# keisuke-777/HandyRL

Measured on AMD Instinct MI355X. Metric: learner env-steps/sec at B=4096 T=32 (TicTacToe net, UPGO/VTRACE), higher is better.
Workload: dtype f32; 1 GPU; TicTacToe SimpleConv2dModel learner step: forward + IS ratios + fused HIP V-trace/UPGO scans + losses + backward + grad all-reduce + clip + Adam; global_batch=4096, per_gpu_batch=4096, seq_len=32, players=2, parallelism=dp1, hip_graph=True

## Files before the change

### handyrl_amd/_native.py

```python

import ctypes
import os

import torch

LIB_PATH = os.path.join(os.path.dirname(os.path.abspath(__file__)), '_lib', 'libhrl.so')
LIB_PATH = os.environ.get('HRL_LIB_PATH', LIB_PATH)

HRL_OK = 0
HRL_EINVAL = -22

ALG = {'MC': 0, 'TD': 1, 'UPGO': 2, 'VTRACE': 3}

_f32p = ctypes.c_void_p
_i64 = ctypes.c_int64
_dbl = ctypes.c_double

SIGNATURES = {
    'hrl_abi_version': (ctypes.c_int, []),
    'hrl_targets_set_short_form': (ctypes.c_int, [ctypes.c_int]),
    'hrl_strerror': (ctypes.c_char_p, [ctypes.c_int]),
    'hrl_compute_target': (ctypes.c_int, [
        ctypes.c_int, _f32p, _f32p, _f32p, _f32p, _f32p,
        _i64, _i64, _i64, _i64, _i64, _i64, _dbl, _dbl, _f32p, _f32p, ctypes.c_void_p]),
    'hrl_compute_targets_fused': (ctypes.c_int, [
        ctypes.c_int, ctypes.c_int, _f32p, _f32p, _f32p, _f32p, _f32p,
        _i64, _i64, _i64, _i64, _i64, _i64, _dbl, _dbl, _f32p, _f32p, ctypes.c_void_p]),
    'hrl_bn_workspace_bytes': (ctypes.c_int64, [_i64, _i64, _i64]),
    'hrl_bn_forward_train': (ctypes.c_int, [
        _f32p, _i64, _i64, _i64, _f32p, _f32p, _f32p, _f32p, _dbl, _dbl, ctypes.c_int, _f32p, _f32p, _f32p,
        ctypes.c_void_p, _i64, ctypes.c_void_p]),
    'hrl_bn_backward': (ctypes.c_int, [
        _f32p, _f32p, _i64, _i64, _i64, _f32p, _f32p, _f32p, _f32p, ctypes.c_int, _f32p, _f32p, _f32p,
        ctypes.c_void_p, _i64, ctypes.c_void_p]),
    'hrl_bn_workspace_bytes_grouped': (ctypes.c_int64, [_i64, _i64, _i64, _i64]),
    'hrl_bn_forward_train_grouped': (ctypes.c_int, [
        _f32p, _i64, _i64, _i64, _i64, _f32p, _f32p, _f32p, _f32p, _dbl, _dbl, ctypes.c_int, _f32p, _f32p, _f32p,
        ctypes.c_void_p, _i64, ctypes.c_void_p]),
    'hrl_bn_backward_grouped': (ctypes.c_int, [
        _f32p, _f32p, _i64, _i64, _i64, _i64, _f32p, _f32p, _f32p, _f32p, ctypes.c_int, _f32p, _f32p, _f32p,
        ctypes.c_void_p, _i64, ctypes.c_void_p]),
    'hrl_loss_workspace_bytes': (ctypes.c_int64, [_i64, _i64, _i64, _i64]),
    'hrl_loss_forward': (ctypes.c_int, [
        _f32p, _f32p, ctypes.c_void_p, _i64, _i64, _i64, _i64, _i64,
        _f32p, _f32p, _f32p, _f32p, _f32p, _f32p, _f32p, _f32p, _f32p,
        ctypes.c_int, ctypes.c_int, ctypes.c_int, _dbl, _dbl, _dbl, _dbl,
        ctypes.c_void_p, _i64, _f32p, ctypes.c_void_p]),
    'hrl_loss_backward': (ctypes.c_int, [
        _f32p, ctypes.c_void_p, _i64, _i64, _i64, _i64, _i64,
        _f32p, _f32p, _f32p, _f32p, _f32p, _f32p, _dbl, _dbl,
        ctypes.c_void_p, _i64, _f32p, _f32p, _f32p, _f32p, ctypes.c_void_p]),
    'hrl_output_mask_forward': (ctypes.c_int, [_f32p, _f32p, _f32p, _f32p, _f32p, _i64, _i64, _i64, _i64, _f32p,
                                               _f32p, ctypes.c_void_p]),
    'hrl_output_mask_backward': (ctypes.c_int, [_f32p, _f32p, _f32p, _f32p, _i64, _i64, _i64, _i64, _f32p, _f32p,
                                                ctypes.c_void_p]),
    'hrl_board_weight': (ctypes.c_int, [_f32p, _i64, _i64, _i64, _i64, _i64, _i64, _f32p, ctypes.c_void_p]),
    'hrl_board_fold': (ctypes.c_int, [_f32p, _i64, _i64, _i64, _i64, _i64, _i64, _f32p, ctypes.c_void_p]),
    'hrl_board_bias': (ctypes.c_int, [_f32p, _i64, _i64, _f32p, ctypes.c_void_p]),
    'hrl_board_bias_fold': (ctypes.c_int, [_f32p, _i64, _i64, _f32p, ctypes.c_void_p]),
    'hrl_conv3x3_workspace_bytes': (ctypes.c_int64, [_i64]),
    'hrl_conv3x3_forward': (ctypes.c_int, [_f32p, _i64, _i64, _i64, _f32p, _f32p, ctypes.c_int, _f32p,
                                           ctypes.c_void_p, _i64, ctypes.c_void_p]),
    'hrl_conv3x3_wgrad': (ctypes.c_int, [_f32p, _f32p, _i64, _i64, _i64, _f32p, ctypes.c_void_p, _i64,
                                         ctypes.c_void_p]),
    'hrl_colsum_workspace_bytes': (ctypes.c_int64, [_i64, _i64]),
    'hrl_colsum': (ctypes.c_int, [_f32p, _i64, _i64, _f32p, ctypes.c_void_p, _i64, ctypes.c_void_p]),
    'hrl_bn_finalize_stats': (ctypes.c_int, [ctypes.c_void_p, _i64, _i64, _i64, _f32p, _f32p, _f32p, _f32p,
                                             ctypes.c_double, ctypes.c_double, _f32p, _f32p, _f32p, _f32p,
                                             ctypes.c_void_p]),
    'hrl_bn_forward_eval': (ctypes.c_int, [_f32p, _i64, _i64, _i64, _f32p, _f32p, _f32p, _f32p, ctypes.c_double,
                                           ctypes.c_int, _f32p, _f32p, ctypes.c_void_p]),
    'hrl_bn_apply': (ctypes.c_int, [_f32p, _i64, _i64, _i64, _f32p, _f32p, ctypes.c_int, _f32p, ctypes.c_void_p]),
    'hrl_conv3x3_stats_blocks': (ctypes.c_int64, [_i64]),
    'hrl_conv3x3_block_sum_blocks': (ctypes.c_int64, [_i64]),
    'hrl_conv3x3_set_split': (ctypes.c_int, [ctypes.c_int]),
    'hrl_conv3x3_set_block_form': (ctypes.c_int, [ctypes.c_int]),
    'hrl_conv3x3_set_fwd_form': (ctypes.c_int, [ctypes.c_int]),
    'hrl_torus_set_split': (ctypes.c_int, [ctypes.c_int]),
    'hrl_torus_set_form': (ctypes.c_int, [ctypes.c_int]),
    'hrl_conv3x3_pack_n': (ctypes.c_int, [ctypes.c_void_p, ctypes.c_int, _f32p, ctypes.c_void_p]),
    'hrl_conv3x3_forward_ex': (ctypes.c_int, [_f32p, _i64, _f32p, _f32p, _f32p, _f32p, ctypes.c_int, _f32p,
                                              ctypes.c_int, _f32p, _f32p, _f32p, _f32p, ctypes.c_void_p,
                                              ctypes.c_void_p, _i64, ctypes.c_void_p]),
    'hrl_bn_finalize_backward': (ctypes.c_int, [ctypes.c_void_p, _i64, _i64, _i64, _f32p, _f32p, _f32p, _f32p,
                                                _f32p, _f32p, ctypes.c_void_p]),
    'hrl_bn_backward_apply': (ctypes.c_int, [_f32p, _f32p, _i64, _i64, _i64, _f32p, _f32p, _f32p, _f32p,
                                             ctypes.c_int, _f32p, _f32p, _f32p, ctypes.c_void_p]),
    'hrl_conv3x3_block_backward': (ctypes.c_int, [_f32p, _f32p, _i64, _f32p, _f32p, _f32p, _f32p, _f32p, _f32p,
                                                  _f32p, _f32p, _f32p, _f32p, _f32p, _f32p, ctypes.c_int, _f32p,
                                                  _f32p, _f32p, ctypes.c_void_p, ctypes.c_void_p, _i64,
                                                  ctypes.c_void_p]),
    'hrl_conv3x3_wgrad_ex': (ctypes.c_int, [_f32p, _f32p, _f32p, _f32p, _i64, _f32p, ctypes.c_void_p, _i64,
                                            ctypes.c_void_p]),
    'hrl_hidden_gather': (ctypes.c_int, [ctypes.c_void_p, _f32p, _i64, _i64, ctypes.c_int, ctypes.c_void_p,
                                         ctypes.c_int, ctypes.c_void_p, ctypes.c_void_p]),
    'hrl_hidden_gather_backward': (ctypes.c_int, [ctypes.c_void_p, _f32p, _i64, _i64, ctypes.c_int, ctypes.c_void_p,
                                                  ctypes.c_int, ctypes.c_void_p, ctypes.c_void_p]),
    'hrl_hidden_gather_backward_add': (ctypes.c_int, [ctypes.c_void_p, _f32p, _i64, _i64, ctypes.c_int,
                                                      ctypes.c_void_p, ctypes.c_int, ctypes.c_void_p, ctypes.c_void_p,
                                                      ctypes.c_void_p, ctypes.c_void_p]),
    'hrl_hidden_update_gather': (ctypes.c_int, [ctypes.c_void_p, ctypes.c_void_p, _i64, _f32p, _f32p, _i64, _i64,
                                                ctypes.c_int, ctypes.c_void_p, ctypes.c_int, ctypes.c_void_p,
                                                ctypes.c_void_p, ctypes.c_void_p]),
    'hrl_hidden_update_gather_backward': (ctypes.c_int, [ctypes.c_void_p, _f32p, _f32p, _i64, _i64, _i64,
                                                         ctypes.c_int, ctypes.c_void_p, ctypes.c_int, ctypes.c_void_p,
                                                         ctypes.c_void_p, ctypes.c_void_p, ctypes.c_void_p,
                                                         ctypes.c_void_p, ctypes.c_void_p, ctypes.c_void_p]),
    'hrl_hidden_update_backward_add': (ctypes.c_int, [ctypes.c_void_p, _f32p, _i64, _i64, _i64, ctypes.c_int,
                                                      ctypes.c_void_p, ctypes.c_void_p, ctypes.c_void_p,
                                                      ctypes.c_void_p, ctypes.c_void_p, ctypes.c_void_p]),
    'hrl_hidden_update': (ctypes.c_int, [ctypes.c_void_p, ctypes.c_void_p, _i64, _f32p, _i64, _i64, ctypes.c_int,
                                         ctypes.c_void_p, ctypes.c_void_p, ctypes.c_void_p]),
    'hrl_hidden_update_backward': (ctypes.c_int, [ctypes.c_void_p, _f32p, _i64, _i64, _i64, ctypes.c_int,
                                                  ctypes.c_void_p, ctypes.c_void_p, ctypes.c_void_p, ctypes.c_void_p]),
    'hrl_lstm_gates_forward': (ctypes.c_int, [_f32p, _i64, _f32p, _f32p, _i64, _i64, _i64, _f32p, _i64, _f32p,
                                              _f32p, _f32p, ctypes.c_void_p]),
    'hrl_lstm_gates_backward': (ctypes.c_int, [_f32p, _f32p, _f32p, _f32p, _f32p, _i64, _i64, _i64, _f32p, _f32p,
                                               ctypes.c_void_p]),
    'hrl_torus_workspace_bytes': (ctypes.c_int64, [_i64]),
    'hrl_torus_stats_blocks': (ctypes.c_int64, [_i64]),
    'hrl_torus_conv_forward': (ctypes.c_int, [_f32p, _i64, _i64, _i64, _i64, _i64, _f32p, _f32p, ctypes.c_int,
                                              _f32p, ctypes.c_void_p, _f32p, _f32p, ctypes.c_void_p, _i64,
                                              ctypes.c_void_p]),
    'hrl_stem_workspace_bytes': (ctypes.c_int64, [_i64]),
    'hrl_stem_forward': (ctypes.c_int, [_f32p, _i64, _i64, _f32p, _f32p, _f32p, ctypes.c_void_p]),
    'hrl_stem_wgrad': (ctypes.c_int, [_f32p, _f32p, _i64, _i64, _f32p, _f32p, ctypes.c_void_p, _i64,
                                      ctypes.c_void_p]),
    'hrl_stem_set_wgrad_form': (ctypes.c_int, [ctypes.c_int]),
    'hrl_stem_set_fwd_form': (ctypes.c_int, [ctypes.c_int]),
    'hrl_clip_grad_norm': (ctypes.c_int, [_f32p, _i64, _dbl, _f32p, ctypes.c_void_p]),
    'hrl_clip_workspace_bytes': (ctypes.c_int64, [_i64]),
    'hrl_grad_fold_norm_blocks': (ctypes.c_int64, [_i64]),
    'hrl_grad_fold_norm': (ctypes.c_int, [_f32p, _i64, ctypes.c_void_p, ctypes.c_void_p, ctypes.c_void_p,
                                          ctypes.c_void_p, ctypes.c_void_p, ctypes.c_void_p, ctypes.c_void_p,
                                          ctypes.c_int, _f32p, ctypes.c_void_p, ctypes.c_void_p, ctypes.c_int,
                                          ctypes.c_void_p, _i64, ctypes.c_void_p]),
    'hrl_adam_clip': (ctypes.c_int, [_f32p, _i64, ctypes.c_void_p, _dbl, _f32p, ctypes.c_void_p, ctypes.c_void_p,
                                     ctypes.c_void_p, ctypes.c_int, _f32p, _f32p, _f32p, _f32p, _dbl, _dbl, _dbl,
                                     _dbl, ctypes.c_void_p, ctypes.c_int, _f32p, ctypes.c_void_p]),
    'hrl_conv3x3_wgrad_partials': (ctypes.c_int64, [_i64, ctypes.c_void_p]),
    'hrl_stem_wgrad_partials': (ctypes.c_int64, [_i64, ctypes.c_void_p]),
    'hrl_clip_grad_norm_ws': (ctypes.c_int, [_f32p, _i64, _dbl, _f32p, ctypes.c_void_p, _i64, ctypes.c_void_p]),
    'hrl_heads_workspace_bytes': (ctypes.c_int64, [_i64]),
    'hrl_heads_bn_parts': (ctypes.c_int64, [_i64]),
    'hrl_heads_set_bwd_form': (ctypes.c_int, [ctypes.c_int]),
    'hrl_heads_forward': (ctypes.c_int, [_f32p, _i64, _f32p, _f32p, _f32p, _f32p, _f32p, _f32p, _f32p, _f32p,
                                         _f32p, _f32p, _f32p, _f32p, ctypes.c_int, ctypes.c_void_p]),
    'hrl_heads_backward': (ctypes.c_int, [_f32p, _i64, _f32p, _f32p, _f32p, _f32p, _f32p, _f32p, _f32p,
                                          ctypes.c_void_p, _f32p, _f32p, _f32p, _f32p, _f32p, _f32p, _f32p, _f32p,
                                          _f32p, _f32p, _f32p, _f32p, ctypes.c_void_p, _i64, ctypes.c_void_p]),
    'hrl_bn_apply_residual': (ctypes.c_int, [_f32p, _f32p, _i64, _i64, _i64, _f32p, _f32p, _f32p, ctypes.c_void_p]),
    'hrl_bn_backward_masked': (ctypes.c_int, [_f32p, _f32p, _f32p, _i64, _i64, _i64, _f32p, _f32p, _f32p, _f32p,
                                              _f32p, _f32p, ctypes.c_void_p, _i64, ctypes.c_void_p]),
    'hrl_torus_conv_wgrad': (ctypes.c_int, [_f32p, _f32p, _i64, _i64, _i64, _i64, _i64, _f32p, _f32p,
                                            ctypes.c_void_p, _i64, ctypes.c_void_p]),
    'hrl_torus_conv_wgrad_bn': (ctypes.c_int, [_f32p, _i64, _i64, _i64, _i64, _f32p, _f32p, _f32p, _f32p,
                                               ctypes.c_int, _f32p, _f32p, _f32p, _f32p, _f32p, _f32p, _f32p, _f32p,
                                               ctypes.c_void_p, _i64, ctypes.c_void_p]),
    'hrl_bn_backward_masked_coefs': (ctypes.c_int, [_f32p, _f32p, _f32p, _i64, _i64, _i64, _f32p, _f32p, _f32p,
                                                    _f32p, _f32p, _f32p, _f32p, ctypes.c_void_p, _i64,
                                                    ctypes.c_void_p]),
    'hrl_torus_unit_forward': (ctypes.c_int, [_f32p, _f32p, _f32p, _f32p, _f32p, _i64, _i64, _i64, _f32p, _f32p,
                                              _f32p, ctypes.c_void_p, ctypes.c_void_p, _i64, ctypes.c_void_p]),
    'hrl_torus_unit_input_grad': (ctypes.c_int, [_f32p, _i64, _i64, _i64, _f32p, _f32p, _f32p, _f32p, _f32p,
                                                 _f32p, _f32p, ctypes.c_void_p, ctypes.c_void_p, _i64,
                                                 ctypes.c_void_p]),
    'hrl_board_conv_workspace_bytes': (ctypes.c_int64, [_i64]),
    'hrl_board_conv_forward': (ctypes.c_int, [_f32p, _i64, _i64, _i64, _i64, _f32p, _i64, _i64, _i64, _f32p, _f32p,
                                              ctypes.c_void_p, _i64, ctypes.c_void_p]),
    'hrl_board_conv_pack': (ctypes.c_int, [_f32p, _i64, _i64, _i64, ctypes.c_void_p, _i64, ctypes.c_void_p]),
    'hrl_board_conv_forward_packed': (ctypes.c_int, [_f32p, _i64, _i64, _i64, _i64, ctypes.c_void_p, _i64, _f32p,
                                                     _f32p, ctypes.c_void_p]),
    'hrl_gboard_pack_bytes': (ctypes.c_int64, [_i64, _i64]),
    'hrl_gboard_pack': (ctypes.c_int, [_f32p, _i64, _i64, _i64, _i64, ctypes.c_void_p, _i64, ctypes.c_void_p]),
    'hrl_gboard_pack_adjoint': (ctypes.c_int, [_f32p, _i64, _i64, _i64, _i64, ctypes.c_void_p, _i64,
                                               ctypes.c_void_p]),
    'hrl_gboard_wgrad_workspace_bytes': (ctypes.c_int64, [_i64, _i64, _i64]),
    'hrl_gboard_wgrad': (ctypes.c_int, [ctypes.c_void_p, ctypes.c_void_p, ctypes.c_void_p, ctypes.c_void_p,
                                        ctypes.c_void_p, ctypes.c_int, _i64, _i64, _f32p, _i64, _i64, _f32p,
                                        ctypes.c_void_p, _i64, ctypes.c_void_p]),
    'hrl_gboard_set_whole_ring': (ctypes.c_int, [ctypes.c_int]),
    'hrl_gboard_set_nctw': (ctypes.c_int, [ctypes.c_int]),
    'hrl_gboard_launch_stats': (ctypes.c_int, [ctypes.c_void_p, ctypes.c_int, ctypes.c_int]),
    'hrl_gboard_pointwise_wgrad_workspace_bytes': (_i64, [_i64, _i64, _i64]),
    'hrl_gboard_pointwise_wgrad': (ctypes.c_int, [_f32p, _i64, _f32p, _i64, _i64, _i64, _i64, _f32p, ctypes.c_void_p,
                                                  _i64, ctypes.c_void_p]),
    'hrl_gboard_forward_groups': (ctypes.c_int, [ctypes.c_void_p, ctypes.c_void_p, _i64, _i64, _i64, ctypes.c_void_p,
                                                 _i64, _i64, _f32p, _i64, ctypes.c_void_p]),
    'hrl_lstm_gates_backward_ex': (ctypes.c_int, [_f32p, _f32p, _f32p, _f32p, _i64, ctypes.c_int, _i64, _f32p, _i64,
                                                  _i64, _i64, _f32p, _f32p, _f32p, ctypes.c_int, ctypes.c_void_p]),
    'hrl_lstm_gates_forward_grouped': (ctypes.c_int, [ctypes.c_int, _f32p, _i64, ctypes.c_void_p, ctypes.c_void_p,
                                                      ctypes.c_void_p, _i64, _i64, _i64, ctypes.c_void_p,
                                                      ctypes.c_void_p, ctypes.c_void_p, ctypes.c_void_p]),
    'hrl_gboard_forward': (ctypes.c_int, [_f32p, _i64, _f32p, _i64, _i64, _i64, _i64, ctypes.c_void_p, _i64, _i64,
                                          _f32p, _f32p, _f32p, ctypes.c_int, _f32p, _i64, ctypes.c_void_p]),
    'hrl_gboard_pointwise': (ctypes.c_int, [_f32p, _i64, _i64, _f32p, _i64, _i64, _i64, _f32p, _i64, _f32p, _f32p,
                                            ctypes.c_int, _f32p, _i64, ctypes.c_void_p]),
    'hrl_torus_head_pool': (ctypes.c_int, [_f32p, _f32p, _i64, _i64, _i64, _i64, _f32p, _f32p, ctypes.c_void_p]),
    'hrl_torus_head_unpool': (ctypes.c_int, [_f32p, _f32p, _f32p, _i64, _i64, _i64, _i64, _f32p,
                                             ctypes.c_void_p]),
    'hrl_bn_backward_apply_masked': (ctypes.c_int, [_f32p, _f32p, _f32p, _i64, _i64, _i64, _f32p, _f32p, _f32p,
                                                    _f32p, _f32p, _f32p, ctypes.c_void_p]),
    'hrl_geister_legal': (ctypes.c_int, [ctypes.c_void_p, ctypes.c_void_p, ctypes.c_void_p, _i64, ctypes.c_void_p,
                                         ctypes.c_void_p]),
    'hrl_geister_observation': (ctypes.c_int, [ctypes.c_void_p, ctypes.c_void_p, ctypes.c_void_p, ctypes.c_void_p,
                                               _i64, ctypes.c_int, _f32p, _f32p, ctypes.c_void_p]),
    'hrl_geister_step': (ctypes.c_int, [ctypes.c_void_p, ctypes.c_void_p, ctypes.c_void_p, ctypes.c_void_p,
                                        ctypes.c_void_p, ctypes.c_void_p, ctypes.c_void_p, ctypes.c_void_p,
                                        ctypes.c_void_p, _i64, ctypes.c_void_p, ctypes.c_void_p]),
    'hrl_selfplay_sample_record': (ctypes.c_int, [_f32p, _i64, ctypes.c_void_p, _f32p, ctypes.c_void_p, _f32p,
                                                  ctypes.c_void_p, ctypes.c_void_p, ctypes.c_void_p, _i64, _i64,
                                                  _i64, _i64, ctypes.c_void_p, _f32p, _f32p, ctypes.c_void_p, _f32p,
                                                  ctypes.c_void_p, ctypes.c_void_p, ctypes.c_void_p]),
    'hrl_masked_rows_copy': (ctypes.c_int, [ctypes.c_int, ctypes.c_void_p, ctypes.c_void_p, ctypes.c_void_p,
                                            ctypes.c_void_p, ctypes.c_void_p, ctypes.c_void_p, _i64,
                                            ctypes.c_void_p]),
    'hrl_geister_observation_record': (ctypes.c_int, [ctypes.c_void_p, ctypes.c_void_p, ctypes.c_void_p,
                                                      ctypes.c_void_p, _i64, ctypes.c_int, _f32p, _f32p,
                                                      ctypes.c_void_p, ctypes.c_void_p, _i64, _f32p, _f32p,
                                                      ctypes.c_void_p]),
}

ABI_VERSION = 27

_lib = None


def load():
    global _lib
    if _lib is not None:
        return _lib
    if not os.path.exists(LIB_PATH):
        raise RuntimeError('HIP library %s is missing: run `python -m handyrl_amd.build` '
                           '(there is no CPU fallback for the learner kernels)' % LIB_PATH)
    lib = ctypes.CDLL(LIB_PATH)
    for name, (res, args) in SIGNATURES.items():
        fn = getattr(lib, name)
        fn.restype = res
        fn.argtypes = args
    if lib.hrl_abi_version() != ABI_VERSION:
        raise RuntimeError('libhrl.so ABI %d != expected %d' % (lib.hrl_abi_version(), ABI_VERSION))
    _lib = lib
    return lib


def check(code, what):
    if code != HRL_OK:
        msg = load().hrl_strerror(code).decode()
        if code == HRL_EINVAL:
            raise ValueError('%s: %s' % (what, msg))
        raise RuntimeError('%s failed (%d): %s' % (what, code, msg))


def ptr(t):
    return None if t is None else ctypes.c_void_p(t.data_ptr())


def ptr_array(tensors):
    arr = (ctypes.c_void_p * len(tensors))(*[None if t is None else t.data_ptr() for t in tensors])
    return arr


def i64_array(values):
    return (ctypes.c_int64 * len(values))(*values)


def stream_of(device):
    return ctypes.c_void_p(torch.cuda.current_stream(device).cuda_stream)
```

### handyrl_amd/csrc/hrl_conv.hip

```cpp

#include <hip/hip_runtime.h>
#include <stdint.h>
#include <stdlib.h>

#include <type_traits>

#include "../../include/hrl_nn.h"
#include "../../include/hrl_targets.h"
#include "hrl_split.h"
#include "hrl_stamps.h"

namespace {

HRL_STAMP_DECL

typedef float f32x4 __attribute__((ext_vector_type(4)));

constexpr int kBoard = 3;
constexpr int kCells = kBoard * kBoard;
constexpr int kTaps = 9;
constexpr int kC = 32;
constexpr int kRow = kC * kCells;
constexpr int kStride = kRow + 2;
constexpr int kTile = 16;
// ... 385 lines not shown
                    acc[tap][1][1] = mfma(a1, b1, acc[tap][1][1]);
                }
            }
        }
        __builtin_amdgcn_wave_barrier();
    }
    __syncthreads();
    float *red = lds;
    constexpr int kW = kTaps * kC * kC;
#pragma unroll
    for (int t = 0; t < kTaps; ++t)
#pragma unroll
        for (int it = 0; it < 2; ++it)
#pragma unroll
            for (int jt = 0; jt < 2; ++jt)
#pragma unroll
                for (int r = 0; r < 4; ++r) {
                    const int ci = it * 16 + (lane >> 4) * 4 + r;
                    const int co = jt * 16 + (lane & 15);
                    red[wave * kW + (t * kC + ci) * kC + co] = acc[t][it][jt][r];
                }
    __syncthreads();
    float *out = partial + (int64_t)blockIdx.x * kW;
    for (int i = threadIdx.x; i < kW; i += kThreads)
        out[i] = ((red[i] + red[kW + i]) + red[2 * kW + i]) + red[3 * kW + i];
}

constexpr int kStrideW = kRow + 4;
typedef float f32x16 __attribute__((ext_vector_type(16)));
typedef __bf16 bf16x8_t __attribute__((ext_vector_type(8)));

__device__ __forceinline__ f32x16 mfma32(const uint4 &a, const uint4 &b, f32x16 c) {
    return __builtin_amdgcn_mfma_f32_32x32x16_bf16(__builtin_bit_cast(bf16x8_t, a), __builtin_bit_cast(bf16x8_t, b),
                                                   c, 0, 0, 0);
}

template <bool PRO>
__global__ __launch_bounds__(kThreads) void conv3x3_wgrad_split_kernel(const float *__restrict__ x,
                                                                       const float *__restrict__ in_alpha,
                                                                       const float *__restrict__ in_beta,
                                                                       const float *__restrict__ dy, int64_t M,
                                                                       float *__restrict__ partial) {
    __shared__ __attribute__((aligned(16))) float lds[2 * kWaves * kTile * kStrideW];
    static_assert(2 * kWaves * kTile * kStrideW >= kWaves * kTaps * kC * kC, "fold buffer");
    const int lane = threadIdx.x & 63;
    const int wave = threadIdx.x >> 6;
    float *xs = lds + wave * kTile * kStrideW;
    float *gs = lds + (kWaves + wave) * kTile * kStrideW;
    const int r = lane & 31, h = lane >> 5;
    float pa = 1.f, pb = 0.f;
    if constexpr (PRO) {
        pa = in_alpha[r];
        pb = in_beta[r];
    }
    const int64_t ntiles = (M + kTile - 1) / kTile;
    const int64_t stride = (int64_t)gridDim.x * kWaves;
    const int64_t lim = M * kRow;

    f32x16 acc[kTaps];
#pragma unroll
    for (int t = 0; t < kTaps; ++t)
#pragma unroll
        for (int i = 0; i < 16; ++i) acc[t][i] = 0.f;

    for (int64_t tile = (int64_t)blockIdx.x * kWaves + wave; tile < ntiles; tile += stride) {
        {
            const int64_t base = tile * kTile * kRow;
            float4 sx[kVec], sg[kVec];
#pragma unroll
            for (int k = 0; k < kVec; ++k) {
                const int64_t e = base + (int64_t)(k * 64 + lane) * 4;
                const int64_t ec = e < lim ? e : lim - 4;
                sx[k] = *reinterpret_cast<const float4 *>(x + ec);
                sg[k] = *reinterpret_cast<const float4 *>(dy + ec);
            }
#pragma unroll
            for (int k = 0; k < kVec; ++k) {
                const int e = (k * 64 + lane) * 4;
                const int row = e / kRow, c = e - row * kRow;
                const bool ok = base + e < lim;
                *reinterpret_cast<float4 *>(xs + row * kStrideW + c) = sx[k];
                *reinterpret_cast<float4 *>(gs + row * kStrideW + c) = ok ? sg[k] : make_float4(0.f, 0.f, 0.f, 0.f);
            }
        }
        __builtin_amdgcn_s_waitcnt(0xc07f);
        __builtin_amdgcn_wave_barrier();

        uint4 Bh[kCells], Bm[kCells], Bl[kCells];
        const float *gcol = gs + (8 * h) * kStrideW + r * kCells;
#pragma unroll
        for (int q = 0; q < kCells; ++q) {
            float v[8];
#pragma unroll
            for (int j = 0; j < 8; ++j) v[j] = gcol[j * kStrideW + q];
            hrl_split::split8(v, Bh[q], Bm[q], Bl[q]);
        }
        const float *xcol = xs + (8 * h) * kStrideW + r * kCells;
#pragma unroll
        for (int p = 0; p < kCells; ++p) {
            float v[8];
#pragma unroll
            for (int j = 0; j < 8; ++j) {
                float a = xcol[j * kStrideW + p];
                if constexpr (PRO) {
                    const float t = a * pa + pb;
                    a = t < 0.f ? 0.f : t;
                }
                v[j] = a;
            }
            uint4 Ah, Am, Al;
            hrl_split::split8(v, Ah, Am, Al);
#pragma unroll
            for (int q = 0; q < kCells; ++q) {
                const int tap = tap_of(p, q);
                if (tap < 0) continue;
                f32x16 c = acc[tap];
                c = mfma32(Al, Bh[q], c);
                c = mfma32(Am, Bm[q], c);
                c = mfma32(Ah, Bl[q], c);
                c = mfma32(Am, Bh[q], c);
                c = mfma32(Ah, Bm[q], c);
                c = mfma32(Ah, Bh[q], c);
                acc[tap] = c;
            }
        }
        __builtin_amdgcn_wave_barrier();
    }
    __syncthreads();
    float *red = lds;
    constexpr int kW = kTaps * kC * kC;
#pragma unroll
    for (int t = 0; t < kTaps; ++t)
#pragma unroll
        for (int i = 0; i < 16; ++i) {
            const int ci = (i & 3) + 8 * (i >> 2) + 4 * h;
            red[wave * kW + (t * kC + ci) * kC + r] = acc[t][i];
        }
    __syncthreads();
    float *out = partial + (int64_t)blockIdx.x * kW;
    for (int i = threadIdx.x; i < kW; i += kThreads)
        out[i] = ((red[i] + red[kW + i]) + red[2 * kW + i]) + red[3 * kW + i];
}

struct BlockBwdArgs {
    const float *g, *y;
    const float *bn_w, *bn_b, *bn_mean, *bn_invstd, *bn_k, *bn_gm;
    const float *x, *in_alpha, *in_beta;
    const float *wpk;
    const float *ep_mean, *ep_alpha, *ep_beta;
    float *gin;
    double *part;
    float *wpart;
    int64_t M;
};

typedef unsigned int u32x3 __attribute__((ext_vector_type(3)));
typedef unsigned int u32x2 __attribute__((ext_vector_type(2)));
typedef unsigned int u32x4 __attribute__((ext_vector_type(4)));

__device__ __forceinline__ __amdgpu_buffer_rsrc_t wave_rsrc(const void *base, uint32_t bytes) {
    const uint64_t p = reinterpret_cast<uint64_t>(base);
    const uint32_t lo = __builtin_amdgcn_readfirstlane((uint32_t)p);
    const uint32_t hi = __builtin_amdgcn_readfirstlane((uint32_t)(p >> 32));
    const uint32_t n = __builtin_amdgcn_readfirstlane(bytes);
    return __builtin_amdgcn_make_buffer_rsrc(reinterpret_cast<void *>(((uint64_t)hi << 32) | lo), (short)0, (int)n,
                                             0x00020000);
}

__device__ __forceinline__ void load_cells(__amdgpu_buffer_rsrc_t rs, int off, float (&d)[kCells]) {
#pragma unroll
    for (int m = 0; m < 3; ++m) {
        const u32x3 v = __builtin_amdgcn_raw_buffer_load_b96(rs, off + 12 * m, 0, 0);
        d[3 * m + 0] = __uint_as_float(v.x);
        d[3 * m + 1] = __uint_as_float(v.y);
        d[3 * m + 2] = __uint_as_float(v.z);
    }
}

__device__ __forceinline__ void store_cells(__amdgpu_buffer_rsrc_t rs, int off, const float (&d)[kCells]) {
#pragma unroll
    for (int m = 0; m < 3; ++m) {
        u32x3 v;
        v.x = __float_as_uint(d[3 * m + 0]);
        v.y = __float_as_uint(d[3 * m + 1]);
        v.z = __float_as_uint(d[3 * m + 2]);
        __builtin_amdgcn_raw_buffer_store_b96(v, rs, off + 12 * m, 0, 0);
    }
}

template <bool PRO, int EPI, bool DG>
__global__ __launch_bounds__(kThreads) void conv3x3_block_bwd_kernel(BlockBwdArgs a) {
    constexpr int kWWords = kTaps * 2 * 3 * 64 * 4;
    constexpr int kTileF = kTile * kStride;
    constexpr int kW = kTaps * kC * kC;
    constexpr int kFoldF = (kWaves - 1) * kW;
    constexpr int kUseF = DG ? kWWords + kWaves * kTileF : 0;
    constexpr int kSmemF = kUseF > kFoldF ? kUseF : kFoldF;
    __shared__ __attribute__((aligned(16))) float smem[kSmemF];
    uint32_t *w_lds_u = reinterpret_cast<uint32_t *>(smem);
    const int lane = threadIdx.x & 63;
    const int wave = threadIdx.x >> 6;
    float *as = smem + kWWords + wave * kTileF;
    if constexpr (DG) {
        for (int i = threadIdx.x; i < kWWords; i += kThreads) {
            const int d = i & 3, l = (i >> 2) & 63, f = i >> 8;
            const int part = f % 3, tc = f / 3;
            const int ci = 8 * (l >> 4) + 2 * d, j = l & 15;
            const float w0 = a.wpk[(tc * kC + ci) * 16 + j];
            const float w1 = a.wpk[(tc * kC + ci + 1) * 16 + j];
            w_lds_u[i] = split_part(w0, part) | (split_part(w1, part) << 16);
        }
    }
    const int r = lane & 31, h = lane >> 5;
    const float mu = a.bn_mean[r], kk = a.bn_k[r], gmn = a.bn_gm[r], is = a.bn_invstd[r];
    const float ww = a.bn_w ? a.bn_w[r] : 1.0f;
    const float al = is * ww;
    const float be = (a.bn_b ? a.bn_b[r] : 0.0f) - mu * al;
    float pa = 1.f, pb = 0.f;
    if constexpr (PRO) {
        pa = a.in_alpha[r];
        pb = a.in_beta[r];
    }
    float em = 0.f, ea = 1.f, eb = 0.f;
    if constexpr (DG && EPI == 2) {
        em = a.ep_mean[r];
        ea = a.ep_alpha[r];
        eb = a.ep_beta[r];
    }
    double s1 = 0.0, s2 = 0.0;
    f32x16 wacc[kTaps];
#pragma unroll
    for (int t = 0; t < kTaps; ++t)
#pragma unroll
        for (int i = 0; i < 16; ++i) wacc[t][i] = 0.f;
    if constexpr (DG) __syncthreads();

    const int64_t ntiles = (a.M + kTile - 1) / kTile;
    const int64_t stride = (int64_t)gridDim.x * kWaves;
    const int off0 = ((8 * h) * kRow + r * kCells) * 4;
    HRL_STAMP_WALL(14);
    int st_it = 0;
    for (int64_t tile = (int64_t)blockIdx.x * kWaves + wave; tile < ntiles; tile += stride, ++st_it) {
        if (st_it < 2) HRL_STAMP(6 * st_it + 0);
        const int64_t row0 = tile * kTile;
        const int rows = (int)min<int64_t>(kTile, a.M - row0);
        const uint32_t bytes = (uint32_t)rows * kRow * 4;
        const int64_t eofs = row0 * kRow;
        const __amdgpu_buffer_rsrc_t rg = wave_rsrc(a.g + eofs, bytes);
        const __amdgpu_buffer_rsrc_t ry = wave_rsrc(a.y + eofs, bytes);
        const __amdgpu_buffer_rsrc_t rx = wave_rsrc(a.x + eofs, bytes);
        float G[8][kCells], X[8][kCells];
        {
            float Y[8][kCells];
            auto bn_apply = [&]() __attribute__((always_inline)) {
#pragma unroll
                for (int j = 0; j < 8; ++j) {
                    const bool valid = 8 * h + j < rows;
#pragma unroll
                    for (int c = 0; c < kCells; ++c) {
                        const float yv = Y[j][c];
                        float gv = G[j][c];
                        if (!(yv * al + be > 0.f)) gv = 0.f;
                        const float t = (yv - mu) * kk;
                        const float d = (((gv - gmn) - t) * is) * ww;
                        G[j][c] = valid ? d : 0.f;
                    }
                }
            };
#pragma unroll
            for (int j = 0; j < 8; ++j) {
                load_cells(rg, off0 + j * kRow * 4, G[j]);
                load_cells(ry, off0 + j * kRow * 4, Y[j]);
                load_cells(rx, off0 + j * kRow * 4, X[j]);
            }
            bn_apply();
        }
        if (st_it < 2) HRL_STAMP(6 * st_it + 1);
        if constexpr (DG) {
#pragma unroll
            for (int j = 0; j < 8; ++j)
#pragma unroll
                for (int c = 0; c < kCells; ++c) as[(8 * h + j) * kStride + r * kCells + c] = G[j][c];
        }
        {
            uint4 Bh[kCells], Bm[kCells], Bl[kCells];
#pragma unroll
            for (int q = 0; q < kCells; ++q) {
                float v[8];
#pragma unroll
                for (int j = 0; j < 8; ++j) v[j] = G[j][q];
                hrl_split::split8(v, Bh[q], Bm[q], Bl[q]);
            }
#pragma unroll
            for (int p = 0; p < kCells; ++p) {
                float v[8];
#pragma unroll
                for (int j = 0; j < 8; ++j) {
                    float xv = X[j][p];
                    if constexpr (PRO) {
                        const float t = xv * pa + pb;
                        xv = t < 0.f ? 0.f : t;
                    }
                    v[j] = xv;
                }
                uint4 Ah, Am, Al;
                hrl_split::split8(v, Ah, Am, Al);
#pragma unroll
                for (int q = 0; q < kCells; ++q) {
                    const int tap = tap_of(p, q);
                    if (tap < 0) continue;
                    f32x16 c = wacc[tap];
                    c = mfma32(Al, Bh[q], c);
                    c = mfma32(Am, Bm[q], c);
                    c = mfma32(Ah, Bl[q], c);
                    c = mfma32(Am, Bh[q], c);
                    c = mfma32(Ah, Bm[q], c);
                    c = mfma32(Ah, Bh[q], c);
                    wacc[tap] = c;
                }
            }
        }
        if (st_it < 2) HRL_STAMP(6 * st_it + 2);
        if constexpr (DG) {
            float R[8][kCells];
            if constexpr (EPI == 2 || EPI == 3) {
#pragma unroll
                for (int j = 0; j < 8; ++j) load_cells(rx, off0 + j * kRow * 4, R[j]);
            }
            __builtin_amdgcn_s_waitcnt(0xc07f);
            __builtin_amdgcn_wave_barrier();
            f32x4 acc[kCells][2];
#pragma unroll
            for (int q = 0; q < kCells; ++q) acc[q][0] = acc[q][1] = (f32x4){0.f, 0.f, 0.f, 0.f};
            split_tile_mfma<false, true>(as, w_lds_u, lane, nullptr, nullptr, acc);
            __builtin_amdgcn_s_waitcnt(0xc07f);
            __builtin_amdgcn_wave_barrier();
            if (st_it < 2) HRL_STAMP(6 * st_it + 3);
#pragma unroll
            for (int q = 0; q < kCells; ++q)
#pragma unroll
                for (int ct = 0; ct < 2; ++ct)
#pragma unroll
                    for (int rr = 0; rr < 4; ++rr) {
                        const int row = (lane >> 4) * 4 + rr;
                        const int co = ct * 16 + (lane & 15);
                        as[row * kStride + co * kCells + q] = acc[q][ct][rr];
                    }
            __builtin_amdgcn_s_waitcnt(0xc07f);
            __builtin_amdgcn_wave_barrier();
            const __amdgpu_buffer_rsrc_t ro = wave_rsrc(a.gin + eofs, bytes);
            float t1 = 0.f, t2 = 0.f;
#pragma unroll
            for (int j = 0; j < 8; ++j) {
                const bool valid = 8 * h + j < rows;
                float o[kCells];
#pragma unroll
                for (int c = 0; c < kCells; ++c) {
                    float v = as[(8 * h + j) * kStride + r * kCells + c];
                    const float rv = (EPI == 2 || EPI == 3) ? R[j][c] : 0.f;
                    if constexpr (EPI == 3) {
                        if (!(rv > 0.f)) v = 0.f;
                    } else if constexpr (EPI == 2) {
                        const float gm = (rv * ea + eb > 0.f && valid) ? v : 0.f;
                        t1 += gm;
                        t2 += gm * (rv - em);
                    }
                    o[c] = v;
                }
                store_cells(ro, off0 + j * kRow * 4, o);
            }
            if constexpr (EPI == 2) {
                s1 += (double)t1;
                s2 += (double)t2;
            }
            __builtin_amdgcn_s_waitcnt(0xc07f);
            __builtin_amdgcn_wave_barrier();
        }
        if (st_it < 2) HRL_STAMP(6 * st_it + 4);
    }
    HRL_STAMP(12);
    __syncthreads();
    float *red = smem;
    if (wave > 0) {
#pragma unroll
        for (int t = 0; t < kTaps; ++t)
#pragma unroll
            for (int i = 0; i < 16; ++i) {
                const int ci = (i & 3) + 8 * (i >> 2) + 4 * h;
                red[(wave - 1) * kW + (t * kC + ci) * kC + r] = wacc[t][i];
            }
    }
    __syncthreads();
    if (wave == 0) {
        float *out = a.wpart + (int64_t)blockIdx.x * kW;
#pragma unroll
        for (int t = 0; t < kTaps; ++t)
#pragma unroll
            for (int i = 0; i < 16; ++i) {
                const int idx = (t * kC + (i & 3) + 8 * (i >> 2) + 4 * h) * kC + r;
                out[idx] = ((wacc[t][i] + red[idx]) + red[kW + idx]) + red[2 * kW + idx];
            }
    }
    if constexpr (DG && EPI == 2) {
        __syncthreads();
        double *dred = reinterpret_cast<double *>(smem);
        dred[((wave * 2 + h) * kC + r) * 2 + 0] = s1;
        dred[((wave * 2 + h) * kC + r) * 2 + 1] = s2;
        __syncthreads();
        if (threadIdx.x < 2 * kC) {
            const int c = threadIdx.x >> 1, k = threadIdx.x & 1;
            double t = 0.0;
            for (int i = 0; i < 2 * kWaves; ++i) t += dred[(i * kC + c) * 2 + k];
            a.part[((int64_t)blockIdx.x * kC + c) * 2 + k] = t;
        }
    }
    HRL_STAMP(13);
    HRL_STAMP_WALL(15);
}

namespace bb2 {

constexpr int kWaves = 8;
constexpr int kThreads = 64 * kWaves;
constexpr int kPartBytes = kCells * kC * kTile * 2;
constexpr int kImgBytes = 3 * kPartBytes;
constexpr int kDy0 = 0;
constexpr int kX0 = 2 * kImgBytes;
constexpr int kXrStride = kRow + 4;
constexpr int kXrBytes = kTile * kXrStride * 4;
constexpr int kXr0 = 4 * kImgBytes;
constexpr int kLdsBytes = kXr0 + 2 * kXrBytes;
static_assert(kLdsBytes <= 160 * 1024, "LDS");

typedef short v4s __attribute__((ext_vector_type(4)));
typedef __attribute__((address_space(3))) v4s lds_v4s;

__device__ __forceinline__ int img_off(int c, int ch, int half) {
    const int R = ch >> 3, j = ch & 7;
    return c * 1024 + R * 256 + 16 * ((2 * j + half) ^ (9 * (R & 1)));
}

__device__ __forceinline__ void bar_lds() {
    asm volatile("s_waitcnt lgkmcnt(0)" ::: "memory");
    __builtin_amdgcn_s_barrier();
    asm volatile("" ::: "memory");
}

template <int W> struct Role;
template <> struct Role<0> { static constexpr bool kIg = true, kCFirst = true; static constexpr int kCt = 0, kNq = 5, kNt = 0;
                             static constexpr int kQ[5] = {4, 5, 6, 7, 8}; static constexpr int kTap[1] = {0}; };
template <> struct Role<1> { static constexpr bool kIg = true, kCFirst = true; static constexpr int kCt = 1, kNq = 5, kNt = 0;
                             static constexpr int kQ[5] = {4, 5, 6, 7, 8}; static constexpr int kTap[1] = {0}; };
template <> struct Role<2> { static constexpr bool kIg = true, kCFirst = false; static constexpr int kCt = 0, kNq = 4, kNt = 0;
                             static constexpr int kQ[4] = {0, 1, 2, 3}; static constexpr int kTap[1] = {0}; };
template <> struct Role<3> { static constexpr bool kIg = true, kCFirst = false; static constexpr int kCt = 1, kNq = 4, kNt = 0;
                             static constexpr int kQ[4] = {0, 1, 2, 3}; static constexpr int kTap[1] = {0}; };
template <> struct Role<4> { static constexpr bool kIg = false, kCFirst = false; static constexpr int kCt = 0, kNq = 0, kNt = 2;
                             static constexpr int kQ[1] = {0}; static constexpr int kTap[2] = {0, 1}; };
template <> struct Role<5> { static constexpr bool kIg = false, kCFirst = false; static constexpr int kCt = 0, kNq = 0, kNt = 2;
                             static constexpr int kQ[1] = {0}; static constexpr int kTap[2] = {2, 5}; };
template <> struct Role<6> { static constexpr bool kIg = false, kCFirst = true; static constexpr int kCt = 0, kNq = 0, kNt = 2;
                             static constexpr int kQ[1] = {0}; static constexpr int kTap[2] = {3, 4}; };
template <> struct Role<7> { static constexpr bool kIg = false, kCFirst = true; static constexpr int kCt = 0, kNq = 0, kNt = 3;
                             static constexpr int kQ[1] = {0}; static constexpr int kTap[3] = {6, 7, 8}; };

template <int W> __device__ constexpr bool uses_p(int p) {
    using R = Role<W>;
    if constexpr (R::kIg) {
        for (int s = 0; s < R::kNq; ++s)
            if (tap_of(p, R::kQ[s]) >= 0) return true;
    } else {
        for (int s = 0; s < R::kNt; ++s) {
            const int dy = R::kTap[s] / 3, dx = R::kTap[s] % 3;
            const int qy = p / 3 - dy + 1, qx = p % 3 - dx + 1;
            if (qy >= 0 && qy < 3 && qx >= 0 && qx < 3) return true;
        }
    }
    return false;
}
template <int W> __device__ constexpr bool uses_tap(int t) {
    using R = Role<W>;
    for (int s = 0; s < R::kNq; ++s)
        for (int p = 0; p < kCells; ++p)
            if (tap_of(p, R::kQ[s]) == t) return true;
    return false;
}

#ifdef HRL_STAMPS
#define BB2_STAMP(it, k)                                                                                        \
    do {                                                                                                       \
        if ((it) == 2 || (it) == 3) {                                                                          \
            const unsigned long long t_ = __builtin_amdgcn_s_memtime();                                        \
            if (lane == 0 && g_hrl_stamps)                                                                     \
                g_hrl_stamps[(((size_t)blockIdx.x * 8 + W) * 2 + (it) - 2) * 8 + (k)] = t_;                    \
        }                                                                                                      \
    } while (0)
#else
#define BB2_STAMP(it, k) do { } while (0)
#endif

template <bool PRO, int EPI, int W>
__device__ __forceinline__ void run(const BlockBwdArgs &a, unsigned char *smem, int lane) {
    using R = Role<W>;
    constexpr bool kIg = R::kIg;
    constexpr int kNq = R::kNq > 0 ? R::kNq : 1;
    constexpr int kNt = R::kNt > 0 ? R::kNt : 1;
    constexpr int kCt = R::kCt;
    const int ch = lane & 31, hh = lane >> 5;
    constexpr bool kFwd = EPI == 1;
    float mu = 0.f, kk = 0.f, gmn = 0.f, is = 1.f, ww = 1.f, al = 1.f, be = 0.f;
    if constexpr (!kFwd) {
        kk = a.bn_k[ch]; gmn = a.bn_gm[ch];
        mu = a.bn_mean[ch]; is = a.bn_invstd[ch];
        ww = a.bn_w ? a.bn_w[ch] : 1.0f;
        al = is * ww;
        be = (a.bn_b ? a.bn_b[ch] : 0.0f) - mu * al;
    }
    float pa = 1.f, pb = 0.f;
    if constexpr (PRO) {
        pa = a.in_alpha[ch];
        pb = a.in_beta[ch];
    }
    uint4 wh[kTaps], wm[kTaps], wl[kTaps];
    if constexpr (kIg) {
        const int ci0 = 8 * (lane >> 4), j = lane & 15;
#pragma unroll
        for (int t = 0; t < kTaps; ++t) {
            if (!uses_tap<W>(t)) continue;
            uint32_t hv[4], mv[4], lv[4];
#pragma unroll
            for (int d = 0; d < 4; ++d) {
                const int tc = t * 2 + kCt;
                const float w0 = a.wpk[(tc * kC + ci0 + 2 * d) * 16 + j];
                const float w1 = a.wpk[(tc * kC + ci0 + 2 * d + 1) * 16 + j];
                uint32_t h0, m0, l0, h1, m1, l1;
                hrl_split::split3(w0, h0, m0, l0);
                hrl_split::split3(w1, h1, m1, l1);
                hv[d] = h0 | (h1 << 16);
                mv[d] = m0 | (m1 << 16);
                lv[d] = l0 | (l1 << 16);
            }
            wh[t] = make_uint4(hv[0], hv[1], hv[2], hv[3]);
            wm[t] = make_uint4(mv[0], mv[1], mv[2], mv[3]);
            wl[t] = make_uint4(lv[0], lv[1], lv[2], lv[3]);
        }
    }
    float em = 0.f, ea = 1.f, eb = 0.f;
    if constexpr (EPI == 2 && kIg) {
        em = a.ep_mean[kCt * 16 + (lane & 15)];
        ea = a.ep_alpha[kCt * 16 + (lane & 15)];
        eb = a.ep_beta[kCt * 16 + (lane & 15)];
    }
    double s1 = 0.0, s2 = 0.0;
    f32x16 wacc[kNt];
#pragma unroll
    for (int t = 0; t < kNt; ++t)
#pragma unroll
        for (int i = 0; i < 16; ++i) wacc[t][i] = 0.f;

    const int64_t ntiles = (a.M + kTile - 1) / kTile;
    const int64_t t0 = blockIdx.x;
    const int64_t step = gridDim.x;
    const int n_iter = t0 < ntiles ? (int)((ntiles - 1 - t0) / step + 1) : 0;
    const int rho0 = 2 * ((W + (ch >> 2)) & 7);
    const int c0 = hh ? 4 : 0;
    const int ldoff = (rho0 * kRow + ch * kCells + c0) * 4;
    float G[2][5], Y[2][5], X[2][5];
    auto rsrc_of = [&](const float *base, int it, int &rows) __attribute__((always_inline)) {
        const int64_t t = t0 + (int64_t)it * step;
        const bool ok = it < n_iter;
        rows = ok ? (int)min<int64_t>(kTile, a.M - t * kTile) : 0;
        return wave_rsrc(base + (ok ? t * kTile * kRow : 0), (uint32_t)rows * kRow * 4);
    };
    auto issue = [&](int it) __attribute__((always_inline)) {
        int rows;
        const __amdgpu_buffer_rsrc_t rg = rsrc_of(a.g, it, rows), ry = rsrc_of(a.y, it, rows),
                                     rx = rsrc_of(a.x, it, rows);
#pragma unroll
        for (int r = 0; r < 2; ++r) {
            const int off = ldoff + r * kRow * 4;
#pragma unroll
            for (int k = kFwd ? 2 : 0; k < 3; ++k) {
                const __amdgpu_buffer_rsrc_t rs = k == 0 ? rg : (k == 1 ? ry : rx);
                float(&d)[5] = k == 0 ? G[r] : (k == 1 ? Y[r] : X[r]);
                const u32x3 v = __builtin_amdgcn_raw_buffer_load_b96(rs, off, 0, 0);
                const u32x2 u = __builtin_amdgcn_raw_buffer_load_b64(rs, off + 12, 0, 0);
                d[0] = __uint_as_float(v.x);
                d[1] = __uint_as_float(v.y);
                d[2] = __uint_as_float(v.z);
                d[3] = __uint_as_float(u.x);
                d[4] = __uint_as_float(u.y);
            }
        }
    };
    auto stage = [&](int it) __attribute__((always_inline)) {
        const int64_t t = t0 + (int64_t)it * step;
        const int rows = (int)max<int64_t>(0, min<int64_t>(kTile, a.M - t * kTile));
        unsigned char *dyi = smem + kDy0 + (it & 1) * kImgBytes;
        unsigned char *xi = smem + kX0 + (it & 1) * kImgBytes;
        uint32_t dp[3][5], xp[3][5];
#pragma unroll
        for (int i = 0; i < 5; ++i) {
            float dv[2], xv2[2];
#pragma unroll
            for (int r = 0; r < 2; ++r) {
                const bool valid = rho0 + r < rows;
                const float yv = Y[r][i];
                float gv = G[r][i];
                if (!(yv * al + be > 0.f)) gv = 0.f;
                const float tt = (yv - mu) * kk;
                float d = (((gv - gmn) - tt) * is) * ww;
                d = valid ? d : 0.f;
                float xv = X[r][i];
                if constexpr (PRO) {
                    const float u = xv * pa + pb;
                    xv = u < 0.f ? 0.f : u;
                }
                if constexpr (kFwd) d = xv;
                dv[r] = d;
                xv2[r] = xv;
            }
            hrl_split::split_pair(dv[0], dv[1], dp[0][i], dp[1][i], dp[2][i]);
            if constexpr (!kFwd) hrl_split::split_pair(xv2[0], xv2[1], xp[0][i], xp[1][i], xp[2][i]);
        }
        const int half = rho0 >> 3, sub = 2 * (rho0 & 7);
#pragma unroll
        for (int i = 0; i < 5; ++i) {
            const int o = img_off(c0 + i, ch, half) + sub;
#pragma unroll
            for (int part = 0; part < 3; ++part) {
                *reinterpret_cast<uint32_t *>(dyi + part * kPartBytes + o) = dp[part][i];
                if constexpr (!kFwd) *reinterpret_cast<uint32_t *>(xi + part * kPartBytes + o) = xp[part][i];
            }
        }
        if constexpr (EPI == 2 || EPI == 3) {
            float *xr = reinterpret_cast<float *>(smem + kXr0 + (it & 1) * kXrBytes);
#pragma unroll
            for (int r = 0; r < 2; ++r)
#pragma unroll
                for (int i = 0; i < 5; ++i) xr[(rho0 + r) * kXrStride + ch * kCells + c0 + i] = X[r][i];
        }
    };
    f32x4 acc[kNq];
    auto compute = [&](int it) __attribute__((always_inline)) {
        const unsigned char *dyi = smem + kDy0 + (it & 1) * kImgBytes;
        if constexpr (!kIg && kFwd) {
        } else if constexpr (!kIg) {
            const unsigned char *xi = smem + kX0 + (it & 1) * kImgBytes;
            const int kg = lane >> 5;
#pragma unroll
            for (int p = 0; p < kCells; ++p) {
                if (!uses_p<W>(p)) continue;
                const int o = img_off(p, ch, kg);
                const uint4 Ah = *reinterpret_cast<const uint4 *>(xi + o);
                const uint4 Am = *reinterpret_cast<const uint4 *>(xi + kPartBytes + o);
                const uint4 Al = *reinterpret_cast<const uint4 *>(xi + 2 * kPartBytes + o);
#pragma unroll
                for (int s = 0; s < R::kNt; ++s) {
                    const int dy = R::kTap[s] / 3, dx = R::kTap[s] % 3;
                    const int qy = p / 3 - dy + 1, qx = p % 3 - dx + 1;
                    if (qy < 0 || qy > 2 || qx < 0 || qx > 2) continue;
                    const int ob = img_off(qy * 3 + qx, ch, kg);
                    const uint4 Bh = *reinterpret_cast<const uint4 *>(dyi + ob);
                    const uint4 Bm = *reinterpret_cast<const uint4 *>(dyi + kPartBytes + ob);
                    const uint4 Bl = *reinterpret_cast<const uint4 *>(dyi + 2 * kPartBytes + ob);
                    f32x16 c = wacc[s];
                    c = mfma32(Al, Bh, c);
                    c = mfma32(Am, Bm, c);
                    c = mfma32(Ah, Bl, c);
                    c = mfma32(Am, Bh, c);
                    c = mfma32(Ah, Bm, c);
                    c = mfma32(Ah, Bh, c);
                    wacc[s] = c;
                }
            }
        } else {
#pragma unroll
            for (int s = 0; s < kNq; ++s) acc[s] = (f32x4){0.f, 0.f, 0.f, 0.f};
            const int g = lane >> 4, i = lane & 15, qq = i >> 2, pp = i & 3;
            const int tr_sub = 8 * (pp & 1);
#pragma unroll
            for (int p = 0; p < kCells; ++p) {
                if (!uses_p<W>(p)) continue;
                uint32_t A[3][4];
#pragma unroll
                for (int part = 0; part < 3; ++part) {
#pragma unroll
                    for (int hlf = 0; hlf < 2; ++hlf) {
                        const int o = part * kPartBytes + img_off(p, 8 * g + 4 * hlf + qq, pp >> 1) + tr_sub;
                        const v4s r = __builtin_amdgcn_ds_read_tr16_b64_v4i16(
                            (lds_v4s *)((__attribute__((address_space(3))) unsigned char *)(dyi + o)));
                        const uint2 u = __builtin_bit_cast(uint2, r);
                        A[part][2 * hlf] = u.x;
                        A[part][2 * hlf + 1] = u.y;
                    }
                }
                const uint4 Ah = make_uint4(A[0][0], A[0][1], A[0][2], A[0][3]);
                const uint4 Am = make_uint4(A[1][0], A[1][1], A[1][2], A[1][3]);
                const uint4 Al = make_uint4(A[2][0], A[2][1], A[2][2], A[2][3]);
#pragma unroll
                for (int s = 0; s < R::kNq; ++s) {
                    const int tap = tap_of(p, R::kQ[s]);
                    if (tap < 0) continue;
                    const uint4 Bl = wl[tap];
                    f32x4 c = acc[s];
                    c = mfma_bf16(Al, wh[tap], c);
                    c = mfma_bf16(Am, wm[tap], c);
                    c = mfma_bf16(Ah, Bl, c);
                    c = mfma_bf16(Am, wh[tap], c);
                    c = mfma_bf16(Ah, wm[tap], c);
                    c = mfma_bf16(Ah, wh[tap], c);
                    acc[s] = c;
                }
            }
        }
    };
    auto epilogue = [&](int it) __attribute__((always_inline)) {
        if constexpr (kIg) {
            int rows;
            const __amdgpu_buffer_rsrc_t ro = rsrc_of(a.gin, it, rows);
            const int co = kCt * 16 + (lane & 15);
            float rv[kNq < 4 ? 4 : kNq][4];
            if constexpr (EPI == 2 || EPI == 3) {
                const float *xr = reinterpret_cast<const float *>(smem + kXr0 + (it & 1) * kXrBytes);
#pragma unroll
                for (int rr = 0; rr < 4; ++rr) {
                    const int row = (lane >> 4) * 4 + rr;
#pragma unroll
                    for (int s = 0; s < R::kNq; ++s) rv[s][rr] = xr[row * kXrStride + co * kCells + R::kQ[s]];
                }
            }
            if constexpr (EPI == 1) {
                float t1 = 0.f, t2 = 0.f;
#pragma unroll
                for (int s = 0; s < R::kNq; ++s) {
#pragma unroll
                    for (int rr = 0; rr < 4; ++rr) {
                        const int row = (lane >> 4) * 4 + rr;
                        const float u = row < rows ? acc[s][rr] : 0.f;
                        t1 += u;
                        t2 += u * u;
                    }
                }
                s1 += (double)t1;
                s2 += (double)t2;
            }
            if constexpr (EPI == 2) {
                float t1 = 0.f, t2 = 0.f;
#pragma unroll
                for (int s = 0; s < R::kNq; ++s) {
#pragma unroll
                    for (int rr = 0; rr < 4; ++rr) {
                        const int row = (lane >> 4) * 4 + rr;
                        const float x0 = rv[s][rr];
                        const float gm = (x0 * ea + eb > 0.f && row < rows) ? acc[s][rr] : 0.f;
                        t1 += gm;
                        t2 += gm * (x0 - em);
                    }
                }
                s1 += (double)t1;
                s2 += (double)t2;
            }
#pragma unroll
            for (int rr = 0; rr < 4; ++rr) {
                const int row = (lane >> 4) * 4 + rr;
                const int off = (row * kRow + co * kCells + R::kQ[0]) * 4;
                float v[kNq];
#pragma unroll
                for (int s = 0; s < R::kNq; ++s) {
                    v[s] = acc[s][rr];
                    if constexpr (EPI == 3)
                        if (!(rv[s][rr] > 0.f)) v[s] = 0.f;
                }
                u32x4 w;
                w.x = __float_as_uint(v[0]);
                w.y = __float_as_uint(v[1]);
                w.z = __float_as_uint(v[2]);
                w.w = __float_as_uint(v[3]);
                __builtin_amdgcn_raw_buffer_store_b128(w, ro, off, 0, 0);
                if constexpr (R::kNq > 4)
                    __builtin_amdgcn_raw_buffer_store_b32(__float_as_uint(v[4 % kNq]), ro, off + 16, 0, 0);
            }
        }
    };

    if (n_iter > 0) {
        issue(0);
        stage(0);
        issue(1);
    }
    bar_lds();
    for (int it = 0; it < n_iter; ++it) {
        BB2_STAMP(it, 0);
        if constexpr (R::kCFirst) {
            compute(it);
            epilogue(it);
            BB2_STAMP(it, 1);
            stage(it + 1);
            issue(it + 2);
            BB2_STAMP(it, 2);
        } else {
            stage(it + 1);
            issue(it + 2);
            BB2_STAMP(it, 1);
            compute(it);
            epilogue(it);
            BB2_STAMP(it, 2);
        }
        bar_lds();
        BB2_STAMP(it, 3);
    }
    if constexpr (!kIg && !kFwd) {
        constexpr int kW = kTaps * kC * kC;
        float *outp = a.wpart + (int64_t)blockIdx.x * kW;
        const int h = lane >> 5;
#pragma unroll
        for (int s = 0; s < R::kNt; ++s)
#pragma unroll
            for (int i = 0; i < 16; ++i) {
                const int ci = (i & 3) + 8 * (i >> 2) + 4 * h;
                outp[(R::kTap[s] * kC + ci) * kC + ch] = wacc[s][i];
            }
    }
    if constexpr (EPI == 1 || EPI == 2) {
        __syncthreads();
        double *dred = reinterpret_cast<double *>(smem);
        if (kIg) {
            dred[(W * 64 + lane) * 2 + 0] = s1;
            dred[(W * 64 + lane) * 2 + 1] = s2;
        }
        __syncthreads();
        if (W == 0) {
            const int c = lane >> 1, k = lane & 1, ct = c >> 4, l16 = c & 15;
            double tot = 0.0;
            for (int w = ct; w < 4; w += 2)
                for (int lg = 0; lg < 4; ++lg) tot += dred[(w * 64 + lg * 16 + l16) * 2 + k];
            a.part[((int64_t)blockIdx.x * kC + c) * 2 + k] = tot;
        }
    }
}

}

namespace fw3 {

constexpr int kSlots = 5;
constexpr int kRawBytes = kTile * kRow * 4;
constexpr int kPieces = kRawBytes / 1024;
constexpr int kImg0 = 0;
constexpr int kRaw0 = 2 * bb2::kImgBytes;
constexpr int kLdsBytes = kRaw0 + kSlots * kRawBytes;
static_assert(kLdsBytes <= 160 * 1024, "LDS");
static_assert(kRawBytes % 1024 == 0, "whole LDS-DMA pieces per tile");

template <int N> __device__ __forceinline__ void vm_wait() { asm volatile("s_waitcnt vmcnt(%0)" ::"n"(N) : "memory"); }

__device__ __forceinline__ void dma16(u32x4 desc, uint32_t voff, uint32_t lds_byte) {
    uint32_t keep;
    asm volatile("s_mov_b32 %0, m0\n\ts_mov_b32 m0, %3\n\ts_nop 0\n\tbuffer_load_dwordx4 %1, %2, 0 offen lds\n\t"
                 "s_mov_b32 m0, %0"
                 : "=&s"(keep)
                 : "v"(voff), "s"(desc), "s"(lds_byte)
                 : "memory");
}

__device__ __forceinline__ u32x4 wave_desc(const void *base, uint32_t bytes) {
    const uint64_t p = reinterpret_cast<uint64_t>(base);
    u32x4 d;
    d.x = __builtin_amdgcn_readfirstlane((uint32_t)p);
    d.y = __builtin_amdgcn_readfirstlane((uint32_t)(p >> 32)) & 0xffffu;
    d.z = __builtin_amdgcn_readfirstlane(bytes);
    d.w = 0x00020000u;
    return d;
}

template <int G> struct Cells;
template <> struct Cells<0> { static constexpr int kN = 3; static constexpr int kQ[3] = {0, 1, 2}; };
template <> struct Cells<1> { static constexpr int kN = 2; static constexpr int kQ[2] = {3, 4}; };
template <> struct Cells<2> { static constexpr int kN = 2; static constexpr int kQ[2] = {5, 6}; };
template <> struct Cells<3> { static constexpr int kN = 2; static constexpr int kQ[2] = {7, 8}; };

template <int G> __device__ constexpr bool g_uses_p(int p) {
    for (int s = 0; s < Cells<G>::kN; ++s)
        if (tap_of(p, Cells<G>::kQ[s]) >= 0) return true;
    return false;
}
template <int G> __device__ constexpr bool g_uses_tap(int t) {
    for (int s = 0; s < Cells<G>::kN; ++s)
        for (int p = 0; p < kCells; ++p)
            if (tap_of(p, Cells<G>::kQ[s]) == t) return true;
    return false;
}

template <int W> __device__ constexpr int pieces_of() {
    int n = 0;
    for (int p = W; p < kPieces; p += 8) ++n;
    return n;
}

template <int NP, int NS>
__device__ __forceinline__ void wait_tile_after(int it) {
    static_assert((kSlots - 2) * (NP + NS) + NS <= 63, "vmcnt");
    if (it == 0) vm_wait<(kSlots - 2) * NP + NS>();
    else if (it == 1) vm_wait<(kSlots - 2) * NP + 2 * NS>();
    else if (it == 2) vm_wait<(kSlots - 2) * NP + 3 * NS>();
    else vm_wait<(kSlots - 2) * (NP + NS) + NS>();
    static_assert(kSlots == 5, "the early-iteration counts above are written for kSlots = 5");
}

template <bool PRO, int W>
__device__ __forceinline__ void run(const BlockBwdArgs &a, unsigned char *smem, int lane) {
    constexpr int kCt = W & 1, G = W >> 1;
    using C = Cells<G>;
    constexpr int kNq = C::kN;
    constexpr int NP = pieces_of<W>();
    constexpr int NS = 4;
    const int64_t ntiles = (a.M + kTile - 1) / kTile;
    const int64_t t0 = blockIdx.x;
    const int64_t step = gridDim.x;
    const int n_iter = t0 < ntiles ? (int)((ntiles - 1 - t0) / step + 1) : 0;
    const int ch = lane & 31, hh = lane >> 5;
    uint4 wh[kTaps], wm[kTaps], wl[kTaps];
    {
        const int ci0 = 8 * (lane >> 4), j = lane & 15;
#pragma unroll
        for (int t = 0; t < kTaps; ++t) {
            if (!g_uses_tap<G>(t)) continue;
            uint32_t hv[4], mv[4], lv[4];
#pragma unroll
            for (int d = 0; d < 4; ++d) {
                const int tc = t * 2 + kCt;
                const float w0 = a.wpk[(tc * kC + ci0 + 2 * d) * 16 + j];
                const float w1 = a.wpk[(tc * kC + ci0 + 2 * d + 1) * 16 + j];
                uint32_t h0, m0, l0, h1, m1, l1;
                hrl_split::split3(w0, h0, m0, l0);
                hrl_split::split3(w1, h1, m1, l1);
                hv[d] = h0 | (h1 << 16);
                mv[d] = m0 | (m1 << 16);
                lv[d] = l0 | (l1 << 16);
            }
            wh[t] = make_uint4(hv[0], hv[1], hv[2], hv[3]);
            wm[t] = make_uint4(mv[0], mv[1], mv[2], mv[3]);
            wl[t] = make_uint4(lv[0], lv[1], lv[2], lv[3]);
        }
    }
    float pa = 1.f, pb = 0.f;
    if constexpr (PRO) {
        pa = a.in_alpha[ch];
        pb = a.in_beta[ch];
    }
    asm volatile("s_waitcnt vmcnt(0)" ::: "memory");
    const uint32_t smem_base = (uint32_t)(uintptr_t)smem;
    auto dma = [&](int it, int slot) __attribute__((always_inline)) {
        const int64_t t = t0 + (int64_t)it * step;
        const bool ok = it < n_iter;
// ... 15 lines not shown
        float xv[2][5];
#pragma unroll
        for (int r = 0; r < 2; ++r) {
            const float *src = raw + (rho0 + r) * kRow + ch * kCells + c0;
#pragma unroll
            for (int i = 0; i < 5; ++i) {
                float v = src[i];
                if constexpr (PRO) {
                    const float u = v * pa + pb;
                    v = u < 0.f ? 0.f : u;
                }
                xv[r][i] = v;
            }
        }
#pragma unroll
        for (int i = 0; i < 5; ++i) hrl_split::split_pair(xv[0][i], xv[1][i], xp[0][i], xp[1][i], xp[2][i]);
        const int half = rho0 >> 3, sub = 2 * (rho0 & 7);
#pragma unroll
        for (int i = 0; i < 5; ++i) {
            const int o = bb2::img_off(c0 + i, ch, half) + sub;
#pragma unroll
            for (int part = 0; part < 3; ++part)
                *reinterpret_cast<uint32_t *>(xi + part * bb2::kPartBytes + o) = xp[part][i];
        }
    };
    const int co = kCt * 16 + (lane & 15);
    const int g = lane >> 4, i16 = lane & 15, qq = i16 >> 2, pp = i16 & 3;
    const int tr_sub = 8 * (pp & 1);
    double s1 = 0.0, s2 = 0.0;
#pragma unroll
    for (int j = 0; j < kSlots; ++j) dma(j, j);
    vm_wait<(kSlots - 1) * NP>();
    bb2::bar_lds();
    stage(0, 0);
    vm_wait<(kSlots - 2) * NP>();
    bb2::bar_lds();
    int slot = 0;
    for (int it = 0; it < n_iter; ++it) {
        BB2_STAMP(it, 0);
        dma(it + kSlots, slot);
        const int next = slot + 1 == kSlots ? 0 : slot + 1;
        stage(it + 1, next);
        BB2_STAMP(it, 1);
        const unsigned char *img = smem + kImg0 + (it & 1) * bb2::kImgBytes;
        f32x4 acc[kNq];
#pragma unroll
        for (int s = 0; s < kNq; ++s) acc[s] = (f32x4){0.f, 0.f, 0.f, 0.f};
#pragma unroll
        for (int p = 0; p < kCells; ++p) {
            if (!g_uses_p<G>(p)) continue;
            uint32_t A[3][4];
#pragma unroll
            for (int part = 0; part < 3; ++part) {
#pragma unroll
                for (int hlf = 0; hlf < 2; ++hlf) {
                    const int o = part * bb2::kPartBytes + bb2::img_off(p, 8 * g + 4 * hlf + qq, pp >> 1) + tr_sub;
                    const bb2::v4s r = __builtin_amdgcn_ds_read_tr16_b64_v4i16(
                        (bb2::lds_v4s *)((__attribute__((address_space(3))) unsigned char *)(img + o)));
                    const uint2 u = __builtin_bit_cast(uint2, r);
                    A[part][2 * hlf] = u.x;
                    A[part][2 * hlf + 1] = u.y;
                }
            }
            const uint4 Ah = make_uint4(A[0][0], A[0][1], A[0][2], A[0][3]);
            const uint4 Am = make_uint4(A[1][0], A[1][1], A[1][2], A[1][3]);
            const uint4 Al = make_uint4(A[2][0], A[2][1], A[2][2], A[2][3]);
#pragma unroll
            for (int s = 0; s < kNq; ++s) {
                const int tap = tap_of(p, C::kQ[s]);
                if (tap < 0) continue;
                f32x4 c = acc[s];
                c = mfma_bf16(Al, wh[tap], c);
                c = mfma_bf16(Am, wm[tap], c);
                c = mfma_bf16(Ah, wl[tap], c);
                c = mfma_bf16(Am, wh[tap], c);
                c = mfma_bf16(Ah, wm[tap], c);
                c = mfma_bf16(Ah, wh[tap], c);
                acc[s] = c;
            }
        }
        BB2_STAMP(it, 2);
        const int64_t t = t0 + (int64_t)it * step;
        const int rows = (int)min<int64_t>(kTile, a.M - t * kTile);
        const __amdgpu_buffer_rsrc_t od = wave_rsrc(a.gin + t * kTile * kRow, (uint32_t)rows * kRow * 4);
        float t1 = 0.f, t2 = 0.f;
#pragma unroll
        for (int s = 0; s < kNq; ++s) {
#pragma unroll
            for (int rr = 0; rr < 4; ++rr) {
                const int row = (lane >> 4) * 4 + rr;
                const float u = row < rows ? acc[s][rr] : 0.f;
                t1 += u;
                t2 += u * u;
            }
        }
        s1 += (double)t1;
        s2 += (double)t2;
#pragma unroll
        for (int rr = 0; rr < 4; ++rr) {
            const int row = (lane >> 4) * 4 + rr;
            const int off = (row * kRow + co * kCells + C::kQ[0]) * 4;
            if constexpr (kNq == 3) {
                u32x3 v;
                v.x = __float_as_uint(acc[0][rr]);
                v.y = __float_as_uint(acc[1][rr]);
                v.z = __float_as_uint(acc[2 % kNq][rr]);
                __builtin_amdgcn_raw_buffer_store_b96(v, od, off, 0, 0);
            } else {
                u32x2 v;
                v.x = __float_as_uint(acc[0][rr]);
                v.y = __float_as_uint(acc[1][rr]);
                __builtin_amdgcn_raw_buffer_store_b64(v, od, off, 0, 0);
            }
        }
        wait_tile_after<NP, NS>(it);
        BB2_STAMP(it, 3);
        bb2::bar_lds();
        slot = next;
    }
    vm_wait<0>();
    __syncthreads();
    double *dred = reinterpret_cast<double *>(smem);
    dred[(W * 64 + lane) * 2 + 0] = s1;
    dred[(W * 64 + lane) * 2 + 1] = s2;
    __syncthreads();
    if (W == 0) {
        const int c = lane >> 1, k = lane & 1, ct = c >> 4, l16 = c & 15;
        double tot = 0.0;
        for (int w = ct; w < 8; w += 2)
            for (int lg = 0; lg < 4; ++lg) tot += dred[(w * 64 + lg * 16 + l16) * 2 + k];
        a.part[((int64_t)blockIdx.x * kC + c) * 2 + k] = tot;
    }
}

}

template <bool PRO>
__global__ __launch_bounds__(bb2::kThreads) void conv3x3_fwd_dma_kernel(BlockBwdArgs a) {
    __shared__ __attribute__((aligned(16))) unsigned char smem[fw3::kLdsBytes];
    const int lane = threadIdx.x & 63;
    const int wave = __builtin_amdgcn_readfirstlane(threadIdx.x >> 6);
    switch (wave) {
    case 0: fw3::run<PRO, 0>(a, smem, lane); break;
    case 1: fw3::run<PRO, 1>(a, smem, lane); break;
    case 2: fw3::run<PRO, 2>(a, smem, lane); break;
    case 3: fw3::run<PRO, 3>(a, smem, lane); break;
    case 4: fw3::run<PRO, 4>(a, smem, lane); break;
    case 5: fw3::run<PRO, 5>(a, smem, lane); break;
    case 6: fw3::run<PRO, 6>(a, smem, lane); break;
    default: fw3::run<PRO, 7>(a, smem, lane); break;
    }
}

template <bool PRO, int EPI>
__global__ __launch_bounds__(bb2::kThreads) void conv3x3_block_bwd2_kernel(BlockBwdArgs a) {
    __shared__ __attribute__((aligned(16))) unsigned char smem[bb2::kLdsBytes];
    const int lane = threadIdx.x & 63;
    const int wave = __builtin_amdgcn_readfirstlane(threadIdx.x >> 6);
    switch (wave) {
    case 0: bb2::run<PRO, EPI, 0>(a, smem, lane); break;
    case 1: bb2::run<PRO, EPI, 1>(a, smem, lane); break;
    case 2: bb2::run<PRO, EPI, 2>(a, smem, lane); break;
    case 3: bb2::run<PRO, EPI, 3>(a, smem, lane); break;
    case 4: bb2::run<PRO, EPI, 4>(a, smem, lane); break;
    case 5: bb2::run<PRO, EPI, 5>(a, smem, lane); break;
    case 6: bb2::run<PRO, EPI, 6>(a, smem, lane); break;
    default: bb2::run<PRO, EPI, 7>(a, smem, lane); break;
    }
}

__global__ __launch_bounds__(256) void conv3x3_wgrad_reduce_kernel(const float *__restrict__ partial, int nparts,
                                                                   float *__restrict__ dw) {
    __shared__ float red[4][64];
    constexpr int kW = kTaps * kC * kC;
    const int col = threadIdx.x & 63, sub = threadIdx.x >> 6;
    const int i = blockIdx.x * 64 + col;
    float s0 = 0.f, s1 = 0.f, s2 = 0.f, s3 = 0.f;
    int w = sub;
    for (; w + 12 < nparts; w += 16) {
        s0 += partial[(int64_t)w * kW + i];
        s1 += partial[(int64_t)(w + 4) * kW + i];
        s2 += partial[(int64_t)(w + 8) * kW + i];
        s3 += partial[(int64_t)(w + 12) * kW + i];
    }
    for (; w < nparts; w += 4) s0 += partial[(int64_t)w * kW + i];
    red[sub][col] = (s0 + s1) + (s2 + s3);
    __syncthreads();
    if (sub == 0) {
        const float s = ((red[0][col] + red[1][col]) + red[2][col]) + red[3][col];
        const int co = i % kC, ci = (i / kC) % kC, tap = i / (kC * kC);
        dw[(co * kC + ci) * kTaps + tap] = s;
    }
}

__global__ void conv3x3_pack_kernel(const float *__restrict__ w, int flip, float *__restrict__ wpk) {
    const int i = blockIdx.x * blockDim.x + threadIdx.x;
    if (i >= kTaps * 2 * kC * 16) return;
    const int j = i % 16, k = (i / 16) % kC, ct = (i / (16 * kC)) % 2, tap = i / (16 * kC * 2);
    const int out_c = ct * 16 + j;
    const int in_c = k;
    float v;
    if (!flip) v = w[(out_c * kC + in_c) * kTaps + tap];
    else v = w[(in_c * kC + out_c) * kTaps + (kTaps - 1 - tap)];
    wpk[i] = v;
}

constexpr int kPack = kTaps * 2 * kC * 16;
struct WeightList {
    const float *w[8];
};
__global__ void conv3x3_pack_n_kernel(WeightList wl, int n, float *__restrict__ packed) {
    const int i = blockIdx.x * blockDim.x + threadIdx.x;
    if (i >= n * 2 * kPack) return;
    const int l = i / (2 * kPack), flip = (i / kPack) & 1, e = i % kPack;
    const int j = e % 16, k = (e / 16) % kC, ct = (e / (16 * kC)) % 2, tap = e / (16 * kC * 2);
    const int out_c = ct * 16 + j, in_c = k;
    const float *w = wl.w[l];
    packed[i] = !flip ? w[(out_c * kC + in_c) * kTaps + tap] : w[(in_c * kC + out_c) * kTaps + (kTaps - 1 - tap)];
}

int g_split = 1;
int g_block_form = 1;
int g_fwd_form = 2;

constexpr int kGrid = 256;

int status() {
    const hipError_t e = hipGetLastError();
    return e == hipSuccess ? HRL_OK : HRL_ELAUNCH_BASE - (int)e;
}

bool aligned16(const void *p) { return (reinterpret_cast<uintptr_t>(p) & 15) == 0; }

int grid_for(int64_t M) {
    const int64_t tiles = (M + kTile - 1) / kTile;
    const int64_t blocks = (tiles + kWaves - 1) / kWaves;
    return (int)(blocks < kGrid ? blocks : kGrid);
}

}

extern "C" {

#ifdef HRL_STAMPS
int hrl_debug_set_stamps_conv(void *buf) { return (int)hipMemcpyToSymbol(HIP_SYMBOL(g_hrl_stamps), &buf, sizeof(buf)); }
#endif

int64_t hrl_conv3x3_workspace_bytes(int64_t M) {
    if (M < 1) return -1;
    return (int64_t)grid_for(M) * kTaps * kC * kC * 4 + (int64_t)kTaps * 2 * kC * 16 * 4 * 2;
}

int64_t hrl_conv3x3_stats_blocks(int64_t M) { return M < 1 ? -1 : grid_for(M); }

int64_t hrl_conv3x3_block_sum_blocks(int64_t M) { return M < 1 ? -1 : grid_for(M); }

int hrl_conv3x3_set_block_form(int form) {
    const int prev = g_block_form;
    g_block_form = form < 0 ? 0 : (form > 1 ? 1 : form);
    return prev;
}

int hrl_conv3x3_set_fwd_form(int form) {
    const int prev = g_fwd_form;
    g_fwd_form = form < 0 ? 0 : (form > 2 ? 2 : form);
    return prev;
}

int hrl_conv3x3_set_split(int on) {
    const int prev = g_split;
    g_split = on ? 1 : 0;
    return prev;
}

int hrl_conv3x3_forward_ex(const float *x, int64_t M, const float *in_alpha, const float *in_beta,
                           const float *weight, const float *bias, int flip, float *y, int epilogue,
                           const float *ref, const float *ep_mean, const float *ep_alpha, const float *ep_beta,
                           double *part, void *workspace, int64_t workspace_bytes, void *stream) {
    if (M < 1 || !x || !weight || !y || !workspace) return HRL_EINVAL;
    if (!aligned16(x) || !aligned16(y) || workspace_bytes < hrl_conv3x3_workspace_bytes(M)) return HRL_EINVAL;
    if ((in_alpha == nullptr) != (in_beta == nullptr)) return HRL_EINVAL;
    if (epilogue < 0 || epilogue > 3) return HRL_EINVAL;
    if ((epilogue == 1 || epilogue == 2) && !part) return HRL_EINVAL;
    if ((epilogue == 2 || epilogue == 3) && (!ref || !aligned16(ref))) return HRL_EINVAL;
    if (epilogue == 2 && (!ep_mean || !ep_alpha || !ep_beta)) return HRL_EINVAL;
    if (epilogue >= 2 && bias) return HRL_EINVAL;
    hipStream_t s = static_cast<hipStream_t>(stream);
    const float *wpk = weight;
    if (!(flip & 2)) {
        float *dst = static_cast<float *>(workspace);
        hipLaunchKernelGGL(conv3x3_pack_kernel, dim3((kPack + 255) / 256), dim3(256), 0, s, weight, flip & 1, dst);
        const int rc = status();
        if (rc) return rc;
        wpk = dst;
    }
    if (epilogue == 1 && (flip & 2) && !bias && g_split && g_fwd_form >= 1 && M * kRow * 4 <= 0xffffffffLL) {
        BlockBwdArgs a{};
        a.x = x; a.in_alpha = in_alpha; a.in_beta = in_beta; a.wpk = wpk; a.gin = y; a.part = part; a.M = M;
        const dim3 grid(grid_for(M)), block(bb2::kThreads);
        if (g_fwd_form == 2) {
            if (in_alpha) hipLaunchKernelGGL((conv3x3_fwd_dma_kernel<true>), grid, block, 0, s, a);
            else hipLaunchKernelGGL((conv3x3_fwd_dma_kernel<false>), grid, block, 0, s, a);
        } else if (in_alpha) {
            hipLaunchKernelGGL((conv3x3_block_bwd2_kernel<true, 1>), grid, block, 0, s, a);
        } else {
            hipLaunchKernelGGL((conv3x3_block_bwd2_kernel<false, 1>), grid, block, 0, s, a);
        }
        return status();
    }
    const dim3 grid(grid_for(M)), block(kThreads);
#define HRL_CONV_LAUNCH(PRO, EPI)                                                                             \
    do {                                                                                                      \
        if (g_split)                                                                                          \
            hipLaunchKernelGGL((conv3x3_kernel<PRO, EPI, true>), grid, block, 0, s, x, M, wpk, bias, in_alpha, \
                               in_beta, ref, ep_mean, ep_alpha, ep_beta, y, part);                            \
        else                                                                                                  \
            hipLaunchKernelGGL((conv3x3_kernel<PRO, EPI, false>), grid, block, 0, s, x, M, wpk, bias, in_alpha, \
                               in_beta, ref, ep_mean, ep_alpha, ep_beta, y, part);                            \
    } while (0)
    const bool pro = in_alpha != nullptr;
    switch (epilogue) {
    case 0: if (pro) HRL_CONV_LAUNCH(true, 0); else HRL_CONV_LAUNCH(false, 0); break;
    case 1: if (pro) HRL_CONV_LAUNCH(true, 1); else HRL_CONV_LAUNCH(false, 1); break;
    case 2: if (pro) HRL_CONV_LAUNCH(true, 2); else HRL_CONV_LAUNCH(false, 2); break;
    default: if (pro) HRL_CONV_LAUNCH(true, 3); else HRL_CONV_LAUNCH(false, 3); break;
    }
#undef HRL_CONV_LAUNCH
    return status();
}

int hrl_conv3x3_pack_n(const float *const *weights, int n, float *packed, void *stream) {
    if (n < 1 || n > 8 || !weights || !packed) return HRL_EINVAL;
    WeightList wl{};
    for (int i = 0; i < n; ++i) {
        if (!weights[i]) return HRL_EINVAL;
        wl.w[i] = weights[i];
    }
    hipLaunchKernelGGL(conv3x3_pack_n_kernel, dim3((n * 2 * kPack + 255) / 256), dim3(256), 0,
                       static_cast<hipStream_t>(stream), wl, n, packed);
    return status();
}

int hrl_conv3x3_forward(const float *x, int64_t M, int64_t C_in, int64_t C_out, const float *weight,
                        const float *bias, int flip, float *y, void *workspace, int64_t workspace_bytes,
                        void *stream) {
    if (C_in != kC || C_out != kC) return HRL_EINVAL;
    return hrl_conv3x3_forward_ex(x, M, nullptr, nullptr, weight, bias, flip, y, 0, nullptr, nullptr, nullptr,
                                  nullptr, nullptr, workspace, workspace_bytes, stream);
}

int hrl_conv3x3_wgrad_ex(const float *x, const float *in_alpha, const float *in_beta, const float *dy, int64_t M,
                         float *dweight, void *workspace, int64_t workspace_bytes, void *stream) {
    if (M < 1 || !x || !dy || !dweight || !workspace) return HRL_EINVAL;
    if ((in_alpha == nullptr) != (in_beta == nullptr)) return HRL_EINVAL;
    if (!aligned16(x) || !aligned16(dy) || workspace_bytes < hrl_conv3x3_workspace_bytes(M)) return HRL_EINVAL;
    hipStream_t s = static_cast<hipStream_t>(stream);
    const int grid = grid_for(M);
    float *partial = static_cast<float *>(workspace) + kTaps * 2 * kC * 16 * 2;
    if (g_split) {
        if (in_alpha)
            hipLaunchKernelGGL((conv3x3_wgrad_split_kernel<true>), dim3(grid), dim3(kThreads), 0, s, x, in_alpha,
                               in_beta, dy, M, partial);
        else
            hipLaunchKernelGGL((conv3x3_wgrad_split_kernel<false>), dim3(grid), dim3(kThreads), 0, s, x, in_alpha,
                               in_beta, dy, M, partial);
    } else if (in_alpha) {
        hipLaunchKernelGGL((conv3x3_wgrad_kernel<true>), dim3(grid), dim3(kThreads), 0, s, x, in_alpha, in_beta, dy,
                           M, partial);
    } else {
        hipLaunchKernelGGL((conv3x3_wgrad_kernel<false>), dim3(grid), dim3(kThreads), 0, s, x, in_alpha, in_beta,
                           dy, M, partial);
    }
    int rc = status();
    if (rc) return rc;
    hipLaunchKernelGGL(conv3x3_wgrad_reduce_kernel, dim3(kTaps * kC * kC / 64), dim3(256), 0, s, partial, grid,
                       dweight);
    return status();
}

int hrl_conv3x3_block_backward(const float *g, const float *y, int64_t M, const float *bn_weight,
                               const float *bn_bias, const float *save_mean, const float *save_invstd,
                               const float *kcoef, const float *gmean, const float *x, const float *in_alpha,
                               const float *in_beta, const float *packed_flip, float *dweight, float *gin,
                               int epilogue, const float *ep_mean, const float *ep_alpha, const float *ep_beta,
                               double *part, void *workspace, int64_t workspace_bytes, void *stream) {
    if (M < 1 || !g || !y || !save_mean || !save_invstd || !kcoef || !gmean || !x || !workspace)
        return HRL_EINVAL;
    if ((in_alpha == nullptr) != (in_beta == nullptr)) return HRL_EINVAL;
    if (workspace_bytes < hrl_conv3x3_workspace_bytes(M) || M * kRow * 4 > 0xffffffffLL) return HRL_EINVAL;
    if (gin && (!packed_flip || epilogue < 0 || epilogue == 1 || epilogue > 3)) return HRL_EINVAL;
    if (gin && epilogue == 2 && (!ep_mean || !ep_alpha || !ep_beta || !part)) return HRL_EINVAL;
    hipStream_t s = static_cast<hipStream_t>(stream);
    const int grid = grid_for(M);
    float *wpart = static_cast<float *>(workspace) + kTaps * 2 * kC * 16 * 2;
    BlockBwdArgs a{g, y, bn_weight, bn_bias, save_mean, save_invstd, kcoef, gmean, x, in_alpha, in_beta, packed_flip,
                   ep_mean, ep_alpha, ep_beta, gin, part, wpart, M};
    const bool pro = in_alpha != nullptr;
#define HRL_BLOCK_LAUNCH(PRO, EPI, DG) \
    hipLaunchKernelGGL((conv3x3_block_bwd_kernel<PRO, EPI, DG>), dim3(grid), dim3(kThreads), 0, s, a)
#define HRL_BLOCK2_LAUNCH(PRO, EPI) \
    hipLaunchKernelGGL((conv3x3_block_bwd2_kernel<PRO, EPI>), dim3(grid), dim3(bb2::kThreads), 0, s, a)
    if (!gin) {
        if (pro) HRL_BLOCK_LAUNCH(true, 0, false); else HRL_BLOCK_LAUNCH(false, 0, false);
    } else if (g_block_form == 0) {
        if (epilogue == 2) {
            if (pro) HRL_BLOCK_LAUNCH(true, 2, true); else HRL_BLOCK_LAUNCH(false, 2, true);
        } else if (epilogue == 3) {
            if (pro) HRL_BLOCK_LAUNCH(true, 3, true); else HRL_BLOCK_LAUNCH(false, 3, true);
        } else {
            if (pro) HRL_BLOCK_LAUNCH(true, 0, true); else HRL_BLOCK_LAUNCH(false, 0, true);
        }
    } else if (epilogue == 2) {
        if (pro) HRL_BLOCK2_LAUNCH(true, 2); else HRL_BLOCK2_LAUNCH(false, 2);
    } else if (epilogue == 3) {
        if (pro) HRL_BLOCK2_LAUNCH(true, 3); else HRL_BLOCK2_LAUNCH(false, 3);
    } else {
        if (pro) HRL_BLOCK2_LAUNCH(true, 0); else HRL_BLOCK2_LAUNCH(false, 0);
    }
#undef HRL_BLOCK_LAUNCH
#undef HRL_BLOCK2_LAUNCH
    int rc = status();
    if (rc || !dweight) return rc;
    hipLaunchKernelGGL(conv3x3_wgrad_reduce_kernel, dim3(kTaps * kC * kC / 64), dim3(256), 0, s, wpart, grid,
                       dweight);
    return status();
}

int64_t hrl_conv3x3_wgrad_partials(int64_t M, int64_t *offset_bytes) {
    if (M < 1) return -1;
    if (offset_bytes) *offset_bytes = (int64_t)kTaps * 2 * kC * 16 * 2 * 4;
    return grid_for(M);
}

int hrl_conv3x3_wgrad(const float *x, const float *dy, int64_t M, int64_t C_in, int64_t C_out, float *dweight,
                      void *workspace, int64_t workspace_bytes, void *stream) {
    if (C_in != kC || C_out != kC) return HRL_EINVAL;
    return hrl_conv3x3_wgrad_ex(x, nullptr, nullptr, dy, M, dweight, workspace, workspace_bytes, stream);
}

}
```

### handyrl_amd/csrc/hrl_heads.hip

```cpp

#include <hip/hip_runtime.h>
#include <stdint.h>

#include <algorithm>

#include "../../include/hrl_nn.h"
#include "../../include/hrl_targets.h"

namespace {

constexpr int kC = 32;
constexpr int kHW = 9;
constexpr int kRow = kC * kHW;
constexpr int kMP = 2, kMV = 1;
constexpr int kM = kMP + kMV;
constexpr int kZ = kM * kHW;
constexpr int kZP = kMP * kHW;
constexpr int kOP = 9;
constexpr int kSC = 4;
constexpr int kNS = kC / kSC;
constexpr int kSF = kSC * kHW;
constexpr int kSV = kSF / 4;
constexpr int kTS = kSF + 1;
constexpr float kSlope = 0.1f;
// ... 222 lines not shown
    __shared__ float tile[64 * kTS];
    __shared__ float sw1[kM * kC], swp[kOP * kZP], swv[kHW], sal[kC], sbe[kC], smu[kC];
    __shared__ float gw1[kM * kC * 64];
    __shared__ float gbn[kC * 2 * 64];
    const int lane = threadIdx.x;
    for (int i = lane; i < kM * kC; i += 64) sw1[i] = w1_at(w, i / kC, i % kC);
    for (int i = lane; i < kOP * kZP; i += 64) swp[i] = w.wp[i];
    if (lane < kHW) swv[lane] = w.wv[lane];
    for (int i = lane; i < kM * kC * 64; i += 64) gw1[i] = 0.f;
    if (bn.alpha && lane < kC) {
        sal[lane] = bn.alpha[lane];
        sbe[lane] = bn.beta[lane];
        smu[lane] = bn.part ? bn.mean[lane] : 0.f;
    }
    if (bn.part)
        for (int i = lane; i < kC * 2 * 64; i += 64) gbn[i] = 0.f;
    __syncthreads();

    float gb1[kM];
#pragma unroll
    for (int i = 0; i < kM; ++i) gb1[i] = 0.f;

    for (int64_t base = (int64_t)blockIdx.x * 64; base < N; base += (int64_t)gridDim.x * 64) {
        const int nrows = (int)min<int64_t>(64, N - base);
        const bool valid = lane < nrows;
        const int64_t n = base + (valid ? lane : 0);
        float4 st[kSV];
        load_slice(h, base, nrows, 0, lane, st);
        float a[kZ], g[kOP], gv;
#pragma unroll
        for (int j = 0; j < kZP; ++j) a[j] = a_p[n * kZP + j];
#pragma unroll
        for (int q = 0; q < kHW; ++q) a[kZP + q] = a_v[n * kHW + q];
#pragma unroll
        for (int k = 0; k < kOP; ++k) g[k] = valid ? dp[n * kOP + k] : 0.f;
        gv = valid ? dv[n] : 0.f;
        if (vt) {
            gv = gv * (1.f - vt[n] * vt[n]);
            if (valid) dv_raw[n] = gv;
        }
        float dz[kZ];
#pragma unroll
        for (int j = 0; j < kZP; ++j) {
            float t = 0.f;
#pragma unroll
            for (int k = 0; k < kOP; ++k) t += g[k] * swp[k * kZP + j];
            dz[j] = a[j] > 0.f ? t : t * kSlope;
        }
#pragma unroll
        for (int q = 0; q < kHW; ++q) {
            const float t = gv * swv[q];
            dz[kZP + q] = a[kZP + q] > 0.f ? t : t * kSlope;
        }
#pragma unroll
        for (int m = 0; m < kM; ++m) {
            float t = 0.f;
#pragma unroll
            for (int q = 0; q < kHW; ++q) t += dz[m * kHW + q];
            gb1[m] += t;
        }
#pragma unroll 1
        for (int s = 0; s < kNS; ++s) {
            slice_to_lds(st, tile, lane);
            lds_fence();
            if (s + 1 < kNS) load_slice(h, base, nrows, s + 1, lane, st);
            float x[kSF], yraw[kSF];
#pragma unroll
            for (int j = 0; j < kSF; ++j) x[j] = yraw[j] = tile[lane * kTS + j];
            if (bn.alpha) {
#pragma unroll
                for (int j = 0; j < kSF; ++j) x[j] = bn_relu(x[j], sal[s * kSC + j / kHW], sbe[s * kSC + j / kHW]);
            }
#pragma unroll
            for (int m = 0; m < kM; ++m)
#pragma unroll
                for (int cc = 0; cc < kSC; ++cc) {
                    float t = 0.f;
#pragma unroll
                    for (int q = 0; q < kHW; ++q) t += dz[m * kHW + q] * x[cc * kHW + q];
                    gw1[(m * kC + s * kSC + cc) * 64 + lane] += t;
                }
            lds_fence();
#pragma unroll
            for (int cc = 0; cc < kSC; ++cc) {
                const int c = s * kSC + cc;
                float t1 = 0.f, t2 = 0.f;
#pragma unroll
                for (int q = 0; q < kHW; ++q) {
                    float t = 0.f;
#pragma unroll
                    for (int m = 0; m < kM; ++m) t += sw1[m * kC + c] * dz[m * kHW + q];
                    tile[lane * kTS + cc * kHW + q] = t;
                    if (bn.part) {
                        const float y = yraw[cc * kHW + q];
                        const float gm = (y * sal[c] + sbe[c] > 0.f) ? t : 0.f;
                        t1 += gm;
                        t2 += gm * (y - smu[c]);
                    }
                }
                if (bn.part) {
                    gbn[(c * 2 + 0) * 64 + lane] += t1;
                    gbn[(c * 2 + 1) * 64 + lane] += t2;
                }
            }
            lds_fence();
#pragma unroll
            for (int k = 0; k < kSV; ++k) {
                const int i = k * 64 + lane;
                const int r = i / kSV, c4 = i - r * kSV;
                if (r < nrows) {
                    const float *sp = tile + r * kTS + c4 * 4;
                    *reinterpret_cast<float4 *>(dh + (base + r) * kRow + s * kSF + c4 * 4) =
                        make_float4(sp[0], sp[1], sp[2], sp[3]);
                }
            }
            lds_fence();
        }
    }
    float *out = part + (int64_t)blockIdx.x * kGN;
    lds_fence();
    for (int i = lane; i < kM * kC; i += 64) {
        float t = 0.f;
        for (int l = 0; l < 64; ++l) t += gw1[i * 64 + l];
        out[kGW1 + i] = t;
    }
#pragma unroll
    for (int i = 0; i < kM; ++i) {
        const float t = wave_sum(gb1[i]);
        if (lane == 0) out[kGB1 + i] = t;
    }
    if (bn.part) {
        const int c = lane >> 1, k = lane & 1;
        double t = 0.0;
        for (int l = 0; l < 64; ++l) t += (double)gbn[(c * 2 + k) * 64 + l];
        bn.part[((int64_t)blockIdx.x * kC + c) * 2 + k] = t;
    }
}

constexpr int kBR = 32;
constexpr int kDZS = 28;
constexpr int kSMS = 40;
constexpr int kSmG = 0, kSmGV = 9, kSmAP = 10, kSmAV = 28;
constexpr int kFcN = kOP * kZP + kHW;
constexpr int kWaves2 = 4;
constexpr int kGR = 8;
constexpr int kGV = kGR * kRow / 4 / 64;

__device__ __forceinline__ void load_group(__amdgpu_buffer_rsrc_t rh, int64_t row0, int lane, hu32x4 (&st)[kGV]) {
    const uint32_t ob = (uint32_t)(row0 * kRow * 4);
#pragma unroll
    for (int k = 0; k < kGV; ++k) st[k] = __builtin_amdgcn_raw_buffer_load_b128(rh, ob + (k * 64 + lane) * 16, 0, 0);
}

template <bool BN>
__global__ __launch_bounds__(256, 2) void heads_bwd2_kernel(const float *__restrict__ h, int64_t N, Weights w, BnIn bn,
                                                         const float *__restrict__ a_p, const float *__restrict__ a_v,
                                                         const float *__restrict__ dp, const float *__restrict__ dv,
                                                         const float *__restrict__ vt, float *__restrict__ dh,
                                                         float *__restrict__ part) {
    __shared__ __attribute__((aligned(16))) float sdz[kWaves2][kBR * kDZS];
    __shared__ __attribute__((aligned(16))) float ssm[kWaves2][kBR * kSMS];
    __shared__ float swp[kOP * kZP], swv[kHW];
    __shared__ __attribute__((aligned(16))) float sx[kWaves2][kGR * kRow];
    static_assert(sizeof(float) * kWaves2 * 64 * 8 <= sizeof(float) * kWaves2 * kBR * kSMS, "fold");
    static_assert(sizeof(double) * kWaves2 * 64 * 2 <= sizeof(float) * kWaves2 * kBR * kDZS, "foldd");
    float(*fold)[64 * 8] = reinterpret_cast<float(*)[64 * 8]>(&ssm[0][0]);
    double(*foldd)[64 * 2] = reinterpret_cast<double(*)[64 * 2]>(&sdz[0][0]);
    const int lane = threadIdx.x & 63;
    const int wave = __builtin_amdgcn_readfirstlane(threadIdx.x >> 6);
    const int c = lane & 31, r = lane >> 5;
    for (int i = threadIdx.x; i < kOP * kZP; i += 256) swp[i] = w.wp[i];
    if (threadIdx.x < kHW) swv[threadIdx.x] = w.wv[threadIdx.x];
    float w1[kM];
#pragma unroll
    for (int m = 0; m < kM; ++m) w1[m] = w1_at(w, m, c);
    float al = 1.f, be = 0.f, mu = 0.f;
    if constexpr (BN) {
        al = bn.alpha[c];
        be = bn.beta[c];
        mu = bn.part ? bn.mean[c] : 0.f;
    }
    __syncthreads();
    float *dzs = sdz[wave];
    float *sm = ssm[wave];
    float gw[kM] = {0.f, 0.f, 0.f}, gb[kM] = {0.f, 0.f, 0.f}, fc[3] = {0.f, 0.f, 0.f};
    double t1d = 0.0, t2d = 0.0;
    int fo_g[3], fo_a[3];
#pragma unroll
    for (int s = 0; s < 3; ++s) {
        const int i = lane + 64 * s;
        const bool pol = i < kOP * kZP;
        fo_g[s] = pol ? kSmG + i / kZP : kSmGV;
        fo_a[s] = pol ? kSmAP + i % kZP : kSmAV + (i - kOP * kZP < kHW ? i - kOP * kZP : 0);
    }
    const __amdgpu_buffer_rsrc_t rh = heads_rsrc(h, (uint32_t)(N * kRow * 4));
    const __amdgpu_buffer_rsrc_t rd = heads_rsrc(dh, (uint32_t)(N * kRow * 4));
    const int64_t nblocks = (N + kBR - 1) / kBR;
    const int64_t wstep = (int64_t)gridDim.x * kWaves2;
    float *sxw = sx[wave];
    hu32x4 st[kGV];
    if ((int64_t)blockIdx.x * kWaves2 + wave < nblocks)
        load_group(rh, ((int64_t)blockIdx.x * kWaves2 + wave) * kBR, lane, st);
    for (int64_t blk = (int64_t)blockIdx.x * kWaves2 + wave; blk < nblocks; blk += wstep) {
        const int64_t base = blk * kBR;
        asm volatile("" ::: "memory");
        {
            const int row = lane & (kBR - 1);
            const int64_t n = base + row;
            const bool valid = n < N;
            const int64_t nn = valid ? n : 0;
            const int j0 = r * kHW;
            float ap[kHW], g[kOP];
#pragma unroll
            for (int j = 0; j < kHW; ++j) ap[j] = a_p[nn * kZP + j0 + j];
#pragma unroll
            for (int k = 0; k < kOP; ++k) g[k] = valid ? dp[nn * kOP + k] : 0.f;
            float dzp[kHW];
#pragma unroll
            for (int j = 0; j < kHW; ++j) {
                asm volatile("" ::: "memory");
                float t = 0.f;
#pragma unroll
                for (int k = 0; k < kOP; ++k) t += g[k] * swp[k * kZP + j0 + j];
                dzp[j] = ap[j] > 0.f ? t : t * kSlope;
            }
            {
                float t = 0.f;
#pragma unroll
                for (int q = 0; q < kHW; ++q) t += dzp[q];
                gb[r] += t;
            }
            float *dzr = dzs + row * kDZS;
            float *smr = sm + row * kSMS;
#pragma unroll
            for (int j = 0; j < kHW; ++j) {
                dzr[j0 + j] = dzp[j];
                smr[kSmAP + j0 + j] = valid ? ap[j] : 0.f;
            }
            if (r == 0) {
                float av[kHW];
#pragma unroll
                for (int q = 0; q < kHW; ++q) av[q] = a_v[nn * kHW + q];
                float gv = valid ? dv[nn] : 0.f;
                if (vt) gv = gv * (1.f - vt[nn] * vt[nn]);
                float t2 = 0.f;
#pragma unroll
                for (int q = 0; q < kHW; ++q) {
                    const float t = gv * swv[q];
                    const float d = av[q] > 0.f ? t : t * kSlope;
                    dzr[kZP + q] = d;
                    t2 += d;
                    smr[kSmAV + q] = valid ? av[q] : 0.f;
                }
                gb[2] += t2;
                dzr[kZ] = 0.f;
#pragma unroll
                for (int k = 0; k < kOP; ++k) smr[kSmG + k] = g[k];
                smr[kSmGV] = gv;
            }
        }
        lds_fence();
#pragma unroll 4
        for (int row = 0; row < kBR; ++row) {
            const float *smr = sm + row * kSMS;
#pragma unroll
            for (int s = 0; s < 3; ++s) fc[s] += smr[fo_g[s]] * smr[fo_a[s]];
        }
#pragma unroll 1
        for (int g = 0; g < kBR / kGR; ++g) {
#pragma unroll
            for (int k = 0; k < kGV; ++k) *reinterpret_cast<hu32x4 *>(sxw + 4 * (k * 64 + lane)) = st[k];
            lds_fence();
            {
                const int64_t nb = g + 1 < kBR / kGR ? base + kGR * (g + 1) : base + wstep * kBR;
                if (nb < N) {
                    load_group(rh, nb, lane, st);
                } else {
#pragma unroll
                    for (int k = 0; k < kGV; ++k) st[k] = (hu32x4){0u, 0u, 0u, 0u};
                }
            }
#pragma unroll 1
            for (int jj = 0; jj < kGR / 2; ++jj) {
                const int lr = 2 * jj + r;
                float *xr = sxw + lr * kRow + c * kHW;
                float x[kHW];
#pragma unroll
                for (int q = 0; q < kHW; ++q) x[q] = xr[q];
                float dz[kZ + 1];
                const float4 *dzr = reinterpret_cast<const float4 *>(dzs + (kGR * g + lr) * kDZS);
#pragma unroll
                for (int t = 0; t < 7; ++t) {
                    const float4 v = dzr[t];
                    dz[4 * t] = v.x; dz[4 * t + 1] = v.y; dz[4 * t + 2] = v.z; dz[4 * t + 3] = v.w;
                }
                float hx[kHW];
#pragma unroll
                for (int q = 0; q < kHW; ++q) hx[q] = BN ? bn_relu(x[q], al, be) : x[q];
#pragma unroll
                for (int m = 0; m < kM; ++m) {
                    float t = 0.f;
#pragma unroll
                    for (int q = 0; q < kHW; ++q) t += dz[m * kHW + q] * hx[q];
                    gw[m] += t;
                }
                float t1 = 0.f, t2 = 0.f;
#pragma unroll
                for (int q = 0; q < kHW; ++q) {
                    float t = 0.f;
#pragma unroll
                    for (int m = 0; m < kM; ++m) t += w1[m] * dz[m * kHW + q];
                    if constexpr (BN) {
                        if (bn.part) {
                            const float gm = (x[q] * al + be > 0.f) ? t : 0.f;
                            t1 += gm;
                            t2 += gm * (x[q] - mu);
                        }
                    }
                    xr[q] = t;
                }
                t1d += (double)t1;
                t2d += (double)t2;
            }
            lds_fence();
            const uint32_t ob = (uint32_t)((base + kGR * g) * kRow * 4);
#pragma unroll
            for (int k = 0; k < kGV; ++k)
                __builtin_amdgcn_raw_buffer_store_b128(*reinterpret_cast<const hu32x4 *>(sxw + 4 * (k * 64 + lane)),
                                                       rd, ob + (k * 64 + lane) * 16, 0, 0);
            lds_fence();
        }
        lds_fence();
    }
    __syncthreads();
    float *fw = fold[wave];
#pragma unroll
    for (int m = 0; m < kM; ++m) fw[m * 64 + lane] = gw[m];
#pragma unroll
    for (int m = 0; m < kM; ++m) fw[(3 + m) * 64 + lane] = gb[m];
    fw[6 * 64 + lane] = 0.f;
    foldd[wave][lane * 2] = t1d;
    foldd[wave][lane * 2 + 1] = t2d;
    __syncthreads();
    float *out = part + (int64_t)blockIdx.x * kGN;
    if (wave == 0) {
        for (int i = lane; i < kM * kC; i += 64) {
            const int m = i / kC, cc = i % kC;
            float t = 0.f;
            for (int wv = 0; wv < kWaves2; ++wv) t += fold[wv][m * 64 + cc] + fold[wv][m * 64 + cc + 32];
            out[kGW1 + i] = t;
        }
        if (lane < kM) {
            const int l0 = lane == 1 ? kBR : 0;
            float t = 0.f;
            for (int wv = 0; wv < kWaves2; ++wv)
                for (int l = 0; l < kBR; ++l) t += fold[wv][(3 + lane) * 64 + l0 + l];
            out[kGB1 + lane] = t;
        }
        if (BN && bn.part) {
            const int cc = lane >> 1, k = lane & 1;
            double t = 0.0;
            for (int wv = 0; wv < kWaves2; ++wv) t += foldd[wv][cc * 2 + k] + foldd[wv][(cc + 32) * 2 + k];
            bn.part[((int64_t)blockIdx.x * kC + cc) * 2 + k] = t;
        }
    }
    __syncthreads();
#pragma unroll
    for (int s = 0; s < 3; ++s) fw[s * 64 + lane] = fc[s];
    __syncthreads();
    if (wave == 0) {
#pragma unroll
        for (int s = 0; s < 3; ++s) {
            const int i = lane + 64 * s;
            if (i < kFcN) {
                float t = 0.f;
                for (int wv = 0; wv < kWaves2; ++wv) t += fold[wv][s * 64 + lane];
                out[kGWP + i] = t;
            }
        }
    }
}

__global__ __launch_bounds__(256) void fc_grad_kernel(const float *__restrict__ a_p, const float *__restrict__ a_v,
                                                      const float *__restrict__ dp, const float *__restrict__ dv,
                                                      int64_t N, int64_t rows_per_block, float *__restrict__ part) {
    const int t = threadIdx.x;
    if (t >= kOP * kZP + kHW) return;
    const int64_t r0 = (int64_t)blockIdx.x * rows_per_block;
    const int64_t r1 = min(N, r0 + rows_per_block);
    const bool pol = t < kOP * kZP;
    const int k = pol ? t / kZP : 0, j = pol ? t % kZP : t - kOP * kZP;
    float acc = 0.f;
    int64_t n = r0;
    for (; n + 8 <= r1; n += 8) {
        float x[8], y[8];
#pragma unroll
        for (int u = 0; u < 8; ++u) {
            x[u] = pol ? dp[(n + u) * kOP + k] : dv[n + u];
            y[u] = pol ? a_p[(n + u) * kZP + j] : a_v[(n + u) * kHW + j];
        }
#pragma unroll
        for (int u = 0; u < 8; ++u) acc += x[u] * y[u];
    }
    for (; n < r1; ++n) acc += pol ? dp[n * kOP + k] * a_p[n * kZP + j] : dv[n] * a_v[n * kHW + j];
    part[(int64_t)blockIdx.x * kGN + kGWP + t] = acc;
}

__global__ __launch_bounds__(256) void heads_reduce_kernel(const float *__restrict__ part, int nparts,
                                                           float *__restrict__ dw1p, float *__restrict__ dw1v,
                                                           float *__restrict__ db1p, float *__restrict__ db1v,
                                                           float *__restrict__ dwp, float *__restrict__ dwv) {
    __shared__ double red[256];
    const int i = blockIdx.x;
    double s = 0.0;
    for (int b = threadIdx.x; b < nparts; b += 256) s += (double)part[(int64_t)b * kGN + i];
    red[threadIdx.x] = s;
    __syncthreads();
    for (int w = 128; w > 0; w >>= 1) {
        if ((int)threadIdx.x < w) red[threadIdx.x] += red[threadIdx.x + w];
        __syncthreads();
    }
    if (threadIdx.x != 0) return;
    const float v = (float)red[0];
    if (i < kGB1) {
        const int m = i / kC, c = i % kC;
        if (m < kMP) dw1p[m * kC + c] = v;
        else dw1v[(m - kMP) * kC + c] = v;
    } else if (i < kGWP) {
        const int m = i - kGB1;
        if (m < kMP) db1p[m] = v;
        else db1v[m - kMP] = v;
    } else if (i < kGWV) {
        dwp[i - kGWP] = v;
    } else {
        dwv[i - kGWV] = v;
    }
}

constexpr int kGridFwd = 4096;
constexpr int kGridBwd = 768;
constexpr int kGridBwd2 = 512;
int g_heads_bwd_form = 2;

int status() {
    const hipError_t e = hipGetLastError();
    return e == hipSuccess ? HRL_OK : HRL_ELAUNCH_BASE - (int)e;
}

bool aligned16(const void *p) { return (reinterpret_cast<uintptr_t>(p) & 15) == 0; }

int grid_for(int64_t N, int cap = kGridBwd) {
    const int64_t blocks = (N + 63) / 64;
    return (int)(blocks < cap ? blocks : cap);
}

int grid_bwd(int64_t N) {
    if (g_heads_bwd_form != 2) return grid_for(N);
    const int64_t wgs = ((N + kBR - 1) / kBR + kWaves2 - 1) / kWaves2;
    return (int)(wgs < kGridBwd2 ? wgs : kGridBwd2);
}

}

extern "C" {

int64_t hrl_heads_workspace_bytes(int64_t N) {
    return N < 1 ? -1 : ((int64_t)std::max(grid_for(N), grid_bwd(N)) * kGN + N) * 4;
}

int64_t hrl_heads_bn_parts(int64_t N) { return N < 1 ? -1 : grid_bwd(N); }

int hrl_heads_set_bwd_form(int form) {
    const int prev = g_heads_bwd_form;
    if (form == 1 || form == 2) g_heads_bwd_form = form;
    return prev;
}

int hrl_heads_forward(const float *h, int64_t N, const float *w1p, const float *b1p, const float *w1v,
                      const float *b1v, const float *wp, const float *wv, const float *bn_alpha, const float *bn_beta,
                      float *a_p, float *a_v, float *p_out, float *v_out, int tanh_v, void *stream) {
    if (N < 1 || !h || !w1p || !b1p || !w1v || !b1v || !wp || !wv || !p_out || !v_out) return HRL_EINVAL;
    if ((a_p == nullptr) != (a_v == nullptr) || (bn_alpha == nullptr) != (bn_beta == nullptr) || !aligned16(h))
        return HRL_EINVAL;
    const Weights w{w1p, w1v, b1p, b1v, wp, wv};
    const BnIn bn{bn_alpha, bn_beta, nullptr, nullptr};
    hipLaunchKernelGGL(heads_fwd_kernel, dim3(grid_for(N, kGridFwd)), dim3(64), 0, static_cast<hipStream_t>(stream), h, N, w,
                       bn, a_p, a_v, p_out, v_out, tanh_v != 0);
    return status();
}

int hrl_heads_backward(const float *h, int64_t N, const float *w1p, const float *w1v, const float *wp,
                       const float *wv, const float *bn_alpha, const float *bn_beta, const float *bn_mean,
                       double *bn_part, const float *a_p, const float *a_v, const float *dp, const float *dv,
                       const float *v_tanh, float *dh, float *dw1p, float *db1p, float *dw1v, float *db1v, float *dwp, float *dwv,
                       void *workspace, int64_t workspace_bytes, void *stream) {
    if (N < 1 || !h || !w1p || !w1v || !wp || !wv || !a_p || !a_v || !dp || !dv || !dh || !workspace)
        return HRL_EINVAL;
    const bool defer = !dw1p && !db1p && !dw1v && !db1v && !dwp && !dwv;
    if (!defer && (!dw1p || !db1p || !dw1v || !db1v || !dwp || !dwv)) return HRL_EINVAL;
    if (defer && g_heads_bwd_form != 2) return HRL_EINVAL;
    if ((bn_alpha == nullptr) != (bn_beta == nullptr) || (bn_part && (!bn_alpha || !bn_mean))) return HRL_EINVAL;
    if (!aligned16(h) || !aligned16(dh) || workspace_bytes < hrl_heads_workspace_bytes(N)) return HRL_EINVAL;
    hipStream_t s = static_cast<hipStream_t>(stream);
    const Weights w{w1p, w1v, nullptr, nullptr, wp, wv};
    const BnIn bn{bn_alpha, bn_beta, bn_mean, bn_part};
    float *part = static_cast<float *>(workspace);
    if (g_heads_bwd_form == 2) {
        if ((N + kBR) * kRow * 4 >= (int64_t)1 << 32) return HRL_EINVAL;
        const int grid = grid_bwd(N);
        if (bn_alpha)
            hipLaunchKernelGGL(heads_bwd2_kernel<true>, dim3(grid), dim3(256), 0, s, h, N, w, bn, a_p, a_v, dp, dv,
                               v_tanh, dh, part);
        else
            hipLaunchKernelGGL(heads_bwd2_kernel<false>, dim3(grid), dim3(256), 0, s, h, N, w, bn, a_p, a_v, dp, dv,
                               v_tanh, dh, part);
        const int rc = status();
        if (rc || defer) return rc;
        hipLaunchKernelGGL(heads_reduce_kernel, dim3(kGN), dim3(256), 0, s, part, grid, dw1p, dw1v, db1p, db1v, dwp,
                           dwv);
        return status();
    }
    const int grid = grid_for(N);
    float *dv_raw = part + (int64_t)grid * kGN;
    hipLaunchKernelGGL(heads_bwd_kernel, dim3(grid), dim3(64), 0, s, h, N, w, bn, a_p, a_v, dp, dv, v_tanh, dv_raw, dh,
                       part);
    int rc = status();
    if (rc) return rc;
    const int64_t rows = (N + grid - 1) / grid;
    hipLaunchKernelGGL(fc_grad_kernel, dim3(grid), dim3(256), 0, s, a_p, a_v, dp, v_tanh ? dv_raw : dv, N, rows, part);
    rc = status();
    if (rc) return rc;
    hipLaunchKernelGGL(heads_reduce_kernel, dim3(kGN), dim3(256), 0, s, part, grid, dw1p, dw1v, db1p, db1v, dwp,
                       dwv);
    return status();
}

}
```

### handyrl_amd/csrc/hrl_targets.hip

```cpp

#include <hip/hip_runtime.h>
#include <stdint.h>

#include <type_traits>

#include "../../include/hrl_targets.h"
#include "hrl_scan.h"

namespace {

using namespace hrl_scan;

HRL_STAMP_DECL

constexpr int kMaxTile = kTChunk * kWave;
constexpr int kMaxVec = kMaxTile / 4 / kWave;
constexpr int kMaxScalar = kMaxTile / kWave;

struct Chunk {
    const float *base;
    int R;
    int L;
    int Lp;
    int n;
// ... 252 lines not shown
    if (g >= G || b >= a.B) return;
    const int64_t row = b * (int64_t)T;
    const float *pv = a.values + row * C + c;
    const float *pr = REW ? a.rewards + row * C + c : nullptr;
    const float *pret = kRet ? a.returns + row * C + c : nullptr;
    const int rc = c / a.rhoDiv;
    const float *prho = kRho ? a.rhos + row * a.rhoC + rc : nullptr;
    const float *pcs = kRho ? a.cs + row * a.rhoC + rc : nullptr;
    float xv[kTChunk], xr[kTChunk], xrho[kTChunk], xc[kTChunk], xret[kTChunk];
    const float boot = a.returns[b * (int64_t)a.retT * C + (int64_t)(a.retT - 1) * C + c];
#pragma unroll
    for (int tt = 0; tt < kTChunk; ++tt) {
        if (tt < T) {
            xv[tt] = pv[tt * C];
            xr[tt] = REW ? pr[tt * C] : 0.f;
            xret[tt] = kRet ? pret[tt * C] : boot;
            xrho[tt] = kRho ? prho[tt * a.rhoC] : 0.f;
            xc[tt] = kRho ? pcs[tt * a.rhoC] : 0.f;
        }
    }
    float *ptg = TGT != kNone ? a.targets + row * C + c : nullptr;
    float *pad = a.advantages + row * C + c;
    Carry s{0.f, 0.f, 0.f, 0.f, 0.f};
#pragma unroll
    for (int tt = kTChunk - 1; tt >= 0; --tt) {
        if (tt < T) {
            float tg, ad;
            fused_step<TGT, ADV, false>(s, tt == T - 1, xv[tt], xr[tt], xrho[tt], xc[tt], xret[tt], boot, a.k, tg,
                                        ad);
            if constexpr (TGT != kNone) ptg[tt * C] = tg;
            pad[tt * C] = ad;
        }
    }
}

int g_short_form = 1;

template <int TGT, int ADV, bool REW, bool RETT, bool VEC>
int launch_one(const Args &a, hipStream_t stream) {
    constexpr bool kRho = (TGT == HRL_ALG_VTRACE) || (ADV == HRL_ALG_VTRACE);
    constexpr bool kRet = RETT && (ADV == HRL_ALG_MC);
    const int G = a.G;
    const int tmax = a.T < kTChunk ? a.T : kTChunk;
    const int vtiles = 1 + (REW ? 1 : 0) + (kRet ? 1 : 0) + 1;
    const size_t vt = (size_t)G * odd_row(tmax, a.C);
    const size_t rt = (size_t)G * odd_row(tmax, a.rhoC);
    const size_t lds = sizeof(float) * (vtiles * vt + (kRho ? 2 : 0) * rt);
    const int64_t blocks = (a.B + G - 1) / G;
    if (blocks > 0x7fffffff) return HRL_EINVAL;
    if (a.T <= kTChunk && (g_short_form == 2 || (g_short_form == 1 && a.B * a.C <= 32768))) {
        Args b = a;
        b.G = kWave / a.C;
        const int64_t waves = (a.B + b.G - 1) / b.G;
        const int64_t wgs = (waves + 3) / 4;
        if (wgs > 0x7fffffff) return HRL_EINVAL;
        hipLaunchKernelGGL((targets_lane_kernel<TGT, ADV, REW, RETT>), dim3((unsigned)wgs), dim3(4 * kWave), 0,
                           stream, b);
    } else {
        if (a.T <= kTChunk)
            hipLaunchKernelGGL((targets_kernel<TGT, ADV, REW, RETT, VEC, true>), dim3((unsigned)blocks), dim3(kWave),
                               lds, stream, a);
        else
            hipLaunchKernelGGL((targets_kernel<TGT, ADV, REW, RETT, VEC, false>), dim3((unsigned)blocks), dim3(kWave),
                               lds, stream, a);
    }
    const hipError_t err = hipGetLastError();
    return err == hipSuccess ? HRL_OK : HRL_ELAUNCH_BASE - (int)err;
}

bool vector_ok(const Args &a) {
    auto aligned = [](const void *p) { return p == nullptr || (reinterpret_cast<uintptr_t>(p) & 15) == 0; };
    if (!aligned(a.values) || !aligned(a.returns) || !aligned(a.rewards) || !aligned(a.rhos) || !aligned(a.cs) ||
        !aligned(a.targets) || !aligned(a.advantages))
        return false;
    if (a.T <= kTChunk) return true;
    return ((a.T * a.C) & 3) == 0 && ((a.T * a.rhoC) & 3) == 0;
}

template <int TGT, int ADV, bool REW>
int launch_vec(const Args &a, hipStream_t s) {
    const bool rett = (ADV == HRL_ALG_MC) && a.retT == a.T && a.T > 1;
    if (vector_ok(a)) return rett ? launch_one<TGT, ADV, REW, true, true>(a, s) : launch_one<TGT, ADV, REW, false, true>(a, s);
    return rett ? launch_one<TGT, ADV, REW, true, false>(a, s) : launch_one<TGT, ADV, REW, false, false>(a, s);
}

template <int TGT, int ADV>
int launch_flags(const Args &a, hipStream_t s) {
    return a.rewards != nullptr ? launch_vec<TGT, ADV, true>(a, s) : launch_vec<TGT, ADV, false>(a, s);
}

template <int TGT>
int launch_adv(int adv, const Args &a, hipStream_t s) {
    switch (adv) {
        case HRL_ALG_MC: return launch_flags<TGT, HRL_ALG_MC>(a, s);
        case HRL_ALG_TD: return launch_flags<TGT, HRL_ALG_TD>(a, s);
        case HRL_ALG_UPGO: return launch_flags<TGT, HRL_ALG_UPGO>(a, s);
        case HRL_ALG_VTRACE: return launch_flags<TGT, HRL_ALG_VTRACE>(a, s);
        default: return HRL_EINVAL;
    }
}

int dispatch(int tgt, int adv, const Args &a, hipStream_t s) {
    switch (tgt) {
        case kNone: return launch_adv<kNone>(adv, a, s);
        case HRL_ALG_TD: return launch_adv<HRL_ALG_TD>(adv, a, s);
        case HRL_ALG_UPGO: return launch_adv<HRL_ALG_UPGO>(adv, a, s);
        case HRL_ALG_VTRACE: return launch_adv<HRL_ALG_VTRACE>(adv, a, s);
        default: return HRL_EINVAL;
    }
}

bool valid_alg(int alg) { return alg >= HRL_ALG_MC && alg <= HRL_ALG_VTRACE; }

int prepare(int target_alg, int adv_alg, const float *values, const float *returns, const float *rewards,
            const float *rhos, const float *cs, int64_t B, int64_t T, int64_t C, int64_t ret_T,
            int64_t rho_C, int64_t rho_div, double lmb, double gamma, float *targets, float *advantages,
            void *stream) {
    if (!valid_alg(target_alg) || !valid_alg(adv_alg)) return HRL_EINVAL;
    if (B < 0 || T < 1 || C < 1 || C > kWave || T > (1 << 24)) return HRL_EINVAL;
    if (ret_T != 1 && ret_T != T) return HRL_EINVAL;
    if (rho_C < 1 || rho_div < 1 || rho_C * rho_div != C) {
        return HRL_EINVAL;
    }
    if (target_alg == HRL_ALG_MC && targets != nullptr) return HRL_EINVAL;
    if (B == 0) return HRL_OK;
    const bool need_rho = target_alg == HRL_ALG_VTRACE || adv_alg == HRL_ALG_VTRACE;
    if (!values || !returns || !advantages || (need_rho && (!rhos || !cs))) return HRL_EINVAL;
    if (B * T * C > (int64_t)1 << 40 || T * C * kWave >= ((int64_t)1 << 31)) return HRL_EINVAL;
    Args a;
    a.values = values; a.returns = returns; a.rewards = rewards; a.rhos = rhos; a.cs = cs;
    a.targets = targets; a.advantages = advantages;
    a.B = B; a.T = (int)T; a.C = (int)C; a.retT = (int)ret_T; a.rhoC = (int)rho_C; a.rhoDiv = (int)rho_div;
    a.k = make_coef(lmb, gamma);
    {
        const int gmax = kWave / a.C;
        int g = gmax < 4 ? gmax : 4;
        while (g * 2 <= gmax && B / (g * 2) >= 1024) g *= 2;
        a.G = g;
    }
    const int tgt = (targets == nullptr || target_alg == HRL_ALG_MC) ? kNone : target_alg;
    return dispatch(tgt, adv_alg, a, static_cast<hipStream_t>(stream));
}

}

extern "C" {

#ifdef HRL_STAMPS
int hrl_debug_set_stamps_targets(void *buf) {
    return (int)hipMemcpyToSymbol(HIP_SYMBOL(g_hrl_stamps), &buf, sizeof(buf));
}
#endif

int hrl_abi_version(void) { return 27; }

int hrl_targets_set_short_form(int form) {
    const int prev = g_short_form;
    g_short_form = form < 0 ? 0 : (form > 2 ? 2 : form);
    return prev;
}

const char *hrl_strerror(int code) {
    if (code == HRL_OK) return "success";
    if (code == HRL_EINVAL) return "invalid argument (algorithm, shape or pointer)";
    if (code <= HRL_ELAUNCH_BASE) return hipGetErrorString(static_cast<hipError_t>(HRL_ELAUNCH_BASE - code));
    return "unknown error";
}

int hrl_compute_target(int alg, const float *values, const float *returns, const float *rewards,
                       const float *rhos, const float *cs, int64_t B, int64_t T, int64_t C, int64_t ret_T,
                       int64_t rho_C, int64_t rho_div, double lmb, double gamma, float *targets,
                       float *advantages, void *stream) {
    return prepare(alg, alg, values, returns, rewards, rhos, cs, B, T, C, ret_T, rho_C, rho_div, lmb, gamma,
                   targets, advantages, stream);
}

int hrl_compute_targets_fused(int target_alg, int adv_alg, const float *values, const float *returns,
                              const float *rewards, const float *rhos, const float *cs, int64_t B, int64_t T,
                              int64_t C, int64_t ret_T, int64_t rho_C, int64_t rho_div, double lmb,
                              double gamma, float *targets, float *advantages, void *stream) {
    return prepare(target_alg, adv_alg, values, returns, rewards, rhos, cs, B, T, C, ret_T, rho_C, rho_div, lmb,
                   gamma, targets, advantages, stream);
}

}
```

### handyrl_amd/nn.py

```python

import ctypes
import operator

import os

import torch
import torch.fx
import torch.nn as nn
import torch.nn.functional as F

from . import _native

__all__ = ['BatchNorm2d', 'BoardConv2d', 'Linear', 'accelerate', 'batch_norm_train', 'fuse_bn_relu', 'unfuse']

_MAX_ROW = 3072
_MAX_ROW_SCALAR = 1024


class DeferredGrads:

    def __init__(self):
        self.conv = {}
        self.late_params = set()
        self.affine = {}
# ... 1559 lines not shown
                _native.ptr_array(g), _native.ptr(m), _native.ptr(m_next), B, P, Pn, len(live), _native.i64_array(F),
                int(summed), _native.ptr_array(st) if any(x is not None for x in st) else None,
                _native.i64_array([x.stride(-2) if x is not None else f for x, f in zip(st, F)]),
                _native.ptr_array(add) if any(x is not None for x in add) else None,
                _native.i64_array([x.stride(-2) if x is not None else f for x, f in zip(add, F)]),
                _native.ptr_array(a), _native.ptr_array(b), _native.stream_of(m.device)),
                'hrl_hidden_update_gather_backward')
            for k, x, y in zip(live, a, b):
                dH[k], dnh[k] = x, y
        return (None, None, None, None, None, None, None, None, *dH, *dnh)


def _board_conv_ok(m):
    k = m.kernel_size
    return (m.stride == (1, 1) and m.dilation == (1, 1) and m.groups == 1 and m.padding_mode == 'zeros'
            and isinstance(m.padding, tuple) and m.padding == (k[0] // 2, k[1] // 2) and k[0] % 2 == 1
            and k[1] % 2 == 1)


class BatchNorm2d(nn.BatchNorm2d):

    fused_relu = False

    def forward(self, x):
        row = x.shape[1] * x.shape[2] * x.shape[3] if x.dim() == 4 else 0
        shape_ok = (x.is_cuda and x.dtype == torch.float32 and x.dim() == 4
                    and x.shape[0] > 0 and (row <= _MAX_ROW_SCALAR or (row % 4 == 0 and row <= _MAX_ROW)))
        if shape_ok and not self.training and self.track_running_stats and self.running_mean is not None:
            return batch_norm_eval(x, self.weight, self.bias, self.running_mean, self.running_var, self.eps,
                                   self.fused_relu)
        use_hip = shape_ok and self.training
        if not use_hip:
            y = super().forward(x)
            return torch.relu(y) if self.fused_relu else y
        self._check_input_dim(x)
        momentum = 0.0 if self.momentum is None else self.momentum
        if self.track_running_stats and self.num_batches_tracked is not None:
            self.num_batches_tracked.add_(1)
            if self.momentum is None:
                momentum = 1.0 / float(self.num_batches_tracked.item())
        rm = self.running_mean if self.track_running_stats else None
        rv = self.running_var if self.track_running_stats else None
        return batch_norm_train(x, self.weight, self.bias, rm, rv, momentum, self.eps, self.fused_relu)


def accelerate(model):
    for name, child in list(model.named_children()):
        if type(child) is nn.Conv2d and _board_conv_ok(child):
            new = BoardConv2d(child.in_channels, child.out_channels, child.kernel_size, stride=1,
                              padding=child.padding, bias=child.bias is not None,
                              device=child.weight.device, dtype=child.weight.dtype)
            new.weight = child.weight
            if child.bias is not None:
                new.bias = child.bias
            new.train(child.training)
            setattr(model, name, new)
        elif type(child) is nn.Linear:
            new = Linear(child.in_features, child.out_features, bias=child.bias is not None,
                         device=child.weight.device, dtype=child.weight.dtype)
            new.weight = child.weight
            if child.bias is not None:
                new.bias = child.bias
            new.train(child.training)
            setattr(model, name, new)
        elif type(child) is nn.BatchNorm2d:
            new = BatchNorm2d(child.num_features, eps=child.eps, momentum=child.momentum,
                              affine=child.affine, track_running_stats=child.track_running_stats)
            new.weight, new.bias = child.weight, child.bias
            if child.track_running_stats:
                new.running_mean, new.running_var = child.running_mean, child.running_var
                new.num_batches_tracked = child.num_batches_tracked
            new.train(child.training)
            setattr(model, name, new)
        else:
            accelerate(child)
    if hasattr(model, 'use_hip'):
        model.use_hip = True
    return model


class _MultiBoardConv(nn.Module):

    def __init__(self, convs):
        super().__init__()
        object.__setattr__(self, 'convs', list(convs))

    def forward(self, x):
        convs = self.convs
        if not (x.is_cuda and x.dim() == 4 and x.dtype == torch.float32
                and x.shape[2] * x.shape[3] <= BOARD_MAX_CELLS):
            return tuple(c(x) for c in convs)
        N, Cin, H, W = x.shape
        HW = H * W
        wb = torch.cat([_BoardWeight.apply(c.weight, H, W) for c in convs], dim=1)
        parts = [_BoardBias.apply(c.bias, HW) if c.bias is not None else c.weight.new_zeros(c.out_channels * HW)
                 for c in convs]
        y = _RowMatmul.apply(x.reshape(N, Cin * HW), wb, torch.cat(parts))
        outs, off = [], 0
        for c in convs:
            n = c.out_channels * HW
            outs.append(y[:, off:off + n].reshape(N, c.out_channels, H, W))
            off += n
        return tuple(outs)


_UNIT = {}

def _unit_coefs(dev):
    u = _UNIT.get(dev)
    if u is None:
        u = _UNIT[dev] = torch.stack([torch.ones(32, device=dev), torch.zeros(32, device=dev)])
    return u


def _chain_forward(h0, meta, relu_in, params, apply_out=True):
    lib = _native.load()
    M = h0.shape[0]
    dev = h0.device
    stream = _native.stream_of(dev)
    P = _native.ptr
    ws_bytes = lib.hrl_conv3x3_workspace_bytes(M)
    ws = torch.empty(ws_bytes, dtype=torch.uint8, device=dev)
    nblk = lib.hrl_conv3x3_stats_blocks(M)
    part = torch.empty(nblk * 32 * 2, dtype=torch.float64, device=dev)
    unit = _unit_coefs(dev) if relu_in else None
    x = h0
    a_prev, b_prev = (unit[0], unit[1]) if relu_in else (None, None)
    ys, coefs = [], []
    weights = [params[3 * i].contiguous() for i in range(len(meta))]
    packed = torch.empty(len(weights), 2, 9216, dtype=torch.float32, device=dev)
    for k in range(0, len(weights), 8):
        _native.check(lib.hrl_conv3x3_pack_n(_native.ptr_array(weights[k:k + 8]), len(weights[k:k + 8]),
                                             P(packed[k]), stream), 'hrl_conv3x3_pack_n')
    for i, (rm, rv, momentum, eps) in enumerate(meta):
        w, gamma, beta = params[3 * i:3 * i + 3]
        y = torch.empty_like(h0)
        _native.check(lib.hrl_conv3x3_forward_ex(P(x), M, P(a_prev), P(b_prev), P(packed[i, 0]), None, 2, P(y),
                                                 1, None, None, None, None, P(part), P(ws), ws_bytes, stream),
                      'hrl_conv3x3_forward_ex')
        coef = torch.empty(4, 32, dtype=torch.float32, device=dev)
        _native.check(lib.hrl_bn_finalize_stats(P(part), nblk, 32, M * 9, P(gamma), P(beta), P(rm), P(rv),
                                                float(momentum), float(eps), P(coef[0]), P(coef[1]),
                                                P(coef[2]), P(coef[3]), stream), 'hrl_bn_finalize_stats')
        ys.append(y)
        coefs.append(coef)
        x, a_prev, b_prev = y, coef[2], coef[3]
    out = None
    if apply_out:
        out = torch.empty_like(h0)
        _native.check(lib.hrl_bn_apply(P(x), M, 32, 9, P(a_prev), P(b_prev), 1, P(out), stream), 'hrl_bn_apply')
    return out, ys, coefs, unit, packed


def _chain_backward(h0, ys, coefs, unit, params, relu_in, g, need_input_grad, packed, part_in=None, nblk_in=0):
    lib = _native.load()
    n = len(ys)
    M = h0.shape[0]
    dev = h0.device
    stream = _native.stream_of(dev)
    P = _native.ptr
    ws_bytes = lib.hrl_conv3x3_workspace_bytes(M)
    ws = torch.empty(ws_bytes, dtype=torch.uint8, device=dev)
    bn_ws_bytes = lib.hrl_bn_workspace_bytes(M, 32, 9)
    bn_ws = torch.empty(bn_ws_bytes, dtype=torch.uint8, device=dev)
    nblk = lib.hrl_conv3x3_block_sum_blocks(M)
    part = torch.empty(nblk * 32 * 2, dtype=torch.float64, device=dev)
    g = g.contiguous()
    grads = [None] * (3 * n)
    sums, sums_n = (part_in, nblk_in) if part_in is not None else (None, 0)
    for i in reversed(range(n)):
        w, gamma, beta = params[3 * i:3 * i + 3]
        mean, invstd = coefs[i][0], coefs[i][1]
        bw, bgam, bbet = _grad_buffer(w), _grad_buffer(gamma), _grad_buffer(beta)
        dgam, dbet = bgam[0], bbet[0]
        if i == 0:
            x, a, b = h0, (unit[0] if unit is not None else None), (unit[1] if unit is not None else None)
        else:
            x, a, b = ys[i - 1], coefs[i - 1][2], coefs[i - 1][3]
        dw = bw[0]
        if sums is not None:
            kg = torch.empty(2, 32, dtype=torch.float32, device=dev)
            _native.check(lib.hrl_bn_finalize_backward(P(sums), sums_n, 32, M * 9, P(gamma), P(invstd),
                                                       P(dgam), P(dbet), P(kg[0]), P(kg[1]), stream),
                          'hrl_bn_finalize_backward')
            gin, epi, ep = None, 0, (None, None, None)
            if i > 0:
                gin, epi, ep = torch.empty_like(h0), 2, (coefs[i - 1][0], coefs[i - 1][2], coefs[i - 1][3])
            elif need_input_grad:
                gin, epi = torch.empty_like(h0), (3 if relu_in else 0)
            df = _defer_folds([bw])
            wsb = ws if df is None else torch.empty(ws_bytes, dtype=torch.uint8, device=dev)
            ev = _block_timing_start()
            _native.check(lib.hrl_conv3x3_block_backward(
                P(g), P(ys[i]), M, P(gamma), P(beta), P(mean), P(invstd), P(kg[0]), P(kg[1]), P(x), P(a), P(b),
                P(packed[i, 1]), None if df is not None else P(dw), P(gin), epi, P(ep[0]), P(ep[1]), P(ep[2]),
                P(part) if i > 0 else None, P(wsb), ws_bytes, stream), 'hrl_conv3x3_block_backward')
            _block_timing_end(ev)
            if df is not None:
                off = ctypes.c_int64(0)
                nparts = lib.hrl_conv3x3_wgrad_partials(M, ctypes.byref(off))
                df.add(wsb[off.value:].view(torch.float32), 9216, 0, nparts, dw, 9216, mode=1)
                df.keep.append(wsb)
            grads[3 * i:3 * i + 3] = [_ret(bw), _ret(bgam), _ret(bbet)]
            g = gin
            if i > 0:
                sums, sums_n = part, lib.hrl_conv3x3_block_sum_blocks(M)
            continue
        dy = torch.empty_like(h0)
        _native.check(lib.hrl_bn_backward(P(ys[i]), P(g), M, 32, 9, P(gamma), P(beta), P(mean), P(invstd),
                                          1, P(dy), P(dgam), P(dbet), P(bn_ws), bn_ws_bytes, stream),
                      'hrl_bn_backward')
        _native.check(lib.hrl_conv3x3_wgrad_ex(P(x), P(a), P(b), P(dy), M, P(dw), P(ws), ws_bytes, stream),
                      'hrl_conv3x3_wgrad_ex')
        grads[3 * i:3 * i + 3] = [_ret(bw), _ret(bgam), _ret(bbet)]
        if i > 0:
            g = torch.empty_like(h0)
            _native.check(lib.hrl_conv3x3_forward_ex(P(dy), M, None, None, P(packed[i, 1]), None, 3, P(g), 2,
                                                     P(ys[i - 1]),
                                                     P(coefs[i - 1][0]), P(coefs[i - 1][2]),
                                                     P(coefs[i - 1][3]), P(part), P(ws), ws_bytes, stream),
                          'hrl_conv3x3_forward_ex(flip, bn sums)')
            sums, sums_n = part, lib.hrl_conv3x3_stats_blocks(M)
        elif need_input_grad:
            g = torch.empty_like(h0)
            _native.check(lib.hrl_conv3x3_forward_ex(P(dy), M, None, None, P(packed[i, 1]), None, 3, P(g),
                                                     3 if relu_in else 0, P(h0) if relu_in else None,
                                                     None, None, None, None, P(ws), ws_bytes, stream),
                          'hrl_conv3x3_forward_ex(flip)')
        else:
            g = None
    return g, grads


class _BoardChain(torch.autograd.Function):

    @staticmethod
    def forward(ctx, h0, meta, relu_in, *params):
        h0 = h0.contiguous()
        out, ys, coefs, unit, packed = _chain_forward(h0, meta, relu_in, params)
        ctx.save_for_backward(h0, *ys, *coefs, packed, *params)
        ctx.n = len(meta)
        ctx.relu_in = relu_in
        return out

    @staticmethod
    def backward(ctx, g):
        n = ctx.n
        t = ctx.saved_tensors
        h0, ys, coefs, packed, params = t[0], list(t[1:1 + n]), list(t[1 + n:1 + 2 * n]), t[1 + 2 * n], t[2 + 2 * n:]
        unit = _unit_coefs(h0.device) if ctx.relu_in else None
        g_in, grads = _chain_backward(h0, ys, coefs, unit, params, ctx.relu_in, g, ctx.needs_input_grad[0], packed)
        return (g_in, None, None, *grads)


class _ChainHeadsFn(torch.autograd.Function):

    @staticmethod
    def forward(ctx, h0, meta, relu_in, tanh_v, w1p, b1p, w1v, b1v, wp, wv, *params):
        h0 = h0.contiguous()
        _, ys, coefs, unit, packed = _chain_forward(h0, meta, relu_in, params, apply_out=False)
        y, coef = ys[-1], coefs[-1]
        N = h0.shape[0]
        dev = h0.device
        lib = _native.load()
        a_p = torch.empty(N, 18, device=dev, dtype=h0.dtype)
        a_v = torch.empty(N, 9, device=dev, dtype=h0.dtype)
        p = torch.empty(N, 9, device=dev, dtype=h0.dtype)
        v = torch.empty(N, 1, device=dev, dtype=h0.dtype)
        P = _native.ptr
        w1p, w1v, wp, wv = w1p.contiguous(), w1v.contiguous(), wp.contiguous(), wv.contiguous()
        _native.check(lib.hrl_heads_forward(P(y), N, P(w1p), P(b1p.contiguous()), P(w1v), P(b1v.contiguous()),
                                            P(wp), P(wv), P(coef[2]), P(coef[3]), P(a_p), P(a_v), P(p), P(v),
                                            int(tanh_v), _native.stream_of(dev)), 'hrl_heads_forward(bn)')
        ctx.save_for_backward(h0, *ys, *coefs, a_p, a_v, w1p, w1v, wp, wv, packed, v, *params)
        ctx.tanh_v = tanh_v
        ctx.biases = (b1p, b1v)
        ctx.n = len(meta)
        ctx.relu_in = relu_in
        return p, v

    @staticmethod
    def backward(ctx, dp, dv):
        n = ctx.n
        t = ctx.saved_tensors
        h0, ys, coefs = t[0], list(t[1:1 + n]), list(t[1 + n:1 + 2 * n])
        a_p, a_v, w1p, w1v, wp, wv, packed, v = t[1 + 2 * n:9 + 2 * n]
        params = t[9 + 2 * n:]
        b1p, b1v = ctx.biases
        N = h0.shape[0]
        dev = h0.device
        lib = _native.load()
        P = _native.ptr
        y, coef = ys[-1], coefs[-1]
        dp, dv = dp.contiguous(), dv.contiguous()
        dh = torch.empty_like(h0)
        hbufs = [_grad_buffer(x) for x in (w1p, b1p, w1v, b1v, wp, wv)]
        ws_bytes = lib.hrl_heads_workspace_bytes(N)
        ws = torch.empty(ws_bytes, dtype=torch.uint8, device=dev)
        nparts = lib.hrl_heads_bn_parts(N)
        bn_part = torch.empty(nparts * 64, dtype=torch.float64, device=dev)
        def call(*dws):
            _native.check(lib.hrl_heads_backward(P(y), N, P(w1p), P(w1v), P(wp), P(wv), P(coef[2]), P(coef[3]),
                                                 P(coef[0]), P(bn_part), P(a_p), P(a_v), P(dp), P(dv),
                                                 P(v) if ctx.tanh_v else None, P(dh), *(P(t) for t in dws),
                                                 P(ws), ws_bytes, _native.stream_of(dev)), 'hrl_heads_backward(bn)')
        df = _defer_folds(hbufs, 6) if lib.hrl_heads_set_bwd_form(0) == 2 else None
        if df is not None:
            _heads_backward_deferred(lib, df, hbufs, N, ws, call)
        else:
            call(*(b[0] for b in hbufs))
        unit = _unit_coefs(dev) if ctx.relu_in else None
        g_in, grads = _chain_backward(h0, ys, coefs, unit, params, ctx.relu_in, dh, ctx.needs_input_grad[0], packed,
                                      part_in=bn_part, nblk_in=nparts)
        return (g_in, None, None, None, *(_ret(b) for b in hbufs), *grads)


class _ConvBNChain(nn.Module):

    def __init__(self, convs, bns, relu_in=False):
        super().__init__()
        object.__setattr__(self, 'convs', list(convs))
        object.__setattr__(self, 'bns', list(bns))
        self.relu_in = relu_in

    @staticmethod
    def layers_ok(convs, bns):
        return all(type(c) is BoardConv2d and c.bias is None and tuple(c.weight.shape) == (32, 32, 3, 3)
                   and _board_conv_ok(c) for c in convs) and \
            all(isinstance(b, BatchNorm2d) and b.affine and b.track_running_stats and b.momentum is not None
                and b.num_features == 32 for b in bns)

    def forward(self, x):
        convs, bns = self.convs, self.bns
        if not self.fused_ok(x):
            if self.relu_in:
                x = torch.relu(x)
            for c, b in zip(convs, bns):
                x = b(c(x))
            return x
        meta, params = self.meta_params()
        return _BoardChain.apply(x, meta, self.relu_in, *params)

    def fused_ok(self, x):
        return (x.is_cuda and x.dtype == torch.float32 and x.dim() == 4 and tuple(x.shape[1:]) == (32, 3, 3)
                and x.shape[0] > 0 and all(b.training and b.fused_relu for b in self.bns)
                and torch.is_grad_enabled())

    def meta_params(self):
        counters = [b.num_batches_tracked for b in self.bns]
        if not _defer_counters(counters):
            torch._foreach_add_(counters, 1)
        meta, params = [], []
        for c, b in zip(self.convs, self.bns):
            meta.append((b.running_mean, b.running_var, b.momentum, b.eps))
            params += [c.weight, b.weight, b.bias]
        return meta, params


class _ChainHeads(nn.Module):

    def __init__(self, chain, heads):
        super().__init__()
        object.__setattr__(self, 'chain', chain)
        object.__setattr__(self, 'heads', heads)
        self.tanh_v = False

    def forward(self, x):
        if not self.chain.fused_ok(x):
            p, v = self.heads(self.chain(x))
            return p, (torch.tanh(v) if self.tanh_v else v)
        (cp, fp), (cv, fv) = _board_head_spec(self.heads.head_p), _board_head_spec(self.heads.head_v)
        meta, params = self.chain.meta_params()
        return _ChainHeadsFn.apply(x, meta, self.chain.relu_in, self.tanh_v, cp.weight, cp.bias, cv.weight, cv.bias,
                                   fp.weight, fv.weight, *params)


def _fuse_chain_heads(gm):
    for node in list(gm.graph.nodes):
        if node.op != 'call_module' or not isinstance(gm.get_submodule(node.target), _FusedHeads):
            continue
        src = node.args[0] if len(node.args) == 1 else None
        if not (isinstance(src, torch.fx.Node) and src.op == 'call_module'
                and isinstance(gm.get_submodule(src.target), _ConvBNChain) and len(src.users) == 1):
            return 0
        fused = _ChainHeads(gm.get_submodule(src.target), gm.get_submodule(node.target))
        gm.add_submodule('_hrl_chain_heads', fused)
        with gm.graph.inserting_before(src):
            call = gm.graph.call_module('_hrl_chain_heads', src.args)
        node.replace_all_uses_with(call)
        gm.graph.erase_node(node)
        gm.graph.erase_node(src)
        for item in list(call.users):
            if item.op == 'call_function' and item.target is operator.getitem and item.args[1] == 1 \
                    and len(item.users) == 1:
                user = next(iter(item.users))
                if _is_tanh(user, item):
                    user.replace_all_uses_with(item)
                    gm.graph.erase_node(user)
                    fused.tanh_v = True
        return 1
    return 0


class _LeafTracer(torch.fx.Tracer):

    def __init__(self, leaves=()):
        super().__init__()
        self.extra = set(id(m) for m in leaves)

    def is_leaf_module(self, m, qualname):
        return isinstance(m, (BatchNorm2d, BoardConv2d, Linear, _MultiBoardConv, _ConvBNChain)) or \
            id(m) in self.extra or super().is_leaf_module(m, qualname)


def _is_tanh(node, arg):
    if node.op == 'call_function' and node.target in (torch.tanh, torch.nn.functional.tanh):
        return node.args == (arg,) and not node.kwargs
    if node.op == 'call_method' and node.target == 'tanh':
        return node.args == (arg,) and not node.kwargs
    return False


def _is_relu(gm, node):
    if node.op == 'call_function' and node.target in (torch.relu, torch.nn.functional.relu):
        return len(node.args) == 1
    if node.op == 'call_method' and node.target == 'relu':
        return len(node.args) == 1
    if node.op == 'call_module':
        return isinstance(gm.get_submodule(node.target), nn.ReLU)
    return False


def fuse_bn_relu(model, example=None):
    if hasattr(model, 'init_hidden') or 'forward' in model.__dict__:
        return 0
    try:
        heads = _head_pair(model)
        graph = _LeafTracer(leaves=heads or ()).trace(model)
    except Exception:
        return 0
    gm = torch.fx.GraphModule(model, graph)
    pairs = []
    for node in gm.graph.nodes:
        if node.op == 'call_module' and isinstance(gm.get_submodule(node.target), BatchNorm2d):
            users = list(node.users)
            if len(users) == 1 and _is_relu(gm, users[0]) and users[0].args[0] is node:
                pairs.append((node, users[0]))
    for bn_node, relu_node in pairs:
        relu_node.replace_all_uses_with(bn_node)
        gm.graph.erase_node(relu_node)
    bns = [gm.get_submodule(n.target) for n, _ in pairs]
    chains = _fuse_chains(gm, set(n for n, _ in pairs))
    merged = 0
    for node in list(gm.graph.nodes):
        sibs = [u for u in node.users if u.op == 'call_module' and type(gm.get_submodule(u.target)) is BoardConv2d
                and u.args == (node,) and not u.kwargs]
        if len(sibs) < 2:
            continue
        name = '_hrl_multiconv%d' % merged
        gm.add_submodule(name, _MultiBoardConv([gm.get_submodule(u.target) for u in sibs]))
        with gm.graph.inserting_after(node):
            multi = gm.graph.call_module(name, (node,))
        anchor = multi
        for i, u in enumerate(sibs):
            with gm.graph.inserting_after(anchor):
                item = gm.graph.call_function(operator.getitem, (multi, i))
# ... 124 lines not shown
```

### include/hrl_nn.h

```cpp
#ifndef HRL_NN_H
#define HRL_NN_H

#include <stdint.h>

#ifdef __cplusplus
extern "C" {
#endif

int64_t hrl_bn_workspace_bytes(int64_t N, int64_t C, int64_t HW);

int hrl_bn_forward_train(const float *x, int64_t N, int64_t C, int64_t HW,
                         const float *weight, const float *bias,
                         float *running_mean, float *running_var, double momentum, double eps, int relu,
                         float *y, float *save_mean, float *save_invstd,
                         void *workspace, int64_t workspace_bytes, void *stream);

int hrl_bn_backward(const float *x, const float *dy, int64_t N, int64_t C, int64_t HW,
                    const float *weight, const float *bias, const float *save_mean, const float *save_invstd,
                    int relu, float *dx, float *dweight, float *dbias,
                    void *workspace, int64_t workspace_bytes, void *stream);

int hrl_bn_finalize_stats(const double *part, int64_t nparts, int64_t C, int64_t count, const float *weight,
                          const float *bias, float *running_mean, float *running_var, double momentum, double eps,
                          float *save_mean, float *save_invstd, float *alpha, float *beta, void *stream);
int hrl_bn_apply(const float *x, int64_t N, int64_t C, int64_t HW, const float *alpha, const float *beta, int relu,
                 float *y, void *stream);
int hrl_bn_forward_eval(const float *x, int64_t N, int64_t C, int64_t HW, const float *weight, const float *bias,
                        const float *running_mean, const float *running_var, double eps, int relu, float *y,
                        float *coef, void *stream);
int64_t hrl_bn_workspace_bytes_grouped(int64_t N, int64_t C, int64_t HW, int64_t G);
int hrl_bn_forward_train_grouped(const float *x, int64_t N, int64_t C, int64_t HW, int64_t G, const float *weight,
                                 const float *bias, float *running_mean, float *running_var, double momentum,
                                 double eps, int relu, float *y, float *save_mean, float *save_invstd,
                                 void *workspace, int64_t workspace_bytes, void *stream);
int hrl_bn_backward_grouped(const float *x, const float *dy, int64_t N, int64_t C, int64_t HW, int64_t G,
                            const float *weight, const float *bias, const float *save_mean, const float *save_invstd,
                            int relu, float *dx, float *dweight, float *dbias, void *workspace,
                            int64_t workspace_bytes, void *stream);
int hrl_bn_finalize_backward(const double *part, int64_t nparts, int64_t C, int64_t count, const float *weight,
                             const float *save_invstd, float *dweight, float *dbias, float *kcoef, float *gmean,
                             void *stream);
int hrl_bn_backward_apply(const float *x, const float *dy, int64_t N, int64_t C, int64_t HW, const float *weight,
                          const float *bias, const float *save_mean, const float *save_invstd, int relu,
                          const float *kcoef, const float *gmean, float *dx, void *stream);

int hrl_bn_apply_residual(const float *x, const float *res, int64_t N, int64_t C, int64_t HW, const float *alpha,
                          const float *beta, float *y, void *stream);
int hrl_bn_backward_masked(const float *x, const float *dy, const float *out, int64_t N, int64_t C, int64_t HW,
                           const float *weight, const float *save_mean, const float *save_invstd, float *dx,
                           float *dweight, float *dbias, void *workspace, int64_t workspace_bytes, void *stream);
int hrl_bn_backward_masked_coefs(const float *x, const float *dy, const float *out, int64_t N, int64_t C,
                                 int64_t HW, const float *weight, const float *save_mean, const float *save_invstd,
                                 float *kcoef, float *gmean, float *dweight, float *dbias, void *workspace,
                                 int64_t workspace_bytes, void *stream);
int hrl_bn_backward_apply_masked(const float *x, const float *dy, const float *out, int64_t N, int64_t C, int64_t HW,
                                 const float *weight, const float *save_mean, const float *save_invstd,
                                 const float *kcoef, const float *gmean, float *dx, void *stream);

int hrl_board_weight(const float *w, int64_t Cout, int64_t Cin, int64_t kh, int64_t kw, int64_t H, int64_t W,
                     float *w_board, void *stream);
int hrl_board_fold(const float *g_board, int64_t Cout, int64_t Cin, int64_t kh, int64_t kw, int64_t H, int64_t W,
                   float *g_w, void *stream);
int hrl_board_bias(const float *b, int64_t Cout, int64_t HW, float *b_board, void *stream);
int hrl_board_bias_fold(const float *g_board, int64_t Cout, int64_t HW, float *g_b, void *stream);

int64_t hrl_colsum_workspace_bytes(int64_t M, int64_t N);
int hrl_colsum(const float *x, int64_t M, int64_t N, float *out, void *workspace, int64_t workspace_bytes,
               void *stream);

int64_t hrl_conv3x3_workspace_bytes(int64_t M);
int hrl_conv3x3_forward(const float *x, int64_t M, int64_t C_in, int64_t C_out, const float *weight,
                        const float *bias, int flip, float *y, void *workspace, int64_t workspace_bytes,
                        void *stream);
int hrl_conv3x3_wgrad(const float *x, const float *dy, int64_t M, int64_t C_in, int64_t C_out, float *dweight,
                      void *workspace, int64_t workspace_bytes, void *stream);

int64_t hrl_conv3x3_stats_blocks(int64_t M);
int hrl_conv3x3_set_split(int on);
int hrl_conv3x3_set_block_form(int form);
int64_t hrl_conv3x3_block_sum_blocks(int64_t M);
int hrl_conv3x3_set_fwd_form(int form);
int hrl_conv3x3_pack_n(const float *const *weights, int n, float *packed, void *stream);
int hrl_conv3x3_forward_ex(const float *x, int64_t M, const float *in_alpha, const float *in_beta,
                           const float *weight, const float *bias, int flip, float *y, int epilogue,
                           const float *ref, const float *ep_mean, const float *ep_alpha, const float *ep_beta,
                           double *part, void *workspace, int64_t workspace_bytes, void *stream);
int hrl_conv3x3_wgrad_ex(const float *x, const float *in_alpha, const float *in_beta, const float *dy, int64_t M,
                         float *dweight, void *workspace, int64_t workspace_bytes, void *stream);

int64_t hrl_conv3x3_wgrad_partials(int64_t M, int64_t *offset_bytes);
int hrl_conv3x3_block_backward(const float *g, const float *y, int64_t M, const float *bn_weight,
                               const float *bn_bias, const float *save_mean, const float *save_invstd,
                               const float *kcoef, const float *gmean, const float *x, const float *in_alpha,
                               const float *in_beta, const float *packed_flip, float *dweight, float *gin,
                               int epilogue, const float *ep_mean, const float *ep_alpha, const float *ep_beta,
                               double *part, void *workspace, int64_t workspace_bytes, void *stream);

int hrl_lstm_gates_forward(const float *zx, int64_t zx_stride, const float *zh, const float *c, int64_t N, int64_t H,
                           int64_t HW, const float *bias, int64_t bias_rows, float *h_out, float *c_out, float *gates,
                           void *stream);
int hrl_lstm_gates_forward_grouped(int L, const float *zh, int64_t zh_stride, const float *const *zx,
                                   const int64_t *zx_strides, const float *const *c, int64_t N, int64_t H, int64_t HW,
                                   float *const *h_out, float *const *c_out, float *const *gates, void *stream);
int hrl_lstm_gates_backward_ex(const float *gates, const float *c, const float *c_out, const float *dh,
                               int64_t dh_stride, int dh_parts, int64_t dh_part_stride, const float *dc_out,
                               int64_t N, int64_t H, int64_t HW, float *dz, float *dc, float *dzx, int dzx_init,
                               void *stream);
int hrl_lstm_gates_backward(const float *gates, const float *c, const float *c_out, const float *dh,
                            const float *dc_out, int64_t N, int64_t H, int64_t HW, float *dz, float *dc,
                            void *stream);

int hrl_hidden_gather(const float *const *H, const float *mask, int64_t B, int64_t P, int nleaves, const int64_t *F,
                      int sum, float *const *out, void *stream);
int hrl_hidden_gather_backward(const float *const *dout, const float *mask, int64_t B, int64_t P, int nleaves,
                               const int64_t *F, int sum, float *const *dH, void *stream);
int hrl_hidden_update(const float *const *H, const float *const *nh, int64_t Pn, const float *mask, int64_t B,
                      int64_t P, int nleaves, const int64_t *F, float *const *out, void *stream);
int hrl_hidden_update_backward(const float *const *dout, const float *mask, int64_t B, int64_t P, int64_t Pn,
                               int nleaves, const int64_t *F, float *const *dH, float *const *dnh, void *stream);
int hrl_hidden_gather_backward_add(const float *const *dout, const float *mask, int64_t B, int64_t P, int nleaves,
                                   const int64_t *F, int sum, const float *const *addend,
                                   const int64_t *addend_strides, float *const *dH, void *stream);
int hrl_hidden_update_backward_add(const float *const *dout, const float *mask, int64_t B, int64_t P, int64_t Pn,
                                   int nleaves, const int64_t *F, const float *const *addend,
                                   const int64_t *addend_strides, float *const *dH, float *const *dnh,
                                   void *stream);
int hrl_hidden_update_gather(const float *const *H, const float *const *nh, int64_t Pn, const float *mask,
                             const float *mask_next, int64_t B, int64_t P, int nleaves, const int64_t *F, int sum,
                             float *const *out, float *const *gathered, void *stream);
int hrl_hidden_update_gather_backward(const float *const *dgathered, const float *mask, const float *mask_next,
                                      int64_t B, int64_t P, int64_t Pn, int nleaves, const int64_t *F, int sum,
                                      const float *const *dstate, const int64_t *dstate_strides,
                                      const float *const *dout_add, const int64_t *dout_add_strides,
                                      float *const *dH, float *const *dnh, void *stream);

int64_t hrl_torus_workspace_bytes(int64_t N);
int hrl_torus_set_split(int on);
int hrl_torus_set_form(int form);
int64_t hrl_torus_stats_blocks(int64_t N);
int hrl_torus_conv_forward(const float *x, int64_t N, int64_t Cin, int64_t Cout, int64_t H, int64_t W,
                           const float *weight, const float *bias, int flip, float *y, double *part,
                           const float *add, const float *add_mask, void *workspace, int64_t workspace_bytes,
                           void *stream);
int hrl_torus_conv_wgrad(const float *x, const float *dy, int64_t N, int64_t Cin, int64_t Cout, int64_t H, int64_t W,
                         float *dweight, float *dbias, void *workspace, int64_t workspace_bytes, void *stream);
int hrl_torus_conv_wgrad_bn(const float *x, int64_t N, int64_t Cin, int64_t H, int64_t W, const float *y,
                            const float *g, const float *alpha, const float *beta, int residual, const float *gamma,
                            const float *save_mean, const float *save_invstd, const float *kcoef, const float *gmean,
                            float *dy, float *dweight, float *dbias, void *workspace, int64_t workspace_bytes,
                            void *stream);

int hrl_torus_unit_forward(const float *y_prev, const float *res, const float *alpha, const float *beta, float *h,
                           int64_t N, int64_t H, int64_t W, const float *weight, const float *bias, float *y,
                           double *part, void *workspace, int64_t workspace_bytes, void *stream);
int64_t hrl_board_conv_workspace_bytes(int64_t Cout);
int hrl_board_conv_forward(const float *x, int64_t N, int64_t Cin, int64_t H, int64_t W, const float *weight,
                           int64_t w_cin_total, int64_t w_ci0, int64_t Cout, const float *bias, float *y,
                           void *workspace, int64_t workspace_bytes, void *stream);
int hrl_board_conv_pack(const float *weight, int64_t w_cin_total, int64_t w_ci0, int64_t Cout, void *packed,
                        int64_t packed_bytes, void *stream);
int hrl_board_conv_forward_packed(const float *x, int64_t N, int64_t Cin, int64_t H, int64_t W, const void *packed,
                                  int64_t Cout, const float *bias, float *y, void *stream);

int64_t hrl_gboard_pack_bytes(int64_t Cout, int64_t Cin_g);
int hrl_gboard_pack(const float *weight, int64_t Cout, int64_t Cin_g, int64_t w_cin_total, int64_t w_ci0,
                    void *packed, int64_t packed_bytes, void *stream);
int hrl_gboard_pack_adjoint(const float *weight, int64_t Cout_fwd, int64_t w_cin_total, int64_t w_ci0,
                            int64_t Cin_slice, void *packed, int64_t packed_bytes, void *stream);
int64_t hrl_gboard_wgrad_workspace_bytes(int64_t Cout, int64_t Cin, int64_t total_games);
int hrl_gboard_wgrad(const float *const *xs, const int64_t *x_strides, const float *const *dys,
                     const int64_t *dy_strides, const int64_t *ns, int nseg, int64_t Cout, int64_t Cin,
                     float *dweight, int64_t w_cin_total, int64_t w_ci0, float *dbias, void *workspace,
                     int64_t workspace_bytes, void *stream);
int hrl_gboard_set_whole_ring(int on);
int hrl_gboard_set_nctw(int nctw);
int hrl_gboard_launch_stats(int64_t *counts, int n, int reset);
int64_t hrl_gboard_pointwise_wgrad_workspace_bytes(int64_t C, int64_t O, int64_t N);
int hrl_gboard_pointwise_wgrad(const float *x, int64_t x_stride, const float *dy, int64_t dy_stride, int64_t N,
                               int64_t C, int64_t O, float *dweight, void *workspace, int64_t workspace_bytes,
                               void *stream);
int hrl_gboard_forward_groups(const float *const *xs, const int64_t *x_strides, int64_t N, int64_t Cin_g,
                              int64_t groups, const void *packed, int64_t packed_bytes, int64_t Cout, float *y,
                              int64_t y_stride, void *stream);
int hrl_gboard_forward(const float *x, int64_t x_stride, const float *x2, int64_t x2_stride, int64_t N, int64_t Cin_g,
                       int64_t groups, const void *packed, int64_t packed_bytes, int64_t Cout, const float *bias,
                       const float *alpha, const float *beta, int relu, float *y, int64_t y_stride, void *stream);

int hrl_gboard_pointwise(const float *x1, int64_t x1_stride, int64_t C1, const float *x2, int64_t x2_stride,
                          int64_t C2, int64_t N, const float *weight, int64_t O, const float *alpha, const float *beta,
                          int relu, float *y, int64_t y_stride, void *stream);

int hrl_torus_head_pool(const float *h, const float *x, int64_t N, int64_t H, int64_t W, int64_t x_stride,
                        float *head, float *avg, void *stream);
int hrl_torus_head_unpool(const float *dhead, const float *davg, const float *x, int64_t N, int64_t H, int64_t W,
                          int64_t x_stride, float *g, void *stream);
int hrl_torus_unit_input_grad(const float *dy, int64_t N, int64_t H, int64_t W, const float *weight, const float *g,
                              const float *out, float *dh, const float *h_mask, const float *y_prev,
                              const float *mean_prev, double *part, void *workspace, int64_t workspace_bytes,
                              void *stream);

int64_t hrl_heads_workspace_bytes(int64_t N);
int64_t hrl_heads_bn_parts(int64_t N);
int hrl_heads_forward(const float *h, int64_t N, const float *w1p, const float *b1p, const float *w1v,
                      const float *b1v, const float *wp, const float *wv, const float *bn_alpha, const float *bn_beta,
                      float *a_p, float *a_v, float *p_out, float *v_out, int tanh_v, void *stream);
int hrl_heads_set_bwd_form(int form);
int hrl_heads_backward(const float *h, int64_t N, const float *w1p, const float *w1v, const float *wp,
                       const float *wv, const float *bn_alpha, const float *bn_beta, const float *bn_mean,
                       double *bn_part, const float *a_p, const float *a_v, const float *dp, const float *dv,
                       const float *v_tanh, float *dh, float *dw1p, float *db1p, float *dw1v, float *db1v, float *dwp, float *dwv,
                       void *workspace, int64_t workspace_bytes, void *stream);

int64_t hrl_stem_workspace_bytes(int64_t N);
int hrl_stem_forward(const float *x, int64_t N, int64_t Cin, const float *weight, const float *bias, float *y,
                     void *stream);
int hrl_stem_wgrad(const float *x, const float *dy, int64_t N, int64_t Cin, float *dweight, float *dbias,
                   void *workspace, int64_t workspace_bytes, void *stream);
int64_t hrl_stem_wgrad_partials(int64_t N, int64_t *row_floats);
int hrl_stem_set_wgrad_form(int form);
int hrl_stem_set_fwd_form(int form);

int64_t hrl_grad_fold_norm_blocks(int64_t n);
int hrl_grad_fold_norm(float *grads, int64_t n, const float *const *parts, const int64_t *strides,
                       const int64_t *col0, const int64_t *nparts, const int64_t *dst, const int64_t *count,
                       const int *modes, int nfolds, float *step, int64_t *const *counters,
                       const int64_t *increments, int ncounters, double *norm_part, int64_t norm_part_bytes,
                       void *stream);
int hrl_adam_clip(float *grads, int64_t n, const double *norm_part, double max_norm, float *total_norm,
                  float *const *params, const int64_t *offsets, const int *live, int ntensors, float *exp_avg,
                  float *exp_avg_sq, const float *lr, const float *step, double beta1, double beta2, double eps,
                  double weight_decay, const float *const *acc_src, int nacc, float *acc_dst, void *stream);

int hrl_clip_grad_norm(float *grads, int64_t n, double max_norm, float *total_norm, void *stream);
int64_t hrl_clip_workspace_bytes(int64_t n);
int hrl_clip_grad_norm_ws(float *grads, int64_t n, double max_norm, float *total_norm, void *workspace,
                          int64_t workspace_bytes, void *stream);

#ifdef __cplusplus
}
#endif

#endif
```

Baseline: 132.1 million env-steps/s.

## Pass compact head pre-activation grads into last conv block backward instead of full dh

The heads backward kernel can now emit only the compact per-cell head pre-activation gradients (28 floats per row) instead of the full hidden-state gradient. The last conv block's backward kernel rebuilds dh on the fly from those values and the 1x1 head weights (w1p, w1v). This avoids writing and re-reading a full N x C x HW gradient tensor between the two kernels. The cost is extra LDS staging and a small dot product per element in the conv backward, and the new path applies only when the block and heads backward forms match.

```diff
diff --git a/handyrl_amd/_native.py b/handyrl_amd/_native.py
--- a/handyrl_amd/_native.py
+++ b/handyrl_amd/_native.py
@@ -90,6 +90,10 @@
                                                   _f32p, _f32p, _f32p, _f32p, _f32p, _f32p, ctypes.c_int, _f32p,
                                                   _f32p, _f32p, ctypes.c_void_p, ctypes.c_void_p, _i64,
                                                   ctypes.c_void_p]),
+    'hrl_conv3x3_block_backward_dz': (ctypes.c_int, [_f32p, _f32p, _f32p, _f32p, _i64, _f32p, _f32p, _f32p, _f32p,
+                                                     _f32p, _f32p, _f32p, _f32p, _f32p, _f32p, _f32p, _f32p,
+                                                     ctypes.c_int, _f32p, _f32p, _f32p, ctypes.c_void_p,
+                                                     ctypes.c_void_p, _i64, ctypes.c_void_p]),
     'hrl_conv3x3_wgrad_ex': (ctypes.c_int, [_f32p, _f32p, _f32p, _f32p, _i64, _f32p, ctypes.c_void_p, _i64,
                                             ctypes.c_void_p]),
     'hrl_hidden_gather': (ctypes.c_int, [ctypes.c_void_p, _f32p, _i64, _i64, ctypes.c_int, ctypes.c_void_p,
@@ -149,6 +153,9 @@
     'hrl_heads_backward': (ctypes.c_int, [_f32p, _i64, _f32p, _f32p, _f32p, _f32p, _f32p, _f32p, _f32p,
                                           ctypes.c_void_p, _f32p, _f32p, _f32p, _f32p, _f32p, _f32p, _f32p, _f32p,
                                           _f32p, _f32p, _f32p, _f32p, ctypes.c_void_p, _i64, ctypes.c_void_p]),
+    'hrl_heads_backward_dz': (ctypes.c_int, [_f32p, _i64, _f32p, _f32p, _f32p, _f32p, _f32p, _f32p, _f32p,
+                                             ctypes.c_void_p, _f32p, _f32p, _f32p, _f32p, _f32p, _f32p, _f32p, _f32p,
+                                             _f32p, _f32p, _f32p, _f32p, ctypes.c_void_p, _i64, ctypes.c_void_p]),
     'hrl_bn_apply_residual': (ctypes.c_int, [_f32p, _f32p, _i64, _i64, _i64, _f32p, _f32p, _f32p, ctypes.c_void_p]),
     'hrl_bn_backward_masked': (ctypes.c_int, [_f32p, _f32p, _f32p, _i64, _i64, _i64, _f32p, _f32p, _f32p, _f32p,
                                               _f32p, _f32p, ctypes.c_void_p, _i64, ctypes.c_void_p]),
@@ -221,7 +228,7 @@
                                                       ctypes.c_void_p]),
 }
 
-ABI_VERSION = 27
+ABI_VERSION = 28
 
 _lib = None
 
diff --git a/handyrl_amd/csrc/hrl_conv.hip b/handyrl_amd/csrc/hrl_conv.hip
--- a/handyrl_amd/csrc/hrl_conv.hip
+++ b/handyrl_amd/csrc/hrl_conv.hip
@@ -561,6 +561,7 @@
     double *part;
     float *wpart;
     int64_t M;
+    const float *w1p = nullptr, *w1v = nullptr;
 };
 
 typedef unsigned int u32x3 __attribute__((ext_vector_type(3)));
@@ -840,6 +841,12 @@
 constexpr int kXr0 = 4 * kImgBytes;
 constexpr int kLdsBytes = kXr0 + 2 * kXrBytes;
 static_assert(kLdsBytes <= 160 * 1024, "LDS");
+constexpr int kDzStride = 28;
+constexpr int kDzBytes = kTile * kDzStride * 4;
+constexpr int kDz0 = kLdsBytes;
+constexpr int kLdsBytesDz = kDz0 + 2 * kDzBytes;
+static_assert(kLdsBytesDz <= 160 * 1024, "LDS");
+static_assert(kDzBytes / 4 <= 7 * 64, "a dword per lane of waves 0..6");
 
 typedef short v4s __attribute__((ext_vector_type(4)));
 typedef __attribute__((address_space(3))) v4s lds_v4s;
@@ -908,8 +915,9 @@
 #define BB2_STAMP(it, k) do { } while (0)
 #endif
 
-template <bool PRO, int EPI, int W>
+template <bool PRO, int EPI, int W, bool DZ = false>
 __device__ __forceinline__ void run(const BlockBwdArgs &a, unsigned char *smem, int lane) {
+    static_assert(!DZ || EPI == 2, "the dz form is the last chain block's");
     using R = Role<W>;
     constexpr bool kIg = R::kIg;
     constexpr int kNq = R::kNq > 0 ? R::kNq : 1;
@@ -929,6 +937,12 @@
     if constexpr (PRO) {
         pa = a.in_alpha[ch];
         pb = a.in_beta[ch];
+    }
+    float w1[3] = {0.f, 0.f, 0.f};
+    if constexpr (DZ) {
+        w1[0] = a.w1p[ch];
+        w1[1] = a.w1p[kC + ch];
+        w1[2] = a.w1v[ch];
     }
     uint4 wh[kTaps], wm[kTaps], wl[kTaps];
     if constexpr (kIg) {
@@ -989,7 +1003,7 @@
         for (int r = 0; r < 2; ++r) {
             const int off = ldoff + r * kRow * 4;
 #pragma unroll
-            for (int k = kFwd ? 2 : 0; k < 3; ++k) {
+            for (int k = kFwd ? 2 : (DZ ? 1 : 0); k < 3; ++k) {
                 const __amdgpu_buffer_rsrc_t rs = k == 0 ? rg : (k == 1 ? ry : rx);
                 float(&d)[5] = k == 0 ? G[r] : (k == 1 ? Y[r] : X[r]);
                 const u32x3 v = __builtin_amdgcn_raw_buffer_load_b96(rs, off, 0, 0);
@@ -1002,11 +1016,29 @@
             }
         }
     };
+    auto load_dz = [&](int it) __attribute__((always_inline)) {
+        float v = 0.f;
+        if constexpr (DZ && W < 7) {
+            const int64_t t = t0 + (int64_t)it * step;
+            const bool ok = it < n_iter;
+            const int rows = ok ? (int)min<int64_t>(kTile, a.M - t * kTile) : 0;
+            const __amdgpu_buffer_rsrc_t rz =
+                wave_rsrc(a.g + (ok ? t * kTile * kDzStride : 0), (uint32_t)rows * kDzStride * 4);
+            v = __uint_as_float(__builtin_amdgcn_raw_buffer_load_b32(rz, (W * 64 + lane) * 4, 0, 0));
+        }
+        return v;
+    };
+    auto put_dz = [&](int it, float v) __attribute__((always_inline)) {
+        if constexpr (DZ && W < 7)
+            reinterpret_cast<float *>(smem + kDz0 + (it & 1) * kDzBytes)[W * 64 + lane] = v;
+    };
+    float DZv = 0.f;
     auto stage = [&](int it) __attribute__((always_inline)) {
         const int64_t t = t0 + (int64_t)it * step;
         const int rows = (int)max<int64_t>(0, min<int64_t>(kTile, a.M - t * kTile));
         unsigned char *dyi = smem + kDy0 + (it & 1) * kImgBytes;
         unsigned char *xi = smem + kX0 + (it & 1) * kImgBytes;
+        const float *dzl = reinterpret_cast<const float *>(smem + kDz0 + (it & 1) * kDzBytes);
         uint32_t dp[3][5], xp[3][5];
 #pragma unroll
         for (int i = 0; i < 5; ++i) {
@@ -1015,7 +1047,15 @@
             for (int r = 0; r < 2; ++r) {
                 const bool valid = rho0 + r < rows;
                 const float yv = Y[r][i];
-                float gv = G[r][i];
+                float gv;
+                if constexpr (DZ) {
+                    const float *dzr = dzl + (rho0 + r) * kDzStride + c0 + i;
+                    gv = 0.f;
+#pragma unroll
+                    for (int m = 0; m < 3; ++m) gv += w1[m] * dzr[m * kCells];
+                } else {
+                    gv = G[r][i];
+                }
                 if (!(yv * al + be > 0.f)) gv = 0.f;
                 const float tt = (yv - mu) * kk;
                 float d = (((gv - gmn) - tt) * is) * ww;
@@ -1193,7 +1233,20 @@
         }
     };
 
-    if (n_iter > 0) {
+    if constexpr (DZ) {
+        if (n_iter > 0) {
+            const float d0 = load_dz(0), d1 = load_dz(1);
+            issue(0);
+            put_dz(0, d0);
+            put_dz(1, d1);
+            DZv = load_dz(2);
+        }
+        bar_lds();
+        if (n_iter > 0) {
+            stage(0);
+            issue(1);
+        }
+    } else if (n_iter > 0) {
         issue(0);
         stage(0);
         issue(1);
@@ -1206,10 +1259,18 @@
             epilogue(it);
             BB2_STAMP(it, 1);
             stage(it + 1);
+            if constexpr (DZ) {
+                put_dz(it + 2, DZv);
+                DZv = load_dz(it + 3);
+            }
             issue(it + 2);
             BB2_STAMP(it, 2);
         } else {
             stage(it + 1);
+            if constexpr (DZ) {
+                put_dz(it + 2, DZv);
+                DZv = load_dz(it + 3);
+            }
             issue(it + 2);
             BB2_STAMP(it, 1);
             compute(it);
@@ -1531,20 +1592,20 @@
     }
 }
 
-template <bool PRO, int EPI>
+template <bool PRO, int EPI, bool DZ = false>
 __global__ __launch_bounds__(bb2::kThreads) void conv3x3_block_bwd2_kernel(BlockBwdArgs a) {
-    __shared__ __attribute__((aligned(16))) unsigned char smem[bb2::kLdsBytes];
+    __shared__ __attribute__((aligned(16))) unsigned char smem[DZ ? bb2::kLdsBytesDz : bb2::kLdsBytes];
     const int lane = threadIdx.x & 63;
     const int wave = __builtin_amdgcn_readfirstlane(threadIdx.x >> 6);
     switch (wave) {
-    case 0: bb2::run<PRO, EPI, 0>(a, smem, lane); break;
-    case 1: bb2::run<PRO, EPI, 1>(a, smem, lane); break;
-    case 2: bb2::run<PRO, EPI, 2>(a, smem, lane); break;
-    case 3: bb2::run<PRO, EPI, 3>(a, smem, lane); break;
-    case 4: bb2::run<PRO, EPI, 4>(a, smem, lane); break;
-    case 5: bb2::run<PRO, EPI, 5>(a, smem, lane); break;
-    case 6: bb2::run<PRO, EPI, 6>(a, smem, lane); break;
-    default: bb2::run<PRO, EPI, 7>(a, smem, lane); break;
+    case 0: bb2::run<PRO, EPI, 0, DZ>(a, smem, lane); break;
+    case 1: bb2::run<PRO, EPI, 1, DZ>(a, smem, lane); break;
+    case 2: bb2::run<PRO, EPI, 2, DZ>(a, smem, lane); break;
+    case 3: bb2::run<PRO, EPI, 3, DZ>(a, smem, lane); break;
+    case 4: bb2::run<PRO, EPI, 4, DZ>(a, smem, lane); break;
+    case 5: bb2::run<PRO, EPI, 5, DZ>(a, smem, lane); break;
+    case 6: bb2::run<PRO, EPI, 6, DZ>(a, smem, lane); break;
+    default: bb2::run<PRO, EPI, 7, DZ>(a, smem, lane); break;
     }
 }
 
@@ -1805,6 +1866,35 @@
     return status();
 }
 
+int hrl_conv3x3_block_backward_dz(const float *dz, const float *w1p, const float *w1v, const float *y, int64_t M,
+                                  const float *bn_weight, const float *bn_bias, const float *save_mean,
+                                  const float *save_invstd, const float *kcoef, const float *gmean, const float *x,
+                                  const float *in_alpha, const float *in_beta, const float *packed_flip,
+                                  float *dweight, float *gin, int epilogue, const float *ep_mean,
+                                  const float *ep_alpha, const float *ep_beta, double *part, void *workspace,
+                                  int64_t workspace_bytes, void *stream) {
+    if (M < 1 || !dz || !w1p || !w1v || !y || !save_mean || !save_invstd || !kcoef || !gmean || !x || !workspace)
+        return HRL_EINVAL;
+    if ((in_alpha == nullptr) != (in_beta == nullptr)) return HRL_EINVAL;
+    if (workspace_bytes < hrl_conv3x3_workspace_bytes(M) || M * kRow * 4 > 0xffffffffLL) return HRL_EINVAL;
+    if (g_block_form != 1 || epilogue != 2 || !gin || !packed_flip) return HRL_EINVAL;
+    if (!ep_mean || !ep_alpha || !ep_beta || !part) return HRL_EINVAL;
+    hipStream_t s = static_cast<hipStream_t>(stream);
+    const int grid = grid_for(M);
+    float *wpart = static_cast<float *>(workspace) + kTaps * 2 * kC * 16 * 2;
+    BlockBwdArgs a{dz, y, bn_weight, bn_bias, save_mean, save_invstd, kcoef, gmean, x, in_alpha, in_beta, packed_flip,
+                   ep_mean, ep_alpha, ep_beta, gin, part, wpart, M, w1p, w1v};
+    if (in_alpha)
+        hipLaunchKernelGGL((conv3x3_block_bwd2_kernel<true, 2, true>), dim3(grid), dim3(bb2::kThreads), 0, s, a);
+    else
+        hipLaunchKernelGGL((conv3x3_block_bwd2_kernel<false, 2, true>), dim3(grid), dim3(bb2::kThreads), 0, s, a);
+    int rc = status();
+    if (rc || !dweight) return rc;
+    hipLaunchKernelGGL(conv3x3_wgrad_reduce_kernel, dim3(kTaps * kC * kC / 64), dim3(256), 0, s, wpart, grid,
+                       dweight);
+    return status();
+}
+
 int64_t hrl_conv3x3_wgrad_partials(int64_t M, int64_t *offset_bytes) {
     if (M < 1) return -1;
     if (offset_bytes) *offset_bytes = (int64_t)kTaps * 2 * kC * 16 * 2 * 4;
diff --git a/handyrl_amd/csrc/hrl_heads.hip b/handyrl_amd/csrc/hrl_heads.hip
--- a/handyrl_amd/csrc/hrl_heads.hip
+++ b/handyrl_amd/csrc/hrl_heads.hip
@@ -398,7 +398,7 @@
     for (int k = 0; k < kGV; ++k) st[k] = __builtin_amdgcn_raw_buffer_load_b128(rh, ob + (k * 64 + lane) * 16, 0, 0);
 }
 
-template <bool BN>
+template <bool BN, bool DZ = false>
 __global__ __launch_bounds__(256, 2) void heads_bwd2_kernel(const float *__restrict__ h, int64_t N, Weights w, BnIn bn,
                                                          const float *__restrict__ a_p, const float *__restrict__ a_v,
                                                          const float *__restrict__ dp, const float *__restrict__ dv,
@@ -440,7 +440,7 @@
         fo_a[s] = pol ? kSmAP + i % kZP : kSmAV + (i - kOP * kZP < kHW ? i - kOP * kZP : 0);
     }
     const __amdgpu_buffer_rsrc_t rh = heads_rsrc(h, (uint32_t)(N * kRow * 4));
-    const __amdgpu_buffer_rsrc_t rd = heads_rsrc(dh, (uint32_t)(N * kRow * 4));
+    const __amdgpu_buffer_rsrc_t rd = heads_rsrc(dh, (uint32_t)(N * (DZ ? kDZS : kRow) * 4));
     const int64_t nblocks = (N + kBR - 1) / kBR;
     const int64_t wstep = (int64_t)gridDim.x * kWaves2;
     float *sxw = sx[wave];
@@ -506,6 +506,16 @@
             }
         }
         lds_fence();
+        if constexpr (DZ) {
+            const uint32_t ob = (uint32_t)(base * kDZS * 4);
+#pragma unroll
+            for (int k = 0; k < (kBR * kDZS / 4 + 63) / 64; ++k) {
+                const int i = k * 64 + lane;
+                if (i < kBR * kDZS / 4)
+                    __builtin_amdgcn_raw_buffer_store_b128(*reinterpret_cast<const hu32x4 *>(dzs + 4 * i), rd,
+                                                           ob + i * 16, 0, 0);
+            }
+        }
 #pragma unroll 4
         for (int row = 0; row < kBR; ++row) {
             const float *smr = sm + row * kSMS;
@@ -563,17 +573,20 @@
                             t2 += gm * (x[q] - mu);
                         }
                     }
-                    xr[q] = t;
+                    if constexpr (!DZ) xr[q] = t;
                 }
                 t1d += (double)t1;
                 t2d += (double)t2;
             }
-            lds_fence();
-            const uint32_t ob = (uint32_t)((base + kGR * g) * kRow * 4);
-#pragma unroll
-            for (int k = 0; k < kGV; ++k)
-                __builtin_amdgcn_raw_buffer_store_b128(*reinterpret_cast<const hu32x4 *>(sxw + 4 * (k * 64 + lane)),
-                                                       rd, ob + (k * 64 + lane) * 16, 0, 0);
+            if constexpr (!DZ) {
+                lds_fence();
+                const uint32_t ob = (uint32_t)((base + kGR * g) * kRow * 4);
+#pragma unroll
+                for (int k = 0; k < kGV; ++k)
+                    __builtin_amdgcn_raw_buffer_store_b128(
+                        *reinterpret_cast<const hu32x4 *>(sxw + 4 * (k * 64 + lane)), rd, ob + (k * 64 + lane) * 16, 0,
+                        0);
+            }
             lds_fence();
         }
         lds_fence();
@@ -735,11 +748,16 @@
     return status();
 }
 
-int hrl_heads_backward(const float *h, int64_t N, const float *w1p, const float *w1v, const float *wp,
-                       const float *wv, const float *bn_alpha, const float *bn_beta, const float *bn_mean,
-                       double *bn_part, const float *a_p, const float *a_v, const float *dp, const float *dv,
-                       const float *v_tanh, float *dh, float *dw1p, float *db1p, float *dw1v, float *db1v, float *dwp, float *dwv,
-                       void *workspace, int64_t workspace_bytes, void *stream) {
+}
+
+namespace {
+
+int heads_backward(const float *h, int64_t N, const float *w1p, const float *w1v, const float *wp, const float *wv,
+                   const float *bn_alpha, const float *bn_beta, const float *bn_mean, double *bn_part,
+                   const float *a_p, const float *a_v, const float *dp, const float *dv, const float *v_tanh, float *dh,
+                   float *dw1p, float *db1p, float *dw1v, float *db1v, float *dwp, float *dwv, void *workspace,
+                   int64_t workspace_bytes, void *stream, bool emit_dz) {
+    if (emit_dz && g_heads_bwd_form != 2) return HRL_EINVAL;
     if (N < 1 || !h || !w1p || !w1v || !wp || !wv || !a_p || !a_v || !dp || !dv || !dh || !workspace)
         return HRL_EINVAL;
     const bool defer = !dw1p && !db1p && !dw1v && !db1v && !dwp && !dwv;
@@ -754,12 +772,15 @@
     if (g_heads_bwd_form == 2) {
         if ((N + kBR) * kRow * 4 >= (int64_t)1 << 32) return HRL_EINVAL;
         const int grid = grid_bwd(N);
-        if (bn_alpha)
-            hipLaunchKernelGGL(heads_bwd2_kernel<true>, dim3(grid), dim3(256), 0, s, h, N, w, bn, a_p, a_v, dp, dv,
-                               v_tanh, dh, part);
-        else
-            hipLaunchKernelGGL(heads_bwd2_kernel<false>, dim3(grid), dim3(256), 0, s, h, N, w, bn, a_p, a_v, dp, dv,
-                               v_tanh, dh, part);
+#define HRL_HEADS_BWD2(BN, DZ)                                                                                       \
+    hipLaunchKernelGGL((heads_bwd2_kernel<BN, DZ>), dim3(grid), dim3(256), 0, s, h, N, w, bn, a_p, a_v, dp, dv, v_tanh, \
+                       dh, part)
+        if (emit_dz) {
+            if (bn_alpha) HRL_HEADS_BWD2(true, true); else HRL_HEADS_BWD2(false, true);
+        } else {
+            if (bn_alpha) HRL_HEADS_BWD2(true, false); else HRL_HEADS_BWD2(false, false);
+        }
+#undef HRL_HEADS_BWD2
         const int rc = status();
         if (rc || defer) return rc;
         hipLaunchKernelGGL(heads_reduce_kernel, dim3(kGN), dim3(256), 0, s, part, grid, dw1p, dw1v, db1p, db1v, dwp,
@@ -782,3 +803,25 @@
 }
 
 }
+
+extern "C" {
+
+int hrl_heads_backward(const float *h, int64_t N, const float *w1p, const float *w1v, const float *wp,
+                       const float *wv, const float *bn_alpha, const float *bn_beta, const float *bn_mean,
+                       double *bn_part, const float *a_p, const float *a_v, const float *dp, const float *dv,
+                       const float *v_tanh, float *dh, float *dw1p, float *db1p, float *dw1v, float *db1v, float *dwp, float *dwv,
+                       void *workspace, int64_t workspace_bytes, void *stream) {
+    return heads_backward(h, N, w1p, w1v, wp, wv, bn_alpha, bn_beta, bn_mean, bn_part, a_p, a_v, dp, dv, v_tanh, dh,
+                          dw1p, db1p, dw1v, db1v, dwp, dwv, workspace, workspace_bytes, stream, false);
+}
+
+int hrl_heads_backward_dz(const float *h, int64_t N, const float *w1p, const float *w1v, const float *wp,
+                          const float *wv, const float *bn_alpha, const float *bn_beta, const float *bn_mean,
+                          double *bn_part, const float *a_p, const float *a_v, const float *dp, const float *dv,
+                          const float *v_tanh, float *dz, float *dw1p, float *db1p, float *dw1v, float *db1v,
+                          float *dwp, float *dwv, void *workspace, int64_t workspace_bytes, void *stream) {
+    return heads_backward(h, N, w1p, w1v, wp, wv, bn_alpha, bn_beta, bn_mean, bn_part, a_p, a_v, dp, dv, v_tanh, dz,
+                          dw1p, db1p, dw1v, db1v, dwp, dwv, workspace, workspace_bytes, stream, true);
+}
+
+}
diff --git a/handyrl_amd/csrc/hrl_targets.hip b/handyrl_amd/csrc/hrl_targets.hip
--- a/handyrl_amd/csrc/hrl_targets.hip
+++ b/handyrl_amd/csrc/hrl_targets.hip
@@ -428,7 +428,7 @@
 }
 #endif
 
-int hrl_abi_version(void) { return 27; }
+int hrl_abi_version(void) { return 28; }
 
 int hrl_targets_set_short_form(int form) {
     const int prev = g_short_form;
diff --git a/handyrl_amd/nn.py b/handyrl_amd/nn.py
--- a/handyrl_amd/nn.py
+++ b/handyrl_amd/nn.py
@@ -1735,7 +1735,21 @@
     return out, ys, coefs, unit, packed
 
 
-def _chain_backward(h0, ys, coefs, unit, params, relu_in, g, need_input_grad, packed, part_in=None, nblk_in=0):
+HEADS_DZ = True
+
+
+def _heads_dz_ok(lib, n):
+    return HEADS_DZ and n >= 2 and lib.hrl_heads_set_bwd_form(0) == 2 and _block_form(lib) == 1
+
+
+def _block_form(lib):
+    form = lib.hrl_conv3x3_set_block_form(1)
+    lib.hrl_conv3x3_set_block_form(form)
+    return form
+
+
+def _chain_backward(h0, ys, coefs, unit, params, relu_in, g, need_input_grad, packed, part_in=None, nblk_in=0,
+                    heads_dz=None):
     lib = _native.load()
     n = len(ys)
     M = h0.shape[0]
@@ -1749,6 +1763,7 @@
     nblk = lib.hrl_conv3x3_block_sum_blocks(M)
     part = torch.empty(nblk * 32 * 2, dtype=torch.float64, device=dev)
     g = g.contiguous()
+    assert heads_dz is None or (part_in is not None and n >= 2)
     grads = [None] * (3 * n)
     sums, sums_n = (part_in, nblk_in) if part_in is not None else (None, 0)
     for i in reversed(range(n)):
@@ -1774,10 +1789,17 @@
             df = _defer_folds([bw])
             wsb = ws if df is None else torch.empty(ws_bytes, dtype=torch.uint8, device=dev)
             ev = _block_timing_start()
-            _native.check(lib.hrl_conv3x3_block_backward(
-                P(g), P(ys[i]), M, P(gamma), P(beta), P(mean), P(invstd), P(kg[0]), P(kg[1]), P(x), P(a), P(b),
-                P(packed[i, 1]), None if df is not None else P(dw), P(gin), epi, P(ep[0]), P(ep[1]), P(ep[2]),
-                P(part) if i > 0 else None, P(wsb), ws_bytes, stream), 'hrl_conv3x3_block_backward')
+            if heads_dz is not None and i == n - 1:
+                _native.check(lib.hrl_conv3x3_block_backward_dz(
+                    P(g), P(heads_dz[0]), P(heads_dz[1]), P(ys[i]), M, P(gamma), P(beta), P(mean), P(invstd),
+                    P(kg[0]), P(kg[1]), P(x), P(a), P(b), P(packed[i, 1]), None if df is not None else P(dw), P(gin),
+                    epi, P(ep[0]), P(ep[1]), P(ep[2]), P(part), P(wsb), ws_bytes, stream),
+                    'hrl_conv3x3_block_backward_dz')
+            else:
+                _native.check(lib.hrl_conv3x3_block_backward(
+                    P(g), P(ys[i]), M, P(gamma), P(beta), P(mean), P(invstd), P(kg[0]), P(kg[1]), P(x), P(a), P(b),
+                    P(packed[i, 1]), None if df is not None else P(dw), P(gin), epi, P(ep[0]), P(ep[1]), P(ep[2]),
+                    P(part) if i > 0 else None, P(wsb), ws_bytes, stream), 'hrl_conv3x3_block_backward')
             _block_timing_end(ev)
             if df is not None:
                 off = ctypes.c_int64(0)
@@ -1876,17 +1898,19 @@
         P = _native.ptr
         y, coef = ys[-1], coefs[-1]
         dp, dv = dp.contiguous(), dv.contiguous()
-        dh = torch.empty_like(h0)
+        use_dz = _heads_dz_ok(lib, n)
+        dh = torch.empty(N, 28, device=dev, dtype=h0.dtype) if use_dz else torch.empty_like(h0)
+        heads_backward = lib.hrl_heads_backward_dz if use_dz else lib.hrl_heads_backward
         hbufs = [_grad_buffer(x) for x in (w1p, b1p, w1v, b1v, wp, wv)]
         ws_bytes = lib.hrl_heads_workspace_bytes(N)
         ws = torch.empty(ws_bytes, dtype=torch.uint8, device=dev)
         nparts = lib.hrl_heads_bn_parts(N)
         bn_part = torch.empty(nparts * 64, dtype=torch.float64, device=dev)
         def call(*dws):
-            _native.check(lib.hrl_heads_backward(P(y), N, P(w1p), P(w1v), P(wp), P(wv), P(coef[2]), P(coef[3]),
-                                                 P(coef[0]), P(bn_part), P(a_p), P(a_v), P(dp), P(dv),
-                                                 P(v) if ctx.tanh_v else None, P(dh), *(P(t) for t in dws),
-                                                 P(ws), ws_bytes, _native.stream_of(dev)), 'hrl_heads_backward(bn)')
+            _native.check(heads_backward(P(y), N, P(w1p), P(w1v), P(wp), P(wv), P(coef[2]), P(coef[3]),
+                                         P(coef[0]), P(bn_part), P(a_p), P(a_v), P(dp), P(dv),
+                                         P(v) if ctx.tanh_v else None, P(dh), *(P(t) for t in dws),
+                                         P(ws), ws_bytes, _native.stream_of(dev)), 'hrl_heads_backward(bn)')
         df = _defer_folds(hbufs, 6) if lib.hrl_heads_set_bwd_form(0) == 2 else None
         if df is not None:
             _heads_backward_deferred(lib, df, hbufs, N, ws, call)
@@ -1894,7 +1918,7 @@
             call(*(b[0] for b in hbufs))
         unit = _unit_coefs(dev) if ctx.relu_in else None
         g_in, grads = _chain_backward(h0, ys, coefs, unit, params, ctx.relu_in, dh, ctx.needs_input_grad[0], packed,
-                                      part_in=bn_part, nblk_in=nparts)
+                                      part_in=bn_part, nblk_in=nparts, heads_dz=(w1p, w1v) if use_dz else None)
         return (g_in, None, None, None, *(_ret(b) for b in hbufs), *grads)
 
 
diff --git a/include/hrl_nn.h b/include/hrl_nn.h
--- a/include/hrl_nn.h
+++ b/include/hrl_nn.h
@@ -95,6 +95,13 @@
                                const float *in_beta, const float *packed_flip, float *dweight, float *gin,
                                int epilogue, const float *ep_mean, const float *ep_alpha, const float *ep_beta,
                                double *part, void *workspace, int64_t workspace_bytes, void *stream);
+int hrl_conv3x3_block_backward_dz(const float *dz, const float *w1p, const float *w1v, const float *y, int64_t M,
+                                  const float *bn_weight, const float *bn_bias, const float *save_mean,
+                                  const float *save_invstd, const float *kcoef, const float *gmean, const float *x,
+                                  const float *in_alpha, const float *in_beta, const float *packed_flip,
+                                  float *dweight, float *gin, int epilogue, const float *ep_mean,
+                                  const float *ep_alpha, const float *ep_beta, double *part, void *workspace,
+                                  int64_t workspace_bytes, void *stream);
 
 int hrl_lstm_gates_forward(const float *zx, int64_t zx_stride, const float *zh, const float *c, int64_t N, int64_t H,
                            int64_t HW, const float *bias, int64_t bias_rows, float *h_out, float *c_out, float *gates,
@@ -210,6 +217,11 @@
                        double *bn_part, const float *a_p, const float *a_v, const float *dp, const float *dv,
                        const float *v_tanh, float *dh, float *dw1p, float *db1p, float *dw1v, float *db1v, float *dwp, float *dwv,
                        void *workspace, int64_t workspace_bytes, void *stream);
+int hrl_heads_backward_dz(const float *h, int64_t N, const float *w1p, const float *w1v, const float *wp,
+                          const float *wv, const float *bn_alpha, const float *bn_beta, const float *bn_mean,
+                          double *bn_part, const float *a_p, const float *a_v, const float *dp, const float *dv,
+                          const float *v_tanh, float *dz, float *dw1p, float *db1p, float *dw1v, float *db1v,
+                          float *dwp, float *dwv, void *workspace, int64_t workspace_bytes, void *stream);
 
 int64_t hrl_stem_workspace_bytes(int64_t N);
 int hrl_stem_forward(const float *x, int64_t N, int64_t Cin, const float *weight, const float *bias, float *y,
```

New measurement: 136.3 million env-steps/s (median of 6 runs). 1.03x the previous value.
